# OCR-D/ocrd_keraslm

Hardware: AMD Instinct MI355X
Metric: chars/sec training (stacked-LSTM forward+backward+Adam) (higher is better)
Workload: dtype bf16; 1 GPU; cfg2: depth=2 width=512 length=256 V=256 1 context, stateful training, 3072 streams/GPU, synthetic 10M-char corpus (SURVEY.md 8d); streams_per_gpu=3072, global_batch=3072, seq_len=256, parallelism=dp1

## Files before the change

ocrd_keraslm_amd/csrc/api.hip:

```cpp
#include <hip/hip_runtime.h>
#include <stdio.h>
#include <stdlib.h>
#include <string.h>
#include <time.h>

#include <functional>
#include <utility>

#include <vector>

#include "kl_common.h"
#include "kl_kernels.h"

namespace {

inline size_t align_up(size_t x, size_t a) { return (x + a - 1) / a * a; }
inline int round_up_i(int x, int a) { return (x + a - 1) / a * a; }

struct Carver {
  unsigned char* base;
  size_t off = 0;
  explicit Carver(void* b) : base(reinterpret_cast<unsigned char*>(b)) {}
  template <typename T>
  T* take(size_t count) {
    off = align_up(off, 256);
    T* p = base ? reinterpret_cast<T*>(base + off) : nullptr;
    off += count * sizeof(T);
    return p;
  }
};

constexpr int KL_SCAN_FLAGS = 256 * 64;
struct Derived {
  std::vector<bf16_t*> UT_hi, UT_lo, KT_hi, KT_lo, Un, Kn;
  bf16_t *E_hi = nullptr, *E_lo = nullptr, *ET = nullptr;
  std::vector<bf16_t*> WTcat;
  std::vector<bf16_t*> UF, KF;
  bf16_t* EF = nullptr;
  std::vector<bf16_t*> WTperm;
  bf16_t* Ecat = nullptr;
  float* EK = nullptr;
  std::vector<float*> CtxK;
  std::vector<bf16_t*> KTp;
  std::vector<float*> bp;
  float* EKp = nullptr;
  bf16_t* comb = nullptr;
  std::vector<float*> CtxKp;
  unsigned* scan_flags = nullptr;
};

struct WindowWs {
  float* P1;
  std::vector<void*> H;
  std::vector<float*> C;
  float* logits;
  float* rowstat;
  int *s_idx, *s_ctx, *s_tgt;
  int* ids_tm = nullptr;
  int scan2_rows = 0;
  bool scan2_bwd = false;
  float *s_masks, *s_probs;
  unsigned *scan_cnt, *scan_status;
  float* reg_scratch;
  std::vector<bf16_t*> G, dZ, Hd;
  std::vector<bf16_t*> Cb;
  std::vector<bf16_t*> Xhi, Xlo;
  std::vector<bf16_t*> HTf, HdT;
  bool ht_ready = false;
  bool km_plan = false;
  unsigned p_bf16_mask = 0;
  bf16_t *dZT, *HT, *dlogits, *dlogitsT, *OHT, *dEKT_bf, *dEK_bf;
  std::vector<bf16_t*> OHC;
  bool segsum = false;
  void* seg_ws = nullptr;
  float *dH, *dEKT;
  std::vector<float*> dc0, dc1, dCtxKT;
};

}

struct kl_handle {
  kl_config cfg;
  int Vp;
  size_t n_params;
  std::vector<size_t> off_K, off_U, off_b, off_Ctx;
  size_t off_E;
  float* params = nullptr;
  void* derived_ws = nullptr;
  size_t derived_bytes = 0;
  Derived d;
  int precision = 0;
  struct GraphKey {
    int kind, B, T, flags, precision;
    const void *states, *loss_acc, *ws, *grads;
    int layout = 0;
    bool operator==(const GraphKey& o) const {
      return kind == o.kind && B == o.B && T == o.T && flags == o.flags && precision == o.precision &&
             states == o.states && loss_acc == o.loss_acc && ws == o.ws && grads == o.grads && layout == o.layout;
    }
  };
  std::vector<std::pair<GraphKey, hipGraphExec_t>> graphs;
  bool graphs_enabled = true;
  bool scan_enabled = true;
  bool seq_bwd = true;
  bool wide_bwd = true;
  void* host_step_ready = nullptr;
  std::vector<int32_t> host_pack;
  bool host_kernarg = true;
  void* walk_ready = nullptr;
  bool inc_ready = false;
  bool big_ready = false;
  bool il_ready = false;
  bool comb_ready = false;
  int last_only = 0;
  int loss_rows = 0;
  bool sentinel = true;
  bool gemm_an = true;
  bool xcd_local = false;
  bool sentinel_bwd = true;
  bool sentinel_roll = true;
  bool sentinel_bwd_all = false;
  bool xcd_local_bwd = false;
  bool w32 = true;
  bool w32_local = false;
  int w32_min_rb = 8;
  bool split8 = true;
  bool split_sentinel = true;
  bool inc_small = true;
  bool fused_step = true;
  bool inc_tile = true;
  int tile_var = 0;
  int tile_rows = -1;
  bool out_fused = true;
  int out_fused_min = 512;
  int inc_small_min = KL_SMALL_STEP_N;
  bool scan2 = true;
  int scan2_rows = 0;
  int scan2_pf = -1;
  bool scan2_bf16 = true;
  bool logits_ws = true;
  bool proj_ws = true;
  bool w128 = true;
  bool w128_tables = true;
  bool w128_multi = true;
  bool w128_fuse = true;
  int w128_min = 1;
  bool fwd8 = true;
  bool fwd8_all = false;
  bool fwd8_tab = true;
  bool fwd8_ls = true;
  bool fwd8_local = true;
  int fwd8_pf = -1;
  bool rt_local = true;
  bool regtile = true;
  bool scan2_flags = true;
  bool flags_zeroed = false;
  struct ViewNote {
    int B, T;
    const void* ws;
    int scan2_rows, g_interleaved, c_in_cb, dh_bf16;
    unsigned p_bf16_mask;
    unsigned wg_route = 0, wg_pair_mask = 0, wg_db_scan_mask = 0, hd_mask = 0;
    unsigned out_route = 0;
  };
  std::vector<ViewNote> view_notes;
  ViewNote* view_note(int B, int T, const void* ws, bool insert) {
    for (auto& n : view_notes)
      if (n.B == B && n.T == T && n.ws == ws) return &n;
    if (!insert) return nullptr;
    if (view_notes.size() >= 64) view_notes.erase(view_notes.begin());
    view_notes.push_back(ViewNote{B, T, ws, 0, 0, 0, 0, 0u});
    return &view_notes.back();
  }
  bool segsum = true;
  bool fuse_wg = true;
  int scan2_pfb = -1;
  int wide_fwd_min = 96;
  double trace_flops[2] = {0.0, 0.0};
  bool trace_on = false;
  std::vector<std::pair<hipEvent_t, hipEvent_t>> trace_ev[2];
  size_t trace_used[2] = {0, 0};
  bool trace_open[2] = {false, false};
  bool trace_persistent[2] = {false, false};
  const char* trace_name[2] = {"lstm_fwd_step_kernel", "lstm_bwd_step_kernel"};
  void trace_begin(int kind, hipStream_t s) {
    if (!trace_on) return;
    if (trace_used[kind] == trace_ev[kind].size()) {
      hipEvent_t a, b;
      if (hipEventCreate(&a) != hipSuccess || hipEventCreate(&b) != hipSuccess) { trace_on = false; return; }
      trace_ev[kind].emplace_back(a, b);
    }
    (void)hipEventRecord(trace_ev[kind][trace_used[kind]].first, s);
    trace_open[kind] = true;
  }
  void trace_end(int kind, hipStream_t s) {
    if (!trace_on || !trace_open[kind]) return;
    trace_open[kind] = false;
    (void)hipEventRecord(trace_ev[kind][trace_used[kind]].second, s);
    ++trace_used[kind];
  }
  void drop_graphs() {
    for (auto& g : graphs) (void)hipGraphExecDestroy(g.second);
    graphs.clear();
  }
};

namespace {

void layout(kl_handle* h) {
  const kl_config& c = h->cfg;
  const size_t W = c.width;
  size_t off = 0;
  h->off_E = off;
  off += (size_t)c.voc_size * W;
  h->off_Ctx.clear();
  for (int n = 0; n < c.n_ctx; ++n) {
    h->off_Ctx.push_back(off);
    off += (size_t)c.ctx_vocab * c.ctx_dim;
  }
  h->off_K.clear();
  h->off_U.clear();
  h->off_b.clear();
  for (int l = 0; l < c.depth; ++l) {
    const size_t D = l == 0 ? W + (size_t)c.ctx_dim * c.n_ctx : W;
    h->off_K.push_back(off);
    off += D * 4 * W;
    h->off_U.push_back(off);
    off += W * 4 * W;
    h->off_b.push_back(off);
    off += 4 * W;
  }
  h->n_params = off;
  h->Vp = round_up_i(c.voc_size, 32);
}

bool config_ok(const kl_config* c) {
  if (!c) return false;
  if (c->depth < 1 || c->depth > 16) return false;
  if (c->width < 32 || (c->width & 31)) return false;
// ... 12 lines not shown
  o.UT_hi.assign(c.depth, nullptr); o.UT_lo.assign(c.depth, nullptr);
  o.KT_hi.assign(c.depth, nullptr); o.KT_lo.assign(c.depth, nullptr);
  o.Un.assign(c.depth, nullptr); o.Kn.assign(c.depth, nullptr);
  for (int l = 0; l < c.depth; ++l) {
    o.UT_hi[l] = cv.take<bf16_t>(4 * W * W);
    o.UT_lo[l] = cv.take<bf16_t>(4 * W * W);
    o.KT_hi[l] = cv.take<bf16_t>(4 * W * W);
    o.KT_lo[l] = cv.take<bf16_t>(4 * W * W);
    o.Un[l] = cv.take<bf16_t>(4 * W * W);
    o.Kn[l] = cv.take<bf16_t>(4 * W * W);
  }
  o.E_hi = cv.take<bf16_t>(Vp * W);
  o.E_lo = cv.take<bf16_t>(Vp * W);
  o.ET = cv.take<bf16_t>(W * Vp);
  o.EK = cv.take<float>(V * 4 * W);
  o.WTcat.assign(c.depth, nullptr);
  for (int l = 0; l < c.depth; ++l) o.WTcat[l] = cv.take<bf16_t>(4 * W * 3 * (l == 0 ? W : 2 * W));
  o.WTperm.assign(c.depth, nullptr);
  if ((W & 31) == 0)
    for (int l = 0; l < c.depth; ++l) o.WTperm[l] = cv.take<bf16_t>(4 * W * 3 * (l == 0 ? W : 2 * W));
  o.Ecat = cv.take<bf16_t>(Vp * 3 * W);
  o.UF.assign(c.depth, nullptr);
  o.KF.assign(c.depth, nullptr);
  if ((W & 31) == 0) {
    for (int l = 0; l < c.depth; ++l) {
      o.UF[l] = cv.take<bf16_t>(4 * W * W * 2);
      if (l > 0) o.KF[l] = cv.take<bf16_t>(4 * W * W * 2);
    }
    o.EF = cv.take<bf16_t>(Vp * W * 2);
  }
  o.CtxK.assign(c.n_ctx, nullptr);
  for (int n = 0; n < c.n_ctx; ++n) o.CtxK[n] = cv.take<float>((size_t)c.ctx_vocab * 4 * W);
  o.KTp.assign(c.depth, nullptr);
  o.bp.assign(c.depth, nullptr);
  for (int l = 1; l < c.depth; ++l) {
    o.KTp[l] = cv.take<bf16_t>(4 * W * W);
    o.bp[l] = cv.take<float>(4 * W);
  }
  o.EKp = cv.take<float>(V * 4 * W);
  o.CtxKp.assign(c.n_ctx, nullptr);
  for (int n = 0; n < c.n_ctx; ++n) o.CtxKp[n] = cv.take<float>((size_t)c.ctx_vocab * 4 * W);
  o.scan_flags = cv.take<unsigned>(KL_SCAN_FLAGS + 64);
  o.comb = nullptr;
  if (h->fwd8_tab && W == 512 && c.n_ctx == 1 && V * (size_t)c.ctx_vocab * 4 * W * sizeof(bf16_t) <= ((size_t)512 << 20))
    o.comb = cv.take<bf16_t>(V * (size_t)c.ctx_vocab * 4 * W);
  return align_up(cv.off, 256);
}

bool kl_segsum_applicable(const kl_handle* h, int B, int T) {
  const kl_config& c = h->cfg;
  if (!h->segsum || B < 1 || T < 1 || (long)B * T > 0x7fffffffL) return false;
  return (long)kl_segment_sums_buckets(c.n_ctx, h->Vp, c.ctx_vocab) <= KL_SEGSUM_MAX_BUCKETS;
}

size_t carve_window(const kl_handle* h, void* base, int B, int T, int training, WindowWs* out) {
  const kl_config& c = h->cfg;
  const size_t W = c.width, V = c.voc_size, Vp = h->Vp, L = c.depth;
  const size_t BT = (size_t)B * T, BTp = round_up_i((int)BT, 8);
  Carver cv(base);
  WindowWs tmp;
  WindowWs& o = out ? *out : tmp;
  o.P1 = cv.take<float>(BT * 4 * W);
  o.H.assign(L, nullptr);
  o.C.assign(L, nullptr);
  for (size_t l = 0; l < L; ++l) {
    o.H[l] = training ? (void*)cv.take<bf16_t>((BT + B) * W) : (void*)cv.take<float>((BT + B) * W);
    o.C[l] = cv.take<float>((BT + B) * W);
  }
  o.Xhi.assign(L, nullptr); o.Xlo.assign(L, nullptr);
  if (!training) {
    for (size_t l = 0; l < L; ++l) {
      o.Xhi[l] = cv.take<bf16_t>((BT + B) * W);
      o.Xlo[l] = cv.take<bf16_t>((BT + B) * W);
    }
  }
  o.logits = cv.take<float>(BT * V);
  o.rowstat = cv.take<float>(BT * 2);
  o.s_idx = cv.take<int>(BT);
  o.s_ctx = cv.take<int>(BT * (size_t)(c.n_ctx > 0 ? c.n_ctx : 1));
  o.s_tgt = cv.take<int>(BT);
  o.s_masks = cv.take<float>(training ? L * (size_t)B * W : 1);
  o.s_probs = cv.take<float>(BT * V);
  o.scan_cnt = cv.take<unsigned>(L * ((size_t)(B + 15) / 16) * T);
  o.scan_status = cv.take<unsigned>(4 + 256);
  o.reg_scratch = cv.take<float>(3 * (W > (size_t)c.ctx_dim ? W : (size_t)c.ctx_dim) + (V > (size_t)c.ctx_vocab ? V : (size_t)c.ctx_vocab) + 8);
  if (training) {
    o.G.assign(L, nullptr); o.dZ.assign(L, nullptr); o.Hd.assign(L, nullptr); o.Cb.assign(L, nullptr);
    o.dc0.assign(L, nullptr); o.dc1.assign(L, nullptr);
    for (size_t l = 0; l < L; ++l) {
      o.G[l] = cv.take<bf16_t>(BT * 4 * W);
      o.dZ[l] = cv.take<bf16_t>(BT * 4 * W);
      o.Hd[l] = l > 0 ? cv.take<bf16_t>(BT * W) : nullptr;
      o.Cb[l] = cv.take<bf16_t>((BT + B) * W);
      o.dc0[l] = cv.take<float>((size_t)B * W);
      o.dc1[l] = cv.take<float>((size_t)B * W);
    }
    o.dZT = cv.take<bf16_t>(4 * W * BTp);
    o.HT = cv.take<bf16_t>(W * BTp);
    o.ids_tm = cv.take<int>((BT + B) * 2);
    o.HTf.assign(L, nullptr); o.HdT.assign(L, nullptr);
    if ((B & 7) == 0) {
      for (size_t l = 0; l < L; ++l) {
        o.HTf[l] = cv.take<bf16_t>(W * (BT + B));
        o.HdT[l] = l > 0 ? cv.take<bf16_t>(W * BT) : nullptr;
      }
    }
    o.dlogits = cv.take<bf16_t>(BT * Vp);
    o.dlogitsT = cv.take<bf16_t>(Vp * BTp);
    o.segsum = kl_segsum_applicable(h, B, T);
    o.OHT = o.segsum ? nullptr : cv.take<bf16_t>(Vp * BTp);
    o.seg_ws = o.segsum ? cv.take<char>(kl_segment_sums_ws_bytes(B, T, c.n_ctx, (int)Vp, c.ctx_vocab)) : nullptr;
    o.OHC.assign(c.n_ctx, nullptr);
    o.dCtxKT.assign(c.n_ctx, nullptr);
    for (int n = 0; n < c.n_ctx; ++n) {
      o.OHC[n] = (o.segsum && n == 0) ? nullptr : cv.take<bf16_t>((size_t)c.ctx_vocab * BTp);
      o.dCtxKT[n] = cv.take<float>(4 * W * (size_t)c.ctx_vocab);
    }
    o.dH = cv.take<float>(BT * W);
    o.dEKT = cv.take<float>(4 * W * Vp);
    o.dEKT_bf = cv.take<bf16_t>(4 * W * Vp);
    o.dEK_bf = cv.take<bf16_t>(Vp * 4 * W);
  }
  return align_up(cv.off, 256);
}

#define KL_TRY(expr)            \
  do {                          \
    int _e = (expr);            \
    if (_e != 0) return _e;     \
  } while (0)

int hip_ok(hipError_t e) { return e == hipSuccess ? 0 : KL_ERR_LAUNCH; }

int prepare_impl(kl_handle* h, int precision, hipStream_t s) {
  const kl_config& c = h->cfg;
  const int W = c.width, V = c.voc_size, Vp = h->Vp;
  const float* P = h->params;
  Derived& d = h->d;
  const bool split = precision == KL_PREC_SPLIT;
  if (!h->flags_zeroed) {
    hipStreamCaptureStatus cap = hipStreamCaptureStatusNone;
    if (hipStreamIsCapturing(s, &cap) == hipSuccess && cap == hipStreamCaptureStatusNone) {
      KL_TRY(kl_zero_async(d.scan_flags, (size_t)(KL_SCAN_FLAGS + 64) * sizeof(unsigned), s));
      h->flags_zeroed = true;
    }
  }
  const float* E = P + h->off_E;
  {
    KlConvJob jobs[KL_CONV_MAX_JOBS];
    int nj = 0;
    auto add = [&](const float* in, long ld_in, int rows, int cols, int rows_pad, bf16_t* hi, bf16_t* lo, long ld_out, int tr) -> int {
      jobs[nj++] = KlConvJob{in, ld_in, rows, cols, rows_pad, tr, hi, lo, ld_out};
      if (nj < KL_CONV_MAX_JOBS) return 0;
      nj = 0;
      return kl_launch_f32_to_bf16_jobs(jobs, KL_CONV_MAX_JOBS, s);
    };
    for (int l = 0; l < c.depth; ++l) {
      const float* K = P + h->off_K[l];
      const float* U = P + h->off_U[l];
      KL_TRY(add(U, 4 * W, W, 4 * W, W, d.UT_hi[l], split ? d.UT_lo[l] : nullptr, W, 1));
      KL_TRY(add(K, 4 * W, W, 4 * W, W, d.KT_hi[l], split ? d.KT_lo[l] : nullptr, W, 1));
      KL_TRY(add(U, 4 * W, W, 4 * W, W, d.Un[l], nullptr, 4 * W, 0));
      KL_TRY(add(K, 4 * W, W, 4 * W, W, d.Kn[l], nullptr, 4 * W, 0));
    }
    KL_TRY(add(E, W, V, W, Vp, d.E_hi, split ? d.E_lo : nullptr, W, 0));
    KL_TRY(add(E, W, V, W, Vp, d.ET, nullptr, Vp, 1));
    if (nj > 0) KL_TRY(kl_launch_f32_to_bf16_jobs(jobs, nj, s));
  }
  KlOperand op;
  memset(&op, 0, sizeof(op));
  op.A = E; op.lda = W; op.a_is_f32 = 1;
  op.WT_hi = d.KT_hi[0]; op.WT_lo = split ? d.KT_lo[0] : nullptr; op.ldw = W; op.K = W;
  KL_TRY(kl_launch_thin_gemm(&op, V, 4 * W, d.EK, 4 * W, nullptr, precision, s));
  for (int n = 0; n < c.n_ctx; ++n) {
    const float* Kc = P + h->off_K[0] + (size_t)(W + n * c.ctx_dim) * 4 * W;
    KL_TRY(kl_launch_small_table(P + h->off_Ctx[n], c.ctx_vocab, c.ctx_dim, Kc, 4 * W, 4 * W, d.CtxK[n], 4 * W, s));
  }
  h->il_ready = precision == KL_PREC_BF16 && h->scan2 && W == 512;
  h->comb_ready = false;
  if (h->il_ready) {
    for (int l = 1; l < c.depth; ++l) {
      KL_TRY(kl_launch_permute_gate_rows_bf16(d.KT_hi[l], d.KTp[l], W, W, s));
      KL_TRY(kl_launch_permute_gate_cols_f32(P + h->off_b[l], nullptr, d.bp[l], 1, W, s));
    }
    KL_TRY(kl_launch_permute_gate_cols_f32(d.EK, P + h->off_b[0], d.EKp, V, W, s));
    for (int n = 0; n < c.n_ctx; ++n) KL_TRY(kl_launch_permute_gate_cols_f32(d.CtxK[n], nullptr, d.CtxKp[n], c.ctx_vocab, W, s));
  }
  h->precision = precision;
  h->inc_ready = false;
  h->big_ready = false;
  return 0;
}

int prepare_incremental(kl_handle* h, hipStream_t s) {
  const kl_config& c = h->cfg;
  const int W = c.width, Vp = h->Vp;
  Derived& d = h->d;
  const bool split = h->precision == KL_PREC_SPLIT;
  if (d.EF) {
    for (int l = 0; l < c.depth; ++l) {
      KL_TRY(kl_launch_frag_major(d.UT_hi[l], split ? d.UT_lo[l] : nullptr, 4 * W, W, W, d.UF[l], s));
      if (l > 0) KL_TRY(kl_launch_frag_major(d.KT_hi[l], split ? d.KT_lo[l] : nullptr, 4 * W, W, W, d.KF[l], s));
    }
    KL_TRY(kl_launch_frag_major(d.E_hi, split ? d.E_lo : nullptr, Vp, W, W, d.EF, s));
  }
  h->inc_ready = true;
  return 0;
}

int prepare_big_step(kl_handle* h, hipStream_t s) {
  const kl_config& c = h->cfg;
  const int W = c.width, V = c.voc_size, Vp = h->Vp;
  const float* P = h->params;
  Derived& d = h->d;
  const bool split = h->precision == KL_PREC_SPLIT;
  const float* E = P + h->off_E;
  for (int l = 0; l < c.depth; ++l) {
    const int Kl = l == 0 ? W : 2 * W;
    const long ld = 3L * Kl;
    const float* K = P + h->off_K[l];
    const float* U = P + h->off_U[l];
    bf16_t* base = d.WTcat[l];
    const int uoff = l == 0 ? 0 : W;
    if (l > 0) {
      KL_TRY(kl_launch_f32_to_bf16_t(K, 4 * W, W, 4 * W, base, split ? base + 2 * Kl : nullptr, ld, 1, s));
      if (split) KL_TRY(kl_launch_f32_to_bf16_t(K, 4 * W, W, 4 * W, base + Kl, nullptr, ld, 1, s));
    }
    KL_TRY(kl_launch_f32_to_bf16_t(U, 4 * W, W, 4 * W, base + uoff, split ? base + 2 * Kl + uoff : nullptr, ld, 1, s));
    if (split) KL_TRY(kl_launch_f32_to_bf16_t(U, 4 * W, W, 4 * W, base + Kl + uoff, nullptr, ld, 1, s));
    if (d.WTperm[l]) KL_TRY(kl_launch_permute_gate_rows(base, d.WTperm[l], W, ld, s));
  }
  KL_TRY(kl_zero_async(d.Ecat, (size_t)Vp * 3 * W * sizeof(bf16_t), s));
  KL_TRY(kl_launch_f32_to_bf16_t(E, W, V, W, d.Ecat, split ? d.Ecat + 2 * W : nullptr, 3 * W, 0, s));
  if (split) KL_TRY(kl_launch_f32_to_bf16_t(E, W, V, W, d.Ecat + W, nullptr, 3 * W, 0, s));
  h->big_ready = true;
  return 0;
}

int build_comb(kl_handle* h, hipStream_t s) {
  const kl_config& c = h->cfg;
  KL_TRY(kl_launch_comb_table(h->d.EKp, h->d.CtxKp[0], c.voc_size, c.ctx_vocab, 4 * c.width, h->d.comb, s));
  h->comb_ready = true;
  return 0;
}

int plan_scan2(const kl_handle* h, int B, int T, bool km_plan, bool need_bwd) {
  const kl_config& c = h->cfg;
  const int W = c.width;
  if (!h->scan2 || !h->scan_enabled || !h->sentinel || !km_plan || T < 3) return 0;
  if (c.n_ctx > 1 && !h->scan2_bf16) return 0;
  if (W != 512) return 0;
  if (h->wide_fwd_min <= 0 || !kl_scan_fwd_wide_applicable(B, T, W) || ((B + 15) / 16) * (W / 64) < h->wide_fwd_min) return 0;
  if (need_bwd && (!h->wide_bwd || !h->seq_bwd || !h->sentinel_bwd || !h->sentinel_roll || !kl_scan_wide2_phases(B, T, W, 16, 6))) return 0;
  const int p16 = kl_scan_wide2_phases(B, T, W, 16, 5), p32 = kl_scan_wide2_phases(B, T, W, 32, 4);
  if (h->scan2_rows == 16) return p16 ? 16 : 0;
  if (h->scan2_rows == 32) return p32 ? 32 : 0;
  if (p32 >= 2) return 32;
  if (p16) return 16;
  return p32 ? 32 : 0;
}

struct FwdCall {
  kl_handle* h; int B, T; const int *idx, *ctx; float* states; const float* masks; int training, split; WindowWs& w; hipStream_t s;
  int W, L; size_t BW; int n_rb;
};
constexpr int FWD_PASS = -1;
static_assert(FWD_PASS < KL_OK, "FWD_PASS must not be a public return code");

static const void* h_rows(const FwdCall& c, int l, int block) {
// ... 283 lines not shown
  return 0;
}

static int fwd_split_fused(const FwdCall& c) {
  const kl_handle* h = c.h; const int L = c.L;
  if (!(!c.training && c.split == KL_PREC_SPLIT && h->scan_enabled && L <= KL_SCAN_MAXL)) return FWD_PASS;
  KlScanFwdSplit a = scan_args<KlScanFwdSplit>(c, L);
  for (int l = 0; l < L; ++l) split_layer_args(c, a, l, l, true);
  for (int l = 0; l < L; ++l) KL_TRY(split_planes(c, l));
  a.sentinel = h->split_sentinel ? 1 : 0;
  if (a.sentinel)
    for (int l = 0; l < L; ++l) KL_TRY(arm_split(c, l));
  else
    KL_TRY(kl_zero_coherent_async(c.w.scan_cnt, (size_t)L * c.n_rb * c.T, c.s));
  const int e = kl_launch_scan_fwd_split(a, c.s);
  return e == KL_ERR_SHAPE ? FWD_PASS : e;
}

static int fwd_fused_thin(const FwdCall& c) {
  kl_handle* h = c.h; const int L = c.L;
  if (!(c.training && h->scan_enabled && L <= KL_SCAN_MAXL)) return FWD_PASS;
  KlScanFwd a = scan_args<KlScanFwd>(c, L);
  for (int l = 0; l < L; ++l) thin_layer_args(c, a, l, l, true);
  KL_TRY(kl_zero_coherent_async(c.w.scan_cnt, (size_t)L * c.n_rb * c.T, c.s));
  h->trace_begin(0, c.s);
  const int e = kl_launch_scan_fwd(a, c.s);
  if (e != 0) return e == KL_ERR_SHAPE ? FWD_PASS : e;
  trace_fwd_scan(c, "lstm_scan_fwd_kernel", (2.0 * L - 1.0) * layer_flops(c));
  return 0;
}

static KlFwdStep wavefront_step(const FwdCall& c, int l, int t) {
  const kl_handle* h = c.h; const WindowWs& w = c.w; const Derived& d = h->d;
  const int B = c.B, W = c.W; const size_t BW = c.BW;
  const bool lo = c.split == KL_PREC_SPLIT;
  KlFwdStep S;
  memset(&S, 0, sizeof(S));
  S.n_rows = B; S.W = W; S.split = c.split; S.n_ops = l > 0 ? 2 : 1;
  KlOperand& u = S.op[S.n_ops - 1];
  u.A = h_rows(c, l, t); u.a_is_f32 = c.training ? 0 : 1; u.lda = W;
  u.WT_hi = d.UT_hi[l]; u.WT_lo = lo ? d.UT_lo[l] : nullptr; u.ldw = W; u.K = W;
  if (l > 0) {
    KlOperand& o = S.op[0];
    o.A = c.training ? (const void*)(layer_in(c, l) + (size_t)t * BW) : h_rows(c, l - 1, t + 1); o.a_is_f32 = c.training ? 0 : 1;
    o.lda = W; o.WT_hi = d.KT_hi[l]; o.WT_lo = lo ? d.KT_lo[l] : nullptr; o.ldw = W; o.K = W;
    S.bias = h->params + h->off_b[l];
  } else {
    S.T1 = w.P1 + (size_t)t * B * 4 * W; S.t1_ld = 4 * W;
  }
  S.c_prev = w.C[l] + (size_t)t * BW; S.c_prev_ld = W;
  S.c_out = w.C[l] + (size_t)(t + 1) * BW; S.c_out_ld = W;
  if (c.training) {
    const LayerMask m = layer_mask(c, l);
    S.h_out_bf16 = (bf16_t*)w.H[l] + (size_t)(t + 1) * BW; S.h_out_bf16_ld = W;
    S.gates_out = w.G[l] + (size_t)t * B * 4 * W; S.gates_ld = 4 * W;
    if (m.mask) {
      S.hmask = m.mask; S.hmask_ld = W;
      S.hd_out_bf16 = m.Hd + (size_t)t * BW; S.hd_out_ld = W;
    }
  } else {
    S.h_out_f32 = (float*)w.H[l] + (size_t)(t + 1) * BW; S.h_out_f32_ld = W;
  }
  return S;
}

static int fwd_wavefront(const FwdCall& c) {
  kl_handle* h = c.h; const int T = c.T, L = c.L;
  for (int dgl = 0; dgl < T + L - 1; ++dgl) {
    KlFwdStep steps[16];
    int ns = 0;
    for (int l = 0; l < L; ++l)
      if (dgl - l >= 0 && dgl - l < T) steps[ns++] = wavefront_step(c, l, dgl - l);
    for (int i = 0; i < ns; i += 4) {
      const bool steady = (ns == L) && dgl >= L && dgl + 8 < T;
      if (steady && dgl % 8 == 0) h->trace_begin(0, c.s);
      KL_TRY(kl_launch_fwd_steps(steps + i, ns - i < 4 ? ns - i : 4, c.s));
      if (steady && dgl % 8 == 7) h->trace_end(0, c.s);
    }
  }
  return 0;
}

int forward_impl(kl_handle* h, int B, int T, const int* idx, const int* ctx, float* states, const float* masks,
                 int training, WindowWs& w, hipStream_t s) {
  const int W = h->cfg.width, L = h->cfg.depth;
  const FwdCall c = {h, B, T, idx, ctx, states, masks, training, training ? 1 : h->precision, w, s, W, L, (size_t)B * W, (B + 15) / 16};
  for (int l = 0; l < L; ++l)
    KL_TRY(kl_launch_state_to_rows(states, B, W, L, l, training ? (bf16_t*)w.H[l] : nullptr, training ? nullptr : (float*)w.H[l], w.C[l], s));
  int e = fwd_wide(c);
  if (e == FWD_PASS && !fwd_w128_tables(c)) KL_TRY(gather_layer0(c));
  if (e == FWD_PASS) e = fwd_w128(c);
  if (e == FWD_PASS) e = fwd_layer_by_layer(c);
  if (e == FWD_PASS) e = fwd_split_pairs(c);
  if (e == FWD_PASS) e = fwd_split_layers(c);
  if (e == FWD_PASS) e = fwd_split_fused(c);
  if (e == FWD_PASS) e = fwd_fused_thin(c);
  if (e == FWD_PASS) e = fwd_wavefront(c);
  KL_TRY(e);
  for (int l = 0; l < L; ++l)
    KL_TRY(kl_launch_rows_to_state(h_rows(c, l, T), training ? 0 : 1, w.C[l] + (size_t)T * c.BW, B, W, L, l, states, s));
  return 0;
}

__global__ void scan_status_kernel(const unsigned* status, float* loss_acc) {
  if (threadIdx.x == 0 && (status[0] | status[1]) != 0) loss_acc[3] += 1.f;
}

__global__ void state_dist2_kernel(const float* __restrict__ pool, long slot_stride, int W, int k,
                                   const int* __restrict__ a, const int* __restrict__ b, int n,
                                   float* __restrict__ out) {
  const int lane = threadIdx.x & 63;
  const int i = blockIdx.x * (blockDim.x >> 6) + (threadIdx.x >> 6);
  if (i >= n) return;
  const float* pa = pool + (long)a[i] * slot_stride + (long)k * W;
  const float* pb = pool + (long)b[i] * slot_stride + (long)k * W;
  float acc = 0.f;
  for (int u = lane; u < W; u += 64) { const float q = pa[u] - pb[u]; acc += q * q; }
#pragma unroll
  for (int off = 32; off > 0; off >>= 1) acc += __shfl_xor(acc, off);
  if (lane == 0) out[i] = acc;
}

}

extern "C" {

int kl_abi_version(void) { return KL_ABI_VERSION; }

const char* kl_error_string(int code) {
  switch (code) {
    case KL_OK: return "ok";
    case KL_ERR_SHAPE: return "unsupported or inconsistent dimensions";
    case KL_ERR_LAUNCH: return "HIP launch/runtime error";
    case KL_ERR_STATE: return "call order violated (bind/prepare first)";
    case KL_ERR_WORKSPACE: return "workspace too small";
    case KL_ERR_ARG: return "null or invalid argument";
    default: return "unknown error";
  }
}

size_t kl_param_count(const kl_config* cfg) {
  if (!config_ok(cfg)) return 0;
  kl_handle tmp;
  tmp.cfg = *cfg;
  layout(&tmp);
  return tmp.n_params;
}

int kl_param_layout(const kl_config* cfg, int index, char* name, size_t name_cap, size_t* offset, size_t* rows,
                    size_t* cols) {
  if (!config_ok(cfg) || index < 0) return KL_ERR_ARG;
  kl_handle t;
  t.cfg = *cfg;
  layout(&t);
  const size_t W = cfg->width;
  char buf[32];
  size_t off, r, c;
  const int n_emb = 1 + cfg->n_ctx;
  if (index == 0) {
    snprintf(buf, sizeof buf, "E"); off = t.off_E; r = cfg->voc_size; c = W;
  } else if (index < n_emb) {
    snprintf(buf, sizeof buf, "Ctx%d", index - 1); off = t.off_Ctx[index - 1]; r = cfg->ctx_vocab; c = cfg->ctx_dim;
  } else {
    const int j = index - n_emb, l = j / 3, k = j % 3;
    if (l >= cfg->depth) return KL_ERR_ARG;
    const size_t D = l == 0 ? W + (size_t)cfg->ctx_dim * cfg->n_ctx : W;
    if (k == 0) { snprintf(buf, sizeof buf, "K%d", l); off = t.off_K[l]; r = D; c = 4 * W; }
    else if (k == 1) { snprintf(buf, sizeof buf, "U%d", l); off = t.off_U[l]; r = W; c = 4 * W; }
    else { snprintf(buf, sizeof buf, "b%d", l); off = t.off_b[l]; r = 1; c = 4 * W; }
  }
  if (name && name_cap) { strncpy(name, buf, name_cap - 1); name[name_cap - 1] = 0; }
  if (offset) *offset = off;
  if (rows) *rows = r;
  if (cols) *cols = c;
  return 0;
}

kl_handle* kl_create(const kl_config* cfg) {
  if (!config_ok(cfg)) return nullptr;
  kl_handle* h = new kl_handle();
  h->cfg = *cfg;
  layout(h);
  const char* env8tb = getenv("KL_FWD8_TAB");
  if (env8tb) h->fwd8_tab = atoi(env8tb) != 0;
  const char* env9 = getenv("KL_SEGSUM");
  if (env9) h->segsum = atoi(env9) != 0;
  return h;
}

void kl_destroy(kl_handle* h) {
  if (h) {
    h->drop_graphs();
    for (auto& list : h->trace_ev)
      for (auto& ev : list) {
        (void)hipEventDestroy(ev.first);
        (void)hipEventDestroy(ev.second);
      }
  }
  delete h;
}

size_t kl_derived_bytes(const kl_handle* h) { return h ? carve_derived(h, nullptr, nullptr) : 0; }

int kl_bind(kl_handle* h, float* params, void* derived, size_t derived_bytes) {
  if (!h || !params || !derived) return KL_ERR_ARG;
  if (derived_bytes < carve_derived(h, nullptr, nullptr)) return KL_ERR_WORKSPACE;
  h->params = params;
  h->derived_ws = derived;
  h->derived_bytes = derived_bytes;
  carve_derived(h, derived, &h->d);
  h->precision = 0;
  h->drop_graphs();
  const char* env = getenv("KL_GRAPH");
  h->graphs_enabled = !(env && env[0] == '0');
  const char* env2 = getenv("KL_SCAN");
  h->scan_enabled = !(env2 && env2[0] == '0');
  const char* env3 = getenv("KL_SEQ_BWD");
  h->seq_bwd = !(env3 && env3[0] == '0');
  const char* env4 = getenv("KL_WIDE_BWD");
  h->wide_bwd = !(env4 && env4[0] == '0');
  const char* env7 = getenv("KL_SENTINEL");
  h->sentinel = !(env7 && env7[0] == '0');
  const char* env7e = getenv("KL_GEMM_AN");
  h->gemm_an = !(env7e && env7e[0] == '0');
  const char* env7c = getenv("KL_XCD_LOCAL");
  h->xcd_local = env7c && env7c[0] == '1';
  const char* env7b = getenv("KL_SENTINEL_BWD");
  h->sentinel_bwd = h->sentinel && !(env7b && env7b[0] == '0');
  h->sentinel_bwd_all = env7b && env7b[0] == '2';
  const char* env7f = getenv("KL_SENTINEL_ROLL");
  h->sentinel_roll = !(env7f && env7f[0] == '0');
  const char* env7d = getenv("KL_XCD_LOCAL_BWD");
  h->xcd_local_bwd = h->xcd_local && env7d && env7d[0] == '1';
  const char* env6f = getenv("KL_W32");
  h->w32 = !(env6f && env6f[0] == '0');
  const char* env6g = getenv("KL_W32_LOCAL");
  h->w32_local = env6g && env6g[0] == '1';
  const char* env6h = getenv("KL_W32_MIN_RB");
  h->w32_min_rb = env6h ? atoi(env6h) : 8;
  const char* env6j = getenv("KL_SPLIT8");
  h->split8 = !(env6j && env6j[0] == '0');
  const char* env6c = getenv("KL_SPLIT_SENTINEL");
  h->split_sentinel = !(env6c && env6c[0] == '0');
  const char* env6b = getenv("KL_INC_SMALL");
  h->inc_small = !(env6b && env6b[0] == '0');
  const char* env6 = getenv("KL_FUSED_STEP");
  h->fused_step = !(env6 && env6[0] == '0');
  const char* env6k = getenv("KL_INC_TILE");
  h->inc_tile = !(env6k && env6k[0] == '0');
  const char* env6l = getenv("KL_TILE_VAR");
  h->tile_var = env6l ? atoi(env6l) : 0;
  const char* env6r = getenv("KL_TILE_ROWS");
  if (env6r) h->tile_rows = atoi(env6r);
  const char* env6m = getenv("KL_OUT_FUSED");
  h->out_fused = !(env6m && env6m[0] == '0');
  const char* env6n = getenv("KL_OUT_FUSED_MIN");
  if (env6n) h->out_fused_min = atoi(env6n);
  const char* env6o = getenv("KL_INC_SMALL_MIN");
  if (env6o) h->inc_small_min = atoi(env6o);
  const char* env6p = getenv("KL_HOST_KERNARG");
  h->host_kernarg = !(env6p && env6p[0] == '0');
  const char* env8 = getenv("KL_SCAN2");
  if (env8) h->scan2 = atoi(env8) != 0;
  const char* env8b = getenv("KL_SCAN2_ROWS");
  if (env8b) h->scan2_rows = atoi(env8b);
  const char* env8c = getenv("KL_SCAN2_PF");
  if (env8c) h->scan2_pf = atoi(env8c);
  const char* env8e = getenv("KL_SCAN2_BF16");
  if (env8e) h->scan2_bf16 = atoi(env8e) != 0;
  const char* env8i = getenv("KL_LOGITS_WS");
  if (env8i) h->logits_ws = atoi(env8i) != 0;
  const char* env8h = getenv("KL_PROJ_WS");
  if (env8h) h->proj_ws = atoi(env8h) != 0;
  const char* env8p = getenv("KL_W128");
  if (env8p) h->w128 = atoi(env8p) != 0;
  const char* env8s = getenv("KL_W128_FUSE");
  if (env8s) h->w128_fuse = atoi(env8s) != 0;
  const char* env8t = getenv("KL_W128_TABLES");
  if (env8t) h->w128_tables = atoi(env8t) != 0;
  const char* env8mm = getenv("KL_W128_MULTI");
  if (env8mm) h->w128_multi = atoi(env8mm) != 0;
  const char* env8q = getenv("KL_W128_MIN");
  if (env8q) h->w128_min = atoi(env8q);
  const char* env8m = getenv("KL_FWD8");
  if (env8m) { h->fwd8 = atoi(env8m) != 0; h->fwd8_all = atoi(env8m) == 2; }
  const char* env8r = getenv("KL_FWD8_LS");
  if (env8r) h->fwd8_ls = atoi(env8r) != 0;
  const char* env8n = getenv("KL_FWD8_LOCAL");
  if (env8n) h->fwd8_local = atoi(env8n) != 0;
  const char* env8o = getenv("KL_FWD8_PF");
  if (env8o) h->fwd8_pf = atoi(env8o);
  const char* env8l = getenv("KL_RT_LOCAL");
  if (env8l) h->rt_local = atoi(env8l) != 0;
  const char* env8k = getenv("KL_REGTILE");
  if (env8k) h->regtile = atoi(env8k) != 0;
  const char* env8g = getenv("KL_SCAN2_FLAGS");
  if (env8g) h->scan2_flags = atoi(env8g) != 0;
  h->flags_zeroed = false;
  const char* env8f = getenv("KL_FUSE_WG");
  if (env8f) h->fuse_wg = atoi(env8f) != 0;
  const char* env8d = getenv("KL_SCAN2_PFB");
  if (env8d) h->scan2_pfb = atoi(env8d);
  const char* env5 = getenv("KL_WIDE_FWD_MIN");
  if (env5) h->wide_fwd_min = atoi(env5);
  return kl_zero_page_ready();
}

int kl_prepare(kl_handle* h, int precision, void* stream) {
  if (!h) return KL_ERR_ARG;
  if (!h->params) return KL_ERR_STATE;
  if (precision != KL_PREC_BF16 && precision != KL_PREC_SPLIT) return KL_ERR_ARG;
  return prepare_impl(h, precision, (hipStream_t)stream);
}

size_t kl_window_workspace_bytes(const kl_handle* h, int B, int T, int training) {
  if (!h || B < 1 || T < 1) return 0;
  return carve_window(h, nullptr, B, T, training, nullptr);
}

static int window_logits(kl_handle* h, int B, int T, const int32_t* idx, const int32_t* ctx, float* states, WindowWs& w,
                         hipStream_t s) {
  const int W = h->cfg.width, V = h->cfg.voc_size, L = h->cfg.depth;
  KL_TRY(kl_zero_async(w.scan_status, (4 + 256) * sizeof(unsigned), s));
  KL_TRY(forward_impl(h, B, T, idx, ctx, states, nullptr, 0, w, s));
  KlOperand op;
  memset(&op, 0, sizeof(op));
  op.A = (float*)w.H[L - 1] + (size_t)B * W; op.lda = W; op.a_is_f32 = 1;
  op.WT_hi = h->d.E_hi; op.WT_lo = h->precision == 3 ? h->d.E_lo : nullptr; op.ldw = W; op.K = W;
  return kl_launch_thin_gemm(&op, B * T, V, w.logits, V, nullptr, h->precision, s);
}

static int forward_window_tail(kl_handle* h, WindowWs& w, int B, int T, const int32_t* tgt, int mean_rows, float* probs, float* loss_acc, hipStream_t s) {
  const int V = h->cfg.voc_size;
  KL_TRY(kl_launch_softmax_ce(w.logits, V, B * T, V, tgt, B, T, 1.0f / (h->last_only ? (float)mean_rows : (float)mean_rows * (float)T),
                              nullptr, 0, tgt ? loss_acc : nullptr, w.rowstat, 1, s, h->last_only));
  if (probs) {
    if (B == 1) KL_TRY(hip_ok(hipMemcpyAsync(probs, w.logits, (size_t)T * V * sizeof(float), hipMemcpyDeviceToDevice, s)));
    else KL_TRY(kl_launch_rows_tm_to_bm(w.logits, V, probs, B, T, V, s));
  }
  if (loss_acc) hipLaunchKernelGGL(scan_status_kernel, dim3(1), dim3(64), 0, s, w.scan_status, loss_acc);
  return hip_ok(hipGetLastError());
}

static int window_logits_training(kl_handle* h, int B, int T, const int32_t* idx, const int32_t* ctx, float* states, WindowWs& w,
                                  hipStream_t s) {
  const int W = h->cfg.width, V = h->cfg.voc_size, L = h->cfg.depth;
  KL_TRY(kl_zero_async(w.scan_status, (4 + 256) * sizeof(unsigned), s));
  w.km_plan = true;
  w.scan2_rows = plan_scan2(h, B, T, true, false);
  KL_TRY(forward_impl(h, B, T, idx, ctx, states, nullptr, 1, w, s));
  const bf16_t* Htop = (const bf16_t*)w.H[L - 1] + (size_t)B * W;
  return kl_launch_gemm_tn(Htop, h->d.E_hi, w.logits, nullptr, B * T, V, W, W, W, V, 0, 1, 1.f, s);
}

static int forward_window_body(kl_handle* h, int B, int T, const int32_t* idx, const int32_t* ctx, const int32_t* tgt,
                      float* states, float* probs, float* loss_acc, void* ws, size_t ws_bytes, void* stream) {
  if (!h || !idx || !states || !ws || B < 1 || T < 1) return KL_ERR_ARG;
  if (h->cfg.n_ctx > 0 && !ctx) return KL_ERR_ARG;
  if (!h->precision) return KL_ERR_STATE;
  hipStream_t s = (hipStream_t)stream;
  WindowWs w;
  if (h->precision == KL_PREC_BF16 && ws_bytes >= carve_window(h, nullptr, B, T, 1, nullptr)) {
    carve_window(h, ws, B, T, 1, &w);
    KL_TRY(window_logits_training(h, B, T, idx, ctx, states, w, s));
    const int mean_rows = (h->loss_rows > 0 && h->loss_rows <= B) ? h->loss_rows : B;
    return forward_window_tail(h, w, B, T, tgt, mean_rows, probs, loss_acc, s);
  }
  if (ws_bytes < carve_window(h, ws, B, T, 0, &w)) return KL_ERR_WORKSPACE;
  KL_TRY(window_logits(h, B, T, idx, ctx, states, w, s));
  return forward_window_tail(h, w, B, T, tgt, B, probs, loss_acc, s);
}

struct TrainCall {
  kl_handle* h; int B, T; const int32_t *idx, *ctx, *tgt; const float* masks; float *grads, *loss_acc; hipStream_t s;
  WindowWs& w; kl_handle::ViewNote& note;
  int W, V, Vp, L, BT, BTp; size_t BW;
  int ksplit;
  long ldtf;
  int dh_mode;
  bool top_masked; float inv_count;
  bool wide_fits, seq128, sequential;
};
constexpr int TRAIN_PASS = -1;
static_assert(TRAIN_PASS < KL_OK, "TRAIN_PASS must not be a public return code");

struct RowsOperand {
  const bf16_t* km; long ld;
  const bf16_t* t; long ldt;
};
static RowsOperand layer_out(const TrainCall& c, int l) {
  const WindowWs& w = c.w;
  if (c.masks != nullptr && l > 0) return {w.Hd[l], c.W, w.ht_ready ? w.HdT[l] : nullptr, c.BT};
  return {(const bf16_t*)w.H[l] + c.BW, c.W, w.ht_ready ? w.HTf[l] + c.B : nullptr, c.ldtf};
}

static int rows_product(const TrainCall& c, bool km, const RowsOperand& a, int M, const RowsOperand& x, int N, float* out, long ldc, bool out_t) {
  const bool onehot = x.km == nullptr;
  if (km) return kl_launch_gemm_an(a.km, onehot ? x.t : x.km, out, M, N, c.BT, a.ld, onehot ? x.ldt : x.ld, ldc, out_t ? 1 : 0, c.s, onehot ? 0 : 1);
  const bf16_t* xT = x.t;
  long ldx = x.ldt; int K = onehot ? c.BTp : c.BT;
  if (!xT) {
    KL_TRY(kl_launch_transpose_bf16(x.km, x.ld, c.w.HT, c.BTp, c.BT, N, c.s));
    xT = c.w.HT; ldx = c.BTp; K = c.BTp;
  }
  return out_t ? kl_launch_gemm_tn(xT, a.t, out, nullptr, N, M, K, ldx, a.ldt, ldc, 2, c.ksplit, 1.f, c.s)
               : kl_launch_gemm_tn(a.t, xT, out, nullptr, M, N, K, a.ldt, ldx, ldc, 2, c.ksplit, 1.f, c.s);
}

static int onehot(const TrainCall& c, const int32_t* src, int classes, int rows, int var, int n_vars, bf16_t* out, float* sums) {
  if (kl_launch_onehot_dense(src, c.B, c.T, rows, var, n_vars, out, c.BTp, c.s) == KL_ERR_SHAPE) {
    KL_TRY(kl_zero_async(out, (size_t)rows * c.BTp * sizeof(bf16_t), c.s));
    KL_TRY(kl_launch_onehot_t(src, c.B, c.T, classes, var, n_vars, out, c.BTp, c.s));
  }
  return kl_zero_async(sums, (size_t)4 * c.W * rows * sizeof(float), c.s);
}

static int train_output_layer(const TrainCall& c) {
  kl_handle* h = c.h; WindowWs& w = c.w; const Derived& d = h->d; hipStream_t s = c.s;
  const int B = c.B, T = c.T, W = c.W, V = c.V, Vp = c.Vp, BT = c.BT, BTp = c.BTp;
  const RowsOperand top = layer_out(c, c.L - 1);
  int fe = KL_ERR_SHAPE;
  if (h->logits_ws && c.loss_acc != nullptr && w.rowstat != nullptr && V == Vp)
    fe = kl_launch_logits_ce_ws(top.km, d.E_hi, c.tgt, w.dlogits, w.rowstat, B, T, W, V, Vp, c.inv_count, h->last_only, s);
  bool dh_done = false;
  if (fe == KL_ERR_SHAPE && h->logits_ws && W == 128 && c.loss_acc != nullptr && w.rowstat != nullptr && !w.scan2_bwd) {
    fe = kl_launch_logits_ce_w128(top.km, d.E_hi, d.ET, c.tgt, w.dlogits, w.dH, w.rowstat, B, T, W, V, Vp, c.inv_count, h->last_only, s);
    dh_done = fe == 0;
  }
  if (fe != 0 && fe != KL_ERR_SHAPE) return fe;
  if (fe == 0) c.note.out_route |= dh_done ? KL_OUT_LOGITS_W128 : KL_OUT_LOGITS_WS;
  if (fe == 0) KL_TRY(kl_launch_rowstat_reduce(w.rowstat, BT, c.loss_acc, s));
  else {
    KL_TRY(kl_launch_gemm_tn(top.km, d.E_hi, w.logits, nullptr, BT, V, W, W, W, V, 0, 1, 1.f, s));
    KL_TRY(kl_launch_softmax_ce(w.logits, V, BT, V, c.tgt, B, T, c.inv_count, w.dlogits, Vp, c.loss_acc, w.rowstat, 1, s, h->last_only));
  }
  int de = KL_ERR_SHAPE;
  if (c.dh_mode == 1 && h->logits_ws) de = kl_launch_dh_ws(w.dlogits, d.ET, reinterpret_cast<bf16_t*>(w.dH), BT, W, Vp, s);
  if (de == 0) c.note.out_route |= KL_OUT_DH_WS;
  if (dh_done) de = 0;
  if (de == KL_ERR_SHAPE) de = kl_launch_gemm_tn(w.dlogits, d.ET, w.dH, nullptr, BT, W, Vp, Vp, Vp, W, c.dh_mode, 1, 1.f, s);
  KL_TRY(de);
  if (BTp != BT) {
    KL_TRY(kl_zero_async(w.dlogitsT, (size_t)Vp * BTp * sizeof(bf16_t), s));
    KL_TRY(kl_zero_async(w.HT, (size_t)W * BTp * sizeof(bf16_t), s));
    KL_TRY(kl_zero_async(w.dZT, (size_t)4 * W * BTp * sizeof(bf16_t), s));
  }
  const bool km_e = w.km_plan && Vp == V && kl_gemm_an_applicable(V, W, BT, Vp);
  if (km_e) c.note.out_route |= KL_OUT_DE_KMAJOR;
  if (!km_e) KL_TRY(kl_launch_transpose_bf16(w.dlogits, Vp, w.dlogitsT, BTp, BT, Vp, s));
  return rows_product(c, km_e, {w.dlogits, Vp, w.dlogitsT, BTp}, V, top, W, c.grads + h->off_E, W, false);
}

static int table_grads(const TrainCall& c) {
  kl_handle* h = c.h; WindowWs& w = c.w; const kl_config& cf = h->cfg; const Derived& d = h->d; hipStream_t s = c.s;
  const int B = c.B, T = c.T, W = c.W, V = c.V, Vp = c.Vp, BT = c.BT, BTp = c.BTp;
  const bool km = w.km_plan, seg = w.segsum;
  const RowsOperand dz = {w.dZ[0], 4 * W, w.dZT, BTp};
  bool pair_ctx = false;
  if (seg) {
    KL_TRY(kl_launch_segment_sums(w.dZ[0], 4 * W, B, T, 4 * W, c.idx, c.ctx, cf.n_ctx, Vp, cf.ctx_vocab, w.dEKT,
                                  cf.n_ctx > 0 ? w.dCtxKT[0] : nullptr, w.seg_ws, s));
    KL_TRY(kl_launch_f32_to_bf16_t(w.dEKT, 4 * W, Vp, 4 * W, w.dEKT_bf, nullptr, Vp, 1, s));
    KL_TRY(kl_launch_f32_to_bf16_t(w.dEKT, 4 * W, Vp, 4 * W, w.dEK_bf, nullptr, 4 * W, 0, s));
  } else {
    KL_TRY(onehot(c, c.idx, V, Vp, 0, 1, w.OHT, w.dEKT));
    pair_ctx = km && h->fuse_wg && cf.n_ctx >= 1 && (Vp % 128) == 0 && kl_gemm_an_applicable(4 * W, Vp + cf.ctx_vocab, BT, 4 * W);
    if (pair_ctx) {
      KL_TRY(onehot(c, c.ctx, cf.ctx_vocab, cf.ctx_vocab, 0, cf.n_ctx, w.OHC[0], w.dCtxKT[0]));
      const int pe = kl_launch_gemm_an2(w.dZ[0], w.OHT, w.dEKT, 4 * W, Vp, BT, 4 * W, BTp, Vp, 0,
                                        w.OHC[0], w.dCtxKT[0], cf.ctx_vocab, BTp, cf.ctx_vocab, 0, s, 0);
      if (pe == KL_ERR_SHAPE) pair_ctx = false;
      else KL_TRY(pe);
    }
    if (!pair_ctx) KL_TRY(rows_product(c, km, dz, 4 * W, {nullptr, 0, w.OHT, BTp}, Vp, w.dEKT, Vp, false));
    KL_TRY(kl_launch_f32_to_bf16_t(w.dEKT, Vp, 4 * W, Vp, w.dEKT_bf, nullptr, Vp, 0, s));
    KL_TRY(kl_launch_f32_to_bf16_t(w.dEKT, Vp, 4 * W, Vp, w.dEK_bf, nullptr, 4 * W, 1, s));
  }
  c.note.wg_route |= (seg ? KL_WG_SEGSUM : 0) | (pair_ctx ? KL_WG_PAIR_CTX : 0);
  KL_TRY(kl_launch_gemm_tn(d.ET, w.dEKT_bf, c.grads + h->off_K[0], nullptr, W, 4 * W, Vp, Vp, Vp, 4 * W, 0, 1, 1.f, s));
  KL_TRY(kl_launch_gemm_tn(w.dEK_bf, d.Kn[0], c.grads + h->off_E, nullptr, V, W, 4 * W, 4 * W, 4 * W, W, 2, 1, 1.f, s));
  for (int n = 0; n < cf.n_ctx; ++n) {
    const bool seg_n = seg && n == 0;
    if (!(pair_ctx && n == 0) && !seg_n) {
      KL_TRY(onehot(c, c.ctx, cf.ctx_vocab, cf.ctx_vocab, n, cf.n_ctx, w.OHC[n], w.dCtxKT[n]));
      KL_TRY(rows_product(c, km, dz, 4 * W, {nullptr, 0, w.OHC[n], BTp}, cf.ctx_vocab, w.dCtxKT[n], cf.ctx_vocab, false));
    }
    const size_t krow = (size_t)(W + n * cf.ctx_dim) * 4 * W;
    KL_TRY(kl_launch_ctx_grads(h->params + h->off_Ctx[n], h->params + h->off_K[0] + krow, 4 * W, cf.ctx_vocab, cf.ctx_dim,
                               w.dCtxKT[n], seg_n ? 1 : cf.ctx_vocab, 4 * W, c.grads + h->off_K[0] + krow, 4 * W,
                               c.grads + h->off_Ctx[n], s, seg_n ? 4 * W : 1));
  }
  return 0;
}

static int weight_grads(const TrainCall& c, int l, bool dzt_ready, bool db_done) {
  kl_handle* h = c.h; WindowWs& w = c.w; hipStream_t s = c.s;
  const int W = c.W, BT = c.BT; const bool km = w.km_plan;
  if (!dzt_ready && !km) KL_TRY(kl_launch_transpose_bf16(w.dZ[l], 4 * W, w.dZT, c.BTp, BT, 4 * W, s));
  const RowsOperand dz = {w.dZ[l], 4 * W, w.dZT, c.BTp}, Hprev = {(const bf16_t*)w.H[l], W, w.ht_ready ? w.HTf[l] : nullptr, c.ldtf};
  bool pair_uk = km && l > 0 && h->fuse_wg && (W % 128) == 0 && kl_gemm_an_applicable(4 * W, 2 * W, BT, 4 * W);
  if (pair_uk) {
    const int pe = kl_launch_gemm_an2(w.dZ[l], Hprev.km, c.grads + h->off_U[l], 4 * W, W, BT, 4 * W, W, 4 * W, 1,
                                      layer_out(c, l - 1).km, c.grads + h->off_K[l], W, W, 4 * W, 1, s, 1);
    if (pe == KL_ERR_SHAPE) pair_uk = false;
    else KL_TRY(pe);
  }
  c.note.wg_route |= km ? KL_WG_KMAJOR : (w.ht_ready ? KL_WG_SCAN_T : KL_WG_TRANSPOSE);
  if (pair_uk) c.note.wg_pair_mask |= 1u << l;
  if (db_done) c.note.wg_db_scan_mask |= 1u << l;
  if (!pair_uk) KL_TRY(rows_product(c, km, dz, 4 * W, Hprev, W, c.grads + h->off_U[l], 4 * W, true));
  if (!db_done) KL_TRY(kl_launch_colsum_bf16(w.dZ[l], 4 * W, BT, 4 * W, c.grads + h->off_b[l], s));
  if (l == 0) return table_grads(c);
  if (!pair_uk) KL_TRY(rows_product(c, km, dz, 4 * W, layer_out(c, l - 1), W, c.grads + h->off_K[l], 4 * W, true));
  return 0;
}

static KlScanBwd bwd_scan_args(const TrainCall& c, int first, int n) {
  const Derived& d = c.h->d;
  KlScanBwd a;
  memset(&a, 0, sizeof(a));
  a.B = c.B; a.T = c.T; a.W = c.W; a.L = n;
  for (int j = 0; j < n; ++j) {
    const int l = first + j;
    a.Un[j] = d.Un[l]; a.G[j] = c.w.G[l]; a.C[j] = c.w.C[l]; a.dZ[j] = c.w.dZ[l];
    a.mask[j] = (c.masks != nullptr && l > 0) ? c.masks + (size_t)l * c.BW : nullptr;
  }
  a.dH = c.w.dH; a.status = c.w.scan_status + 1;
  return a;
}

static int arm_dz(const TrainCall& c, int l, ArmMode mode) {
  const size_t T = c.T, BW = c.BW;
  if (mode == ARM_COUNTERS) return kl_zero_coherent_async(c.w.scan_cnt, (size_t)((c.B + 15) / 16) * T, c.s);
  const size_t first = mode == ARM_ROLLING ? (T - 2) * BW * 4 : 0, steps = mode == ARM_ROLLING ? 2 : T;
  return kl_fill_u32_async(c.w.dZ[l] + first, steps * BW * 4 * sizeof(bf16_t), 0xFFFFFFFFu, c.s);
}

static void trace_bwd_scan(const TrainCall& c, const char* kernel, double flops) {
  c.h->trace_persistent[1] = true; c.h->trace_name[1] = kernel; c.h->trace_flops[1] = flops;
  c.h->trace_end(1, c.s);
}

static int bwd_w128_multi(const TrainCall& c) {
  kl_handle* h = c.h;
  const int B = c.B, T = c.T, W = c.W, L = c.L;
  if (!(c.seq128 && h->w128_fuse && h->w128_multi && kl_scan_w128_multi_fits(B, L))) return TRAIN_PASS;
  KlScanBwd a = bwd_scan_args(c, 0, L);
  for (int l = 0; l < L; ++l) { a.Kn[l] = h->d.Kn[l]; a.db_l[l] = c.grads + h->off_b[l]; }
  const bool roll = h->sentinel_roll && T >= 3;
  a.sentinel = roll ? 2 : 1;
  for (int l = 1; l < L; ++l) KL_TRY(arm_dz(c, l, roll ? ARM_ROLLING : ARM_ALL_STEPS));
  h->trace_begin(1, c.s);
  const int e = kl_launch_scan_bwd_w128_multi(a, c.s);
  if (e != 0) return e == KL_ERR_SHAPE ? TRAIN_PASS : e;
  trace_bwd_scan(c, "lstm_scan_bwd_w128_multi_kernel", (double)(2 * L - 1) * B * T * (2.0 * W * 4.0 * W));
  for (int l = L - 1; l >= 0; --l) KL_TRY(weight_grads(c, l, false, true));
  return 0;
}

enum BwdKernel { BWD_REGTILE, BWD_WIDE2, BWD_WIDE, BWD_W128, BWD_W32, BWD_THIN };
static const char* const BWD_KERNEL_NAME[] = {"lstm_scan_bwd_regtile_kernel", "lstm_scan_bwd_wide2_kernel", "lstm_scan_bwd_wide_kernel",
                                              "lstm_scan_bwd_w128_kernel",    "lstm_scan_bwd_w32_kernel",   "lstm_scan_bwd_kernel"};

static int launch_layer_scan(const TrainCall& c, int l, KlScanBwd& a, bool rt, bool fuse_dx, BwdKernel* ran) {
  kl_handle* h = c.h; WindowWs& w = c.w; hipStream_t s = c.s;
  if (w.scan2_bwd) {
    *ran = rt ? BWD_REGTILE : BWD_WIDE2;
    return rt ? kl_launch_scan_bwd_regtile(a, s) : kl_launch_scan_bwd_wide2(a, s);
  }
  *ran = BWD_WIDE;
  int e = h->wide_bwd ? kl_launch_scan_bwd_wide(a, s) : KL_ERR_SHAPE;
  if (e == KL_ERR_SHAPE && c.seq128) {
    KlScanBwd a1 = a;
// ... 53 lines not shown
    BwdKernel ran;
    KL_TRY(launch_layer_scan(c, l, a, rt, fuse_dx, &ran));
    trace_bwd_scan(c, BWD_KERNEL_NAME[ran], (double)B * T * (2.0 * W * 4.0 * W));
    KL_TRY(weight_grads(c, l, a.dZT != nullptr, ran != BWD_THIN));
  }
  return 0;
}

static int bwd_fused_thin(const TrainCall& c) {
  kl_handle* h = c.h;
  const int B = c.B, T = c.T, W = c.W, L = c.L;
  if (!(h->scan_enabled && L <= KL_SCAN_MAXL)) return TRAIN_PASS;
  KlScanBwd a = bwd_scan_args(c, 0, L);
  a.counters = c.w.scan_cnt;
  for (int l = 0; l < L; ++l) a.Kn[l] = h->d.Kn[l];
  KL_TRY(kl_zero_coherent_async(c.w.scan_cnt, (size_t)L * ((B + 15) / 16) * T, c.s));
  h->trace_begin(1, c.s);
  const int e = kl_launch_scan_bwd(a, c.s);
  if (e != 0) return e == KL_ERR_SHAPE ? TRAIN_PASS : e;
  trace_bwd_scan(c, "lstm_scan_bwd_kernel", (double)B * T * (2.0 * (2.0 * L - 1.0) * W * 4.0 * W));
  return 0;
}

static int bwd_wavefront(const TrainCall& c) {
  kl_handle* h = c.h; WindowWs& w = c.w; const Derived& d = h->d; hipStream_t s = c.s;
  const int B = c.B, T = c.T, W = c.W, L = c.L;
  const size_t BW = c.BW; const float* masks = c.masks;
  for (int dgl = 0; dgl < T + L - 1; ++dgl) {
    KlBwdStep steps[16];
    int ns = 0;
    for (int j = 0; j < L; ++j) {
      const int l = L - 1 - j;
      const int t = T - 1 - (dgl - j);
      if (t < 0 || t >= T) continue;
      KlBwdStep& S = steps[ns++];
      memset(&S, 0, sizeof(S));
      S.n_rows = B; S.W = W;
      int p = 0;
      if (l < L - 1) {
        KlOperand& o = S.op[p++];
        o.A = w.dZ[l + 1] + (size_t)t * B * 4 * W; o.lda = 4 * W; o.a_is_f32 = 0;
        o.WT_hi = d.Kn[l + 1]; o.ldw = 4 * W; o.K = 4 * W;
        if (masks != nullptr && l > 0) { S.op0_mask = masks + (size_t)l * BW; S.op0_mask_ld = W; }
      } else {
        S.dh_in = w.dH + (size_t)t * BW; S.dh_in_ld = W;
        if (c.top_masked) { S.dh_mask = masks + (size_t)l * BW; S.dh_mask_ld = W; }
      }
      if (t < T - 1) {
        KlOperand& o = S.op[p++];
        o.A = w.dZ[l] + (size_t)(t + 1) * B * 4 * W; o.lda = 4 * W; o.a_is_f32 = 0;
        o.WT_hi = d.Un[l]; o.ldw = 4 * W; o.K = 4 * W;
      }
      S.n_ops = p;
      if (S.op0_mask && !(l < L - 1)) S.op0_mask = nullptr;
      S.gates = w.G[l] + (size_t)t * B * 4 * W; S.gates_ld = 4 * W;
      S.c = w.C[l] + (size_t)(t + 1) * BW; S.c_ld = W;
      S.c_prev = w.C[l] + (size_t)t * BW; S.c_prev_ld = W;
      float* dc_rd = (t & 1) ? w.dc1[l] : w.dc0[l];
      float* dc_wr = (t & 1) ? w.dc0[l] : w.dc1[l];
      if (t < T - 1) { S.dc_in = dc_rd; S.dc_in_ld = W; }
      S.dc_out = dc_wr; S.dc_out_ld = W;
      S.dz_out = w.dZ[l] + (size_t)t * B * 4 * W; S.dz_ld = 4 * W;
    }
    for (int i = 0; i < ns; i += 4) {
      const bool steady = (ns == L) && dgl >= L && dgl + 8 < T;
      if (steady && dgl % 8 == 0) h->trace_begin(1, s);
      KL_TRY(kl_launch_bwd_steps(steps + i, ns - i < 4 ? ns - i : 4, s));
      if (steady && dgl % 8 == 7) h->trace_end(1, s);
    }
  }
  return 0;
}

static int train_window_body(kl_handle* h, int B, int T, const int32_t* idx, const int32_t* ctx, const int32_t* tgt,
                    float* states, const float* masks, float* grads, float* loss_acc, void* ws, size_t ws_bytes,
                    void* stream) {
  hipStream_t s = (hipStream_t)stream;
  WindowWs w;
  if (ws_bytes < carve_window(h, ws, B, T, 1, &w)) return KL_ERR_WORKSPACE;
  const kl_config& cf = h->cfg;
  const int W = cf.width, V = cf.voc_size, Vp = h->Vp, L = cf.depth;
  const int BT = B * T, BTp = round_up_i(BT, 8);
  const float* P = h->params;
  KL_TRY(kl_zero_async(grads, h->n_params * sizeof(float), s));
  KL_TRY(kl_zero_async(w.scan_status, (4 + 256) * sizeof(unsigned), s));
  w.km_plan = h->gemm_an && BTp == BT && kl_gemm_an_applicable(4 * W, W, BT, 4 * W);
  w.scan2_rows = plan_scan2(h, B, T, w.km_plan, true);
  w.scan2_bwd = w.scan2_rows != 0;
  KL_TRY(forward_impl(h, B, T, idx, ctx, states, masks, 1, w, s));
  const int n_rb_all = (B + 15) / 16, nug = W / 16;
  const bool thin_fits = (n_rb_all + 512 / nug - 1) / (512 / nug) <= (W == 1024 ? 8 : 4) &&
                         (long)T * B * 4 * W * 2 <= 0xfffffff0L;
  const bool wide_fits = h->wide_bwd && kl_scan_bwd_wide_applicable(B, T, W) && BTp == BT && (B & 7) == 0;
  const bool seq128 = h->scan_enabled && h->seq_bwd && h->w128 && B >= h->w128_min && kl_scan_w128_applicable(B, T, W) && !w.scan2_bwd;
  const bool sequential = seq128 || (h->scan_enabled && h->seq_bwd &&
                          ((L > 1 && L <= KL_SCAN_MAXL && (W == 512 || W == 256 || W == 128) && n_rb_all > 512 / (L * nug)) ||
                           W == 1024 || (L > KL_SCAN_MAXL && (W == 512 || W == 256 || W == 128 || W == 64))) &&
                          (thin_fits || wide_fits));
  const int mean_rows = (h->loss_rows > 0 && h->loss_rows <= B) ? h->loss_rows : B;
  const TrainCall c = {h, B, T, idx, ctx, tgt, masks, grads, loss_acc, s, w, *h->view_note(B, T, ws, true), W, V, Vp, L, BT, BTp, (size_t)B * W,
                        BT >= 4096 ? 8 : (BT >= 1024 ? 4 : 1),  (long)(T + 1) * B,
                        w.scan2_bwd ? 1 : 0,
                        masks != nullptr && L > 1,
                        1.0f / (h->last_only ? (float)mean_rows : (float)mean_rows * (float)T), wide_fits, seq128, sequential};
  c.note = kl_handle::ViewNote{B, T, ws, w.scan2_rows, w.scan2_bwd ? 1 : 0, (w.scan2_bwd && h->scan2_bf16) ? 1 : 0, w.scan2_bwd ? 1 : 0,
                               w.p_bf16_mask};
  c.note.hd_mask = masks != nullptr ? ((1u << L) - 1u) & ~1u : 0u;
  KL_TRY(train_output_layer(c));
  int e = bwd_w128_multi(c);
  if (e == TRAIN_PASS) e = bwd_layer_by_layer(c);
  if (e == TRAIN_PASS) {
    e = bwd_fused_thin(c);
    if (e == TRAIN_PASS) e = bwd_wavefront(c);
    for (int l = L - 1; l >= 0 && e == 0; --l) e = weight_grads(c, l, false, false);
  }
  KL_TRY(e);
  std::vector<const float*> ctabs(cf.n_ctx);
  std::vector<float*> gctabs(cf.n_ctx);
  for (int n = 0; n < cf.n_ctx; ++n) { ctabs[n] = P + h->off_Ctx[n]; gctabs[n] = grads + h->off_Ctx[n]; }
  KL_TRY(kl_launch_regulariser_grads(P + h->off_E, V, W, ctabs.data(), cf.n_ctx, cf.ctx_vocab, cf.ctx_dim,
                                     grads + h->off_E, gctabs.data(), loss_acc, w.reg_scratch, s));
  hipLaunchKernelGGL(scan_status_kernel, dim3(1), dim3(64), 0, s, w.scan_status, loss_acc);
  return hip_ok(hipGetLastError());
}

int kl_adam_step_scaled(kl_handle* h, const float* grads, float grad_scale, float* m, float* v, int t, float lr, float b1,
                        float b2, float eps, float clip, void* stream) {
  if (!h || !grads || !m || !v || t < 1) return KL_ERR_ARG;
  if (!h->params) return KL_ERR_STATE;
  hipStream_t s = (hipStream_t)stream;
  const double lr_t = (double)lr * sqrt(1.0 - pow((double)b2, (double)t)) / (1.0 - pow((double)b1, (double)t));
  KL_TRY(kl_launch_adam(h->params, grads, m, v, h->n_params, (float)lr_t, b1, b2, eps, clip, grad_scale, s));
  return prepare_impl(h, h->precision ? h->precision : KL_PREC_BF16, s);
}

int kl_adam_step(kl_handle* h, const float* grads, float* m, float* v, int t, float lr, float b1, float b2,
                 float eps, float clip, void* stream) {
  return kl_adam_step_scaled(h, grads, 1.0f, m, v, t, lr, b1, b2, eps, clip, stream);
}

namespace {
struct StepWs {
  float* prow;
  float* z;
  bf16_t* A3;
  bf16_t* rows[16];
  size_t bytes;
};
static StepWs step_carve(const kl_handle* h, int n, void* ws) {
  const size_t W = h->cfg.width;
  Carver cv(ws);
  StepWs w;
  w.prow = cv.take<float>((size_t)n * 4 * W);
  w.z = cv.take<float>((size_t)n * 4 * W);
  w.A3 = cv.take<bf16_t>((size_t)n * 3 * 2 * W);
  for (int l = 0; l < h->cfg.depth; ++l) w.rows[l] = cv.take<bf16_t>((size_t)n * 3 * (l == 0 ? 1 : 2) * W);
  w.bytes = align_up(cv.off, 256);
  return w;
}

struct GateSrc { const float* T1; const int32_t* i1; const float* T2; const int32_t* i2; const float* bias; };
static GateSrc gate_src(const kl_handle* h, int l, const float* prow, const int32_t* idx, const int32_t* ctx) {
  if (l > 0) return {nullptr, nullptr, nullptr, nullptr, h->params + h->off_b[l]};
  if (prow) return {prow, nullptr, nullptr, nullptr, nullptr};
  return {h->d.EK, idx, h->d.CtxK[0], ctx, h->params + h->off_b[0]};
}

static KlIncCellArgs inc_cell_args(const kl_handle* h, int l, int n, float* pool, const int32_t* slot_in, const int32_t* slot_out,
                                   const float* prow, const int32_t* idx, const int32_t* ctx) {
  const int W = h->cfg.width;
  const GateSrc g = gate_src(h, l, prow, idx, ctx);
  KlIncCellArgs a;
  memset(&a, 0, sizeof(a));
  a.n = n; a.W = W; a.split = h->precision;
  a.pool = pool; a.slot_ld = (long)2 * h->cfg.depth * W; a.slot_in = slot_in; a.slot_out = slot_out;
  a.h_off = 2 * l * W; a.c_off = (2 * l + 1) * W; a.x_off = l > 0 ? 2 * (l - 1) * W : -1;
  a.UF = h->d.UF[l]; a.KF = h->d.KF[l];
  a.T1 = g.T1; a.i1 = g.i1; a.T2 = g.T2; a.i2 = g.i2; a.bias = g.bias;
  return a;
}

static int output_thin(const kl_handle* h, int n, const float* pool, const int32_t* slots, float* out, bool softmax, hipStream_t s) {
  const Derived& d = h->d;
  const int W = h->cfg.width, L = h->cfg.depth, V = h->cfg.voc_size, split = h->precision;
  KlOperand op;
  memset(&op, 0, sizeof(op));
  op.A = pool + (size_t)2 * (L - 1) * W; op.lda = (long)2 * L * W; op.row_index = slots; op.a_is_f32 = 1;
  op.WT_hi = d.E_hi; op.WT_lo = split == 3 ? d.E_lo : nullptr; op.ldw = W; op.K = W;
  KL_TRY(kl_launch_thin_gemm(&op, n, V, out, V, nullptr, split, s));
  return softmax ? kl_launch_softmax_ce(out, V, n, V, nullptr, n, 1, 1.f, nullptr, 0, nullptr, nullptr, 0, s) : 0;
}

struct StepCall {
  kl_handle* h; int n; const int32_t *idx, *ctx; float* pool; const int32_t *slot_in, *slot_out; float* probs;
  const float* prow;
  hipStream_t s;
};

struct StepPlan {
  int layers, out;
  KlIncTilePlan tile;
  KlIncCellPlan cell[16];
// ... 556 lines not shown
                      float* tprob, int32_t* alt_id, float* alt_p, int32_t* rank, void* stream) {
  return kl_launch_rate_topk(logits, ld, rows, V, tgt, B, T, K, tprob, alt_id, alt_p, rank, (hipStream_t)stream);
}

}

extern "C" int kl_test_fwd_step(const uint16_t* A, long lda, const uint16_t* WT, long ldw, int K, int n_ops,
                                int n_rows, int W, int fused, int iters, float* c_out, uint16_t* h_out,
                                void* stream) {
  KlFwdStep st[4];
  if (fused < 1 || fused > 4 || n_ops < 1 || n_ops > 2) return KL_ERR_ARG;
  for (int f = 0; f < fused; ++f) {
    KlFwdStep& S = st[f];
    memset(&S, 0, sizeof(S));
    S.n_rows = n_rows; S.W = W; S.split = 1; S.n_ops = n_ops;
    for (int p = 0; p < n_ops; ++p) {
      KlOperand& o = S.op[p];
      o.A = A; o.lda = lda; o.WT_hi = WT + (size_t)(f * 2 + p) * (size_t)4 * W * ldw; o.ldw = ldw;
      o.K = K; o.a_is_f32 = 0;
    }
    S.c_out = c_out + (size_t)f * n_rows * W; S.c_out_ld = W;
    S.h_out_bf16 = h_out + (size_t)f * n_rows * W; S.h_out_bf16_ld = W;
  }
  for (int i = 0; i < iters; ++i) {
    int e = kl_launch_fwd_steps(st, fused, (hipStream_t)stream);
    if (e) return e;
  }
  return 0;
}


namespace {

int run_graphed(kl_handle* h, const kl_handle::GraphKey& key, hipStream_t s, const std::function<int()>& body) {
  if (!h->graphs_enabled || h->trace_on || s == nullptr) return body();
  for (auto& g : h->graphs)
    if (g.first == key) return hip_ok(hipGraphLaunch(g.second, s));
  if (hipStreamBeginCapture(s, hipStreamCaptureModeThreadLocal) != hipSuccess) {
    (void)hipGetLastError();
    h->graphs_enabled = false;
    return body();
  }
  const int e = body();
  hipGraph_t graph = nullptr;
  const hipError_t ce = hipStreamEndCapture(s, &graph);
  if (e != 0 || ce != hipSuccess || graph == nullptr) {
    if (graph) (void)hipGraphDestroy(graph);
    (void)hipGetLastError();
    h->graphs_enabled = false;
    return e != 0 ? e : body();
  }
  hipGraphExec_t exec = nullptr;
  const hipError_t ie = hipGraphInstantiate(&exec, graph, nullptr, nullptr, 0);
  (void)hipGraphDestroy(graph);
  if (ie != hipSuccess || exec == nullptr) {
    (void)hipGetLastError();
    h->graphs_enabled = false;
    return body();
  }
  if (h->graphs.size() >= 16) h->drop_graphs();
  h->graphs.emplace_back(key, exec);
  return hip_ok(hipGraphLaunch(exec, s));
}

}

extern "C" int kl_set_loss_rows(kl_handle* h, int rows) {
  if (!h || rows < 0) return KL_ERR_ARG;
  h->loss_rows = rows;
  return 0;
}

extern "C" int kl_set_window_mode(kl_handle* h, int last_only) {
  if (!h) return KL_ERR_ARG;
  h->last_only = last_only ? 1 : 0;
  return 0;
}

namespace {

int stage_window(const kl_handle* h, const WindowWs& w, int B, int T, const int32_t* idx, const int32_t* ctx,
                 const int32_t* tgt, const float* masks, hipStream_t s) {
  const size_t BT = (size_t)B * T;
  KL_TRY(hip_ok(hipMemcpyAsync(w.s_idx, idx, BT * sizeof(int), hipMemcpyDeviceToDevice, s)));
  if (h->cfg.n_ctx > 0)
    KL_TRY(hip_ok(hipMemcpyAsync(w.s_ctx, ctx, BT * h->cfg.n_ctx * sizeof(int), hipMemcpyDeviceToDevice, s)));
  if (tgt) KL_TRY(hip_ok(hipMemcpyAsync(w.s_tgt, tgt, BT * sizeof(int), hipMemcpyDeviceToDevice, s)));
  if (masks)
    KL_TRY(hip_ok(hipMemcpyAsync(w.s_masks, masks, (size_t)h->cfg.depth * B * h->cfg.width * sizeof(float),
                                 hipMemcpyDeviceToDevice, s)));
  return 0;
}

}

extern "C" int kl_forward_window(kl_handle* h, int B, int T, const int32_t* idx, const int32_t* ctx, const int32_t* tgt,
                                 float* states, float* probs, float* loss_acc, void* ws, size_t ws_bytes,
                                 void* stream) {
  if (!h || !idx || !states || !ws || B < 1 || T < 1) return KL_ERR_ARG;
  if (h->cfg.n_ctx > 0 && !ctx) return KL_ERR_ARG;
  if (!h->precision) return KL_ERR_STATE;
  hipStream_t s = (hipStream_t)stream;
  WindowWs w;
  const int layout = (h->precision == KL_PREC_BF16 && ws_bytes >= carve_window(h, nullptr, B, T, 1, nullptr)) ? 1 : 0;
  if (ws_bytes < carve_window(h, ws, B, T, layout, &w)) return KL_ERR_WORKSPACE;
  const size_t BT = (size_t)B * T;
  KL_TRY(stage_window(h, w, B, T, idx, ctx, tgt, nullptr, s));
  kl_handle::GraphKey key{0, B, T, (tgt ? 1 : 0) | (probs ? 2 : 0) | (h->last_only ? 4 : 0) | (h->loss_rows << 3), h->precision, states, loss_acc, ws, nullptr, layout};
  KL_TRY(run_graphed(h, key, s, [&]() {
    return forward_window_body(h, B, T, w.s_idx, w.s_ctx, tgt ? w.s_tgt : nullptr, states, probs ? w.s_probs : nullptr,
                               loss_acc, ws, ws_bytes, stream);
  }));
  if (probs)
    KL_TRY(hip_ok(hipMemcpyAsync(probs, w.s_probs, BT * h->cfg.voc_size * sizeof(float), hipMemcpyDeviceToDevice, s)));
  return 0;
}

namespace {

struct AltsWs {
  float* tprob;
  int* alt_id;
  float* alt_p;
  int* rank;
};

size_t carve_alts(void* base, size_t BT, int K, AltsWs* out) {
  Carver cv(base);
  AltsWs tmp;
  AltsWs& o = out ? *out : tmp;
  o.tprob = cv.take<float>(BT);
  o.alt_id = cv.take<int>(BT * K);
  o.alt_p = cv.take<float>(BT * K);
  o.rank = cv.take<int>(BT);
  return align_up(cv.off, 256);
}

int rate_window_impl(kl_handle* h, int layout, int K, int B, int T, const int32_t* idx, const int32_t* ctx,
                     const int32_t* tgt, float* states, float* tprob, int32_t* alt_id, float* alt_p, int32_t* rank,
                     double* bits, float* status, void* ws, size_t ws_bytes, void* stream) {
  const bool alts = K != 0;
  if (!h || !idx || !states || !ws || B < 1 || T < 1) return KL_ERR_ARG;
  if (h->cfg.n_ctx > 0 && !ctx) return KL_ERR_ARG;
  if (alts ? !tgt || !alt_id || !alt_p || K < 1 || K > KL_RATE_ALTS_MAX : (tprob || bits) && !tgt) return KL_ERR_ARG;
  if ((layout ? h->precision != KL_PREC_BF16 : !h->precision) || h->last_only) return KL_ERR_STATE;
  hipStream_t s = (hipStream_t)stream;
  WindowWs w;
  AltsWs a{};
  const size_t BT = (size_t)B * T;
  const size_t n_window = carve_window(h, nullptr, B, T, layout, nullptr);
  if (ws_bytes < n_window + (alts ? carve_alts(nullptr, BT, K, nullptr) : 0)) return KL_ERR_WORKSPACE;
  carve_window(h, ws, B, T, layout, &w);
  if (alts) carve_alts(reinterpret_cast<unsigned char*>(ws) + n_window, BT, K, &a);
  else a.tprob = w.s_probs;
  const bool pick = alts || tprob || bits;
  KL_TRY(stage_window(h, w, B, T, idx, ctx, pick ? tgt : nullptr, nullptr, s));
  const int flags = (tprob ? 1 : 0) | (bits ? 2 : 0) | (alts ? (rank ? 4 : 0) | (K << 3) : 0);
  kl_handle::GraphKey key{(alts ? 3 : 2) + 2 * layout, B, T, flags, h->precision, states, status, ws, bits, layout};
  KL_TRY(run_graphed(h, key, s, [&]() {
    const int V = h->cfg.voc_size;
    KL_TRY(layout ? window_logits_training(h, B, T, w.s_idx, w.s_ctx, states, w, s)
                  : window_logits(h, B, T, w.s_idx, w.s_ctx, states, w, s));
    if (alts) KL_TRY(kl_launch_rate_topk(w.logits, V, B * T, V, w.s_tgt, B, T, K, a.tprob, a.alt_id, a.alt_p, a.rank, s));
    else if (pick) KL_TRY(kl_launch_rate_pick(w.logits, V, B * T, V, w.s_tgt, B, T, a.tprob, s));
    if (bits) KL_TRY(kl_launch_rate_bits(a.tprob, w.s_tgt, B, T, bits, s));
    if (status) hipLaunchKernelGGL(scan_status_kernel, dim3(1), dim3(64), 0, s, w.scan_status, status);
// ... 202 lines not shown
```

ocrd_keraslm_amd/csrc/elementwise.hip:

```cpp
#include <string.h>

#include "kl_common.h"
#include "kl_kernels.h"

namespace {

struct CtxTabs { const float* t[8]; };

__global__ void embed_gather_kernel(const float* __restrict__ E, CtxTabs tabs, int n_ctx, int ctx_dim, int W,
                                    const int* __restrict__ idx, const int* __restrict__ ctx, int B, int T,
                                    bf16_t* __restrict__ X, long ldx, int Dp) {
  const int chunks = Dp >> 3;
  const long total = (long)B * T * chunks;
  for (long e = blockIdx.x * (long)blockDim.x + threadIdx.x; e < total; e += (long)gridDim.x * blockDim.x) {
    const int c = (int)(e % chunks);
    const long row = e / chunks;
    const int b = (int)(row % B), t = (int)(row / B);
    const int id = idx[(long)b * T + t];
    frag16 o;
#pragma unroll
    for (int j = 0; j < 8; ++j) {
      const int d = c * 8 + j;
      float v = 0.f;
      if (d < W) {
        v = E[(long)id * W + d];
      } else if (d < W + n_ctx * ctx_dim) {
        const int n = (d - W) / ctx_dim, dd = (d - W) % ctx_dim;
        const int cid = ctx[((long)b * T + t) * n_ctx + n];
        v = tabs.t[n][(long)cid * ctx_dim + dd];
      }
      o.s[j] = f2bf(v);
    }
    *reinterpret_cast<uint4*>(X + row * ldx + c * 8) = o.u;
  }
}

__global__ void transpose_bf16_kernel(const bf16_t* __restrict__ in, long ld_in, bf16_t* __restrict__ out,
                                      long ld_out, int rows, int cols) {
  __shared__ bf16_t tile[64][66];
  const int r0 = blockIdx.y * 64, c0 = blockIdx.x * 64;
  const int tx = threadIdx.x & 63, ty = threadIdx.x >> 6;
  for (int i = ty; i < 64; i += 4) {
    const int r = r0 + i, c = c0 + tx;
    tile[i][tx] = (r < rows && c < cols) ? in[(long)r * ld_in + c] : (bf16_t)0;
  }
  __syncthreads();
  for (int i = ty; i < 64; i += 4) {
    const int c = c0 + i, r = r0 + tx;
    if (c < cols && r < rows) out[(long)c * ld_out + r] = tile[tx][i];
  }
}

__global__ void f32_to_bf16_kernel(const float* __restrict__ in, long ld_in, int rows, int cols,
                                   bf16_t* __restrict__ out_hi, bf16_t* __restrict__ out_lo, long ld_out,
                                   int transpose) {
  __shared__ float tile[64][65];
  const int r0 = blockIdx.y * 64, c0 = blockIdx.x * 64;
  const int tx = threadIdx.x & 63, ty = threadIdx.x >> 6;
  for (int i = ty; i < 64; i += 4) {
    const int r = r0 + i, c = c0 + tx;
    tile[i][tx] = (r < rows && c < cols) ? in[(long)r * ld_in + c] : 0.f;
  }
  __syncthreads();
  for (int i = ty; i < 64; i += 4) {
    int orow, ocol;
    float v;
    if (transpose) {
      orow = c0 + i; ocol = r0 + tx; v = tile[tx][i];
      if (orow >= cols || ocol >= rows) continue;
    } else {
      orow = r0 + i; ocol = c0 + tx; v = tile[i][tx];
      if (orow >= rows || ocol >= cols) continue;
    }
    bf16_t hi, lo;
    split_bf16(v, hi, lo);
    out_hi[(long)orow * ld_out + ocol] = hi;
    if (out_lo) out_lo[(long)orow * ld_out + ocol] = lo;
  }
}

__global__ void f32_to_bf16_jobs_kernel(const KlConvJobs jobs) {
  __shared__ float tile[64][65];
  const KlConvJob __attribute__((address_space(4)))* jp =
      (const KlConvJob __attribute__((address_space(4)))*)__builtin_amdgcn_kernarg_segment_ptr() + blockIdx.z;
  const float* in = jp->in;
  const long ld_in = jp->ld_in, ld_out = jp->ld_out;
  const int rows = jp->rows, cols = jp->cols, rows_pad = jp->rows_pad, transpose = jp->transpose;
  bf16_t* out_hi = jp->out_hi;
  bf16_t* out_lo = jp->out_lo;
  const int r0 = blockIdx.y * 64, c0 = blockIdx.x * 64;
  if (r0 >= rows_pad || c0 >= cols) return;
  const int tx = threadIdx.x & 63, ty = threadIdx.x >> 6;
  for (int i = ty; i < 64; i += 4) {
    const int r = r0 + i, c = c0 + tx;
    tile[i][tx] = (r < rows && c < cols) ? in[(long)r * ld_in + c] : 0.f;
  }
  __syncthreads();
  for (int i = ty; i < 64; i += 4) {
    int orow, ocol;
    float v;
    if (transpose) {
      orow = c0 + i; ocol = r0 + tx; v = tile[tx][i];
      if (orow >= cols || ocol >= rows_pad) continue;
    } else {
      orow = r0 + i; ocol = c0 + tx; v = tile[i][tx];
      if (orow >= rows_pad || ocol >= cols) continue;
    }
    bf16_t hi, lo;
    split_bf16(v, hi, lo);
    out_hi[(long)orow * ld_out + ocol] = hi;
    if (out_lo) out_lo[(long)orow * ld_out + ocol] = lo;
  }
}

__global__ void softmax_ce_kernel(float* __restrict__ logits, long ld, int rows, int V, const int* __restrict__ tgt,
                                  int B, int T, float inv_count, bf16_t* __restrict__ dlogits, long ld_dl,
                                  float* __restrict__ rowstat, int time_major, int last_only) {
  const int lane = threadIdx.x & 63;
  const int row = blockIdx.x * (blockDim.x >> 6) + (threadIdx.x >> 6);
  if (row >= rows) return;
  float* x = logits + (long)row * ld;
  float mx = -INFINITY;
  int amax = 0;
  for (int v = lane; v < V; v += 64) {
    const float a = x[v];
    if (a > mx) { mx = a; amax = v; }
  }
#pragma unroll
  for (int off = 32; off > 0; off >>= 1) {
    const float o = __shfl_xor(mx, off);
    const int oi = __shfl_xor(amax, off);
    if (o > mx || (o == mx && oi < amax)) { mx = o; amax = oi; }
  }
  float sum = 0.f;
  for (int v = lane; v < V; v += 64) sum += expf(x[v] - mx);
#pragma unroll
  for (int off = 32; off > 0; off >>= 1) sum += __shfl_xor(sum, off);
  const float inv = 1.f / sum;
  int t = -2;
  bool counts = true;
  if (tgt) {
    const int b = time_major ? row % B : row / T;
    const int tt = time_major ? row / B : row % T;
    t = tgt[(long)b * T + tt];
    if (last_only && tt != T - 1) { t = -1; counts = false; }
    if (t < -1) { t = -1; counts = false; }
  }
  const bool keep_probs = dlogits == nullptr;
  float pt = 0.f;
  for (int v = lane; v < V; v += 64) {
    const float p = expf(x[v] - mx) * inv;
    if (keep_probs) x[v] = p;
    if (v == t) pt = p;
  }
  if (!tgt) return;
#pragma unroll
  for (int off = 32; off > 0; off >>= 1) pt += __shfl_xor(pt, off);
  const bool valid = t >= 0;
  const bool active = valid && pt >= 1e-7f && pt <= 1.f - 1e-7f;
  if (dlogits) {
    bf16_t* d = dlogits + (long)row * ld_dl;
    for (int v = lane; v < ld_dl; v += 64) {
      float g = (active && v < V) ? expf(x[v] - mx) * inv : 0.f;
      if (active && v == t) g -= 1.f;
      d[v] = f2bf(g * inv_count);
    }
  }
  if (lane == 0 && rowstat) {
    float l = 0.f;
    if (valid) {
      const float pc = fminf(fmaxf(pt, 1e-7f), 1.f - 1e-7f);
      l = -logf(pc) * inv_count;
    }
    const int tsafe = valid ? t : 0;
    rowstat[2 * (long)row] = l;
    rowstat[2 * (long)row + 1] = (counts && amax == tsafe) ? inv_count : 0.f;
  }
}

__global__ void softmax_ce_v256_kernel(float* __restrict__ logits, long ld, int rows, int V, const int* __restrict__ tgt,
                                       int B, int T, float inv_count, bf16_t* __restrict__ dlogits, long ld_dl,
                                       float* __restrict__ rowstat, int time_major, int last_only) {
  const int lane = threadIdx.x & 63;
  const int row = blockIdx.x * (blockDim.x >> 6) + (threadIdx.x >> 6);
  if (row >= rows) return;
  float* x = logits + (long)row * ld;
// ... 107 lines not shown
}

__global__ void onehot_dense_kernel(const int* __restrict__ ids, int B, int T, int n_rows, int col, int n_cols,
                                    bf16_t* __restrict__ out, long ld) {
  const long r0 = ((long)blockIdx.x * blockDim.x + threadIdx.x) * 8;
  if (r0 >= ld) return;
  const long total = (long)B * T;
  int id[8];
#pragma unroll
  for (int j = 0; j < 8; ++j) {
    const long r = r0 + j;
    id[j] = -1;
    if (r < total) {
      const int b = (int)(r % B), t = (int)(r / B);
      id[j] = ids[((long)b * T + t) * n_cols + col];
    }
  }
  const int v0 = blockIdx.y * 32;
  for (int v = v0; v < v0 + 32 && v < n_rows; ++v) {
    uint4 w;
    w.x = (id[0] == v ? 0x3F80u : 0u) | (id[1] == v ? 0x3F800000u : 0u);
    w.y = (id[2] == v ? 0x3F80u : 0u) | (id[3] == v ? 0x3F800000u : 0u);
    w.z = (id[4] == v ? 0x3F80u : 0u) | (id[5] == v ? 0x3F800000u : 0u);
    w.w = (id[6] == v ? 0x3F80u : 0u) | (id[7] == v ? 0x3F800000u : 0u);
    *reinterpret_cast<uint4*>(out + (long)v * ld + r0) = w;
  }
}

__global__ void reg_stats_kernel(const float* __restrict__ X, int R, int D, float* __restrict__ scratch) {
  extern __shared__ float sm[];
  float* col = sm;
  float* red = sm + D;
  const int tid = threadIdx.x, nt = blockDim.x;
  float* mean = scratch;
  float* s1 = scratch + D;
  float* s2 = scratch + 2 * D;
  float* nr = scratch + 3 * D;
  for (int d = tid; d < D; d += nt) col[d] = 0.f;
  __syncthreads();
  if (D <= nt) {
    const int ng = nt / D, g = tid / D, d = tid % D;
    if (g < ng) {
      float a = 0.f;
#pragma unroll 8
      for (int r = 1 + g; r < R; r += ng) a += X[(long)r * D + d];
      atomicAdd(&col[d], a);
    }
  } else {
    for (int d = tid; d < D; d += nt) {
      float a = 0.f;
#pragma unroll 8
      for (int r = 1; r < R; ++r) a += X[(long)r * D + d];
      col[d] = a;
    }
  }
  float n1 = 0.f, n2 = 0.f;
  for (int r = tid >> 6; r < R; r += nt >> 6) {
    float a = 0.f;
    for (int d = tid & 63; d < D; d += 64) { const float x = X[(long)r * D + d]; a += x * x; }
#pragma unroll
    for (int off = 32; off > 0; off >>= 1) a += __shfl_xor(a, off);
    if ((tid & 63) == 0) {
      nr[r] = a;
      if (r >= 1) { n1 += a; n2 += a * a; }
    }
  }
  __syncthreads();
  for (int d = tid; d < D; d += nt) {
    const float a = col[d];
    mean[d] = a / (float)(R - 1);
    s1[d] = a - X[(long)(R - 1) * D + d];
    s2[d] = a - X[(long)1 * D + d];
  }
  red[tid] = n1;
  red[nt + tid] = n2;
  __syncthreads();
  for (int s = nt >> 1; s > 0; s >>= 1) {
    if (tid < s) { red[tid] += red[tid + s]; red[nt + tid] += red[nt + tid + s]; }
    __syncthreads();
  }
  if (tid == 0) { scratch[3 * D + R] = red[0]; scratch[3 * D + R + 1] = red[nt]; }
}

__global__ void reg_apply_kernel(const float* __restrict__ X, int R, int D, float* __restrict__ gX, int mode,
                                 const float* __restrict__ scratch, float* __restrict__ loss_acc) {
  __shared__ float red[256];
  const float* mean = scratch;
  const float* s1 = scratch + D;
  const float* s2 = scratch + 2 * D;
  const float* nr = scratch + 3 * D;
  const float N1 = scratch[3 * D + R], N2 = scratch[3 * D + R + 1];
  const float c_low = mode == 0 ? 0.01f : 0.02f;
  const float Rp = (float)(R - 1);
  float loss = 0.f;
  const long total = (long)R * D;
  for (long e = blockIdx.x * (long)blockDim.x + threadIdx.x; e < total; e += (long)gridDim.x * blockDim.x) {
    const int r = (int)(e / D), d = (int)(e % D);
    const float x = X[e];
    const float q = 1.f - nr[r];
    float g = -4.f * c_low * q * x;
    if (d == 0) loss += c_low * q * q;
    if (mode == 0) {
      if (r == 0) { const float u = x - mean[d]; g += 2.f * u; loss += u * u; }
    } else {
      if (r >= 2) g += 0.2f * s1[d];
      if (r == 0) {
        const float md = mean[d];
        g += 4.f * (Rp * x - N1 * md);
        loss += 0.2f * s1[d] * s2[d] + 2.f * (Rp * x * x - 2.f * x * md * N1 + md * md * N2);
      }
    }
    gX[e] += g;
  }
  red[threadIdx.x] = loss;
  __syncthreads();
  for (int s = blockDim.x >> 1; s > 0; s >>= 1) {
    if (threadIdx.x < s) red[threadIdx.x] += red[threadIdx.x + s];
    __syncthreads();
  }
  if (threadIdx.x == 0 && loss_acc) atomicAdd(loss_acc + 2, red[0]);
}

__global__ void state_to_rows_kernel(const float* __restrict__ states, int B, int W, int L, int layer,
                                     bf16_t* __restrict__ h_bf16, float* __restrict__ h_f32,
                                     float* __restrict__ c_f32) {
  const long total = (long)B * W;
  for (long e = blockIdx.x * (long)blockDim.x + threadIdx.x; e < total; e += (long)gridDim.x * blockDim.x) {
    const int b = (int)(e / W), u = (int)(e % W);
    const float* s = states + ((long)b * 2 * L + 2 * layer) * W;
    if (h_bf16) h_bf16[e] = f2bf(s[u]);
    if (h_f32) h_f32[e] = s[u];
    if (c_f32) c_f32[e] = s[W + u];
  }
}

__global__ void fill_f32_kernel(float* p, size_t n, float v) {
  for (size_t i = blockIdx.x * (size_t)blockDim.x + threadIdx.x; i < n; i += (size_t)gridDim.x * blockDim.x) p[i] = v;
}

inline int grid_for(long total, int block) {
  long g = (total + block - 1) / block;
  if (g > 2048) g = 2048;
  if (g < 1) g = 1;
  return (int)g;
}
inline int ok() { return hipGetLastError() == hipSuccess ? 0 : KL_ERR_LAUNCH; }

}

int kl_launch_embed_gather(const float* E, const float* const* ctx_tabs, int n_ctx, int ctx_dim, int W,
                           const int* idx, const int* ctx, int B, int T, bf16_t* X, long ldx, int Dp,
                           hipStream_t stream) {
  if (n_ctx > 8 || (Dp & 7) || (ldx & 7)) return KL_ERR_SHAPE;
  CtxTabs tabs;
  for (int i = 0; i < 8; ++i) tabs.t[i] = i < n_ctx ? ctx_tabs[i] : nullptr;
  const long total = (long)B * T * (Dp >> 3);
  hipLaunchKernelGGL(embed_gather_kernel, dim3(grid_for(total, 256)), dim3(256), 0, stream, E, tabs, n_ctx, ctx_dim,
                     W, idx, ctx, B, T, X, ldx, Dp);
  return ok();
}

int kl_launch_transpose_bf16(const bf16_t* in, long ld_in, bf16_t* out, long ld_out, int rows, int cols,
                             hipStream_t stream) {
  dim3 grid((cols + 63) / 64, (rows + 63) / 64);
  hipLaunchKernelGGL(transpose_bf16_kernel, grid, dim3(256), 0, stream, in, ld_in, out, ld_out, rows, cols);
  return ok();
}

int kl_launch_f32_to_bf16_t(const float* in, long ld_in, int rows, int cols, bf16_t* out_hi, bf16_t* out_lo,
                            long ld_out, int transpose, hipStream_t stream) {
  dim3 grid((cols + 63) / 64, (rows + 63) / 64);
  hipLaunchKernelGGL(f32_to_bf16_kernel, grid, dim3(256), 0, stream, in, ld_in, rows, cols, out_hi, out_lo, ld_out,
                     transpose);
  return ok();
}

int kl_launch_f32_to_bf16_jobs(const KlConvJob* jobs, int n, hipStream_t stream) {
  if (n < 1 || n > KL_CONV_MAX_JOBS) return KL_ERR_SHAPE;
  KlConvJobs all;
  memset(&all, 0, sizeof(all));
  int gx = 1, gy = 1;
  for (int j = 0; j < n; ++j) {
    all.job[j] = jobs[j];
    if (all.job[j].rows_pad < all.job[j].rows) all.job[j].rows_pad = all.job[j].rows;
    gx = max(gx, (jobs[j].cols + 63) / 64);
    gy = max(gy, (all.job[j].rows_pad + 63) / 64);
  }
  hipLaunchKernelGGL(f32_to_bf16_jobs_kernel, dim3(gx, gy, n), dim3(256), 0, stream, all);
  return ok();
}

__global__ void comb_table_kernel(const float* __restrict__ A, const float* __restrict__ B, int R2, int N8, bf16_t* __restrict__ out, long total) {
  for (long e = blockIdx.x * (long)blockDim.x + threadIdx.x; e < total; e += (long)gridDim.x * blockDim.x) {
    const int j = (int)(e % N8);
    const long row = e / N8;
    const int c = (int)(row % R2), v = (int)(row / R2);
    const float4* pa = reinterpret_cast<const float4*>(A + ((long)v * N8 + j) * 8);
    const float4* pb = reinterpret_cast<const float4*>(B + ((long)c * N8 + j) * 8);
    const float4 a0 = pa[0], a1 = pa[1], b0 = pb[0], b1 = pb[1];
    uint4 o;
    o.x = (unsigned)f2bf(a0.x + b0.x) | ((unsigned)f2bf(a0.y + b0.y) << 16);
    o.y = (unsigned)f2bf(a0.z + b0.z) | ((unsigned)f2bf(a0.w + b0.w) << 16);
    o.z = (unsigned)f2bf(a1.x + b1.x) | ((unsigned)f2bf(a1.y + b1.y) << 16);
// ... 97 lines not shown

int kl_launch_state_to_rows(const float* states, int B, int W, int L, int layer, bf16_t* h_bf16, float* h_f32,
                            float* c_f32, hipStream_t stream) {
  hipLaunchKernelGGL(state_to_rows_kernel, dim3(grid_for((long)B * W, 256)), dim3(256), 0, stream, states, B, W, L,
                     layer, h_bf16, h_f32, c_f32);
  return ok();
}

int kl_launch_fill_f32(float* p, size_t n, float v, hipStream_t stream) {
  hipLaunchKernelGGL(fill_f32_kernel, dim3(grid_for((long)n, 256)), dim3(256), 0, stream, p, n, v);
  return ok();
}

namespace {
__global__ void zero_kernel(uint4* p16, size_t n16, unsigned* tail, size_t ntail) {
  for (size_t i = blockIdx.x * (size_t)blockDim.x + threadIdx.x; i < n16; i += (size_t)gridDim.x * blockDim.x)
    p16[i] = uint4{0, 0, 0, 0};
  if (blockIdx.x == 0 && threadIdx.x < ntail) tail[threadIdx.x] = 0;
}
__global__ void zero_coherent_kernel(unsigned* p, size_t n) {
  for (size_t i = blockIdx.x * (size_t)blockDim.x + threadIdx.x; i < n; i += (size_t)gridDim.x * blockDim.x)
    __hip_atomic_store(p + i, 0u, __ATOMIC_RELAXED, __HIP_MEMORY_SCOPE_AGENT);
}
}

int kl_zero_async(void* p, size_t bytes, hipStream_t stream) {
  if (bytes == 0) return 0;
  if ((reinterpret_cast<uintptr_t>(p) & 3) || (bytes & 3)) return KL_ERR_ARG;
  uintptr_t a = reinterpret_cast<uintptr_t>(p);
  size_t head = ((16 - (a & 15)) & 15);
  if (head > bytes) head = bytes;
  unsigned* hp = reinterpret_cast<unsigned*>(p);
  size_t nhead = head / 4;
  uint4* body = reinterpret_cast<uint4*>(a + head);
  size_t n16 = (bytes - head) / 16;
  unsigned* tp = reinterpret_cast<unsigned*>(a + head + n16 * 16);
  size_t ntail = (bytes - head - n16 * 16) / 4;
  if (nhead) hipLaunchKernelGGL(zero_kernel, dim3(1), dim3(64), 0, stream, (uint4*)nullptr, (size_t)0, hp, nhead);
  long g = (long)((n16 + 255) / 256);
  if (g > 2048) g = 2048;
  if (g < 1) g = 1;
  hipLaunchKernelGGL(zero_kernel, dim3((unsigned)g), dim3(256), 0, stream, body, n16, tp, ntail);
  return ok();
}

namespace {
__global__ void fill16_kernel(uint4* p, size_t n16, unsigned v) {
  for (size_t i = blockIdx.x * (size_t)blockDim.x + threadIdx.x; i < n16; i += (size_t)gridDim.x * blockDim.x)
    p[i] = uint4{v, v, v, v};
}
}

int kl_fill_u32_async(void* p, size_t bytes, unsigned value, hipStream_t stream) {
  if (bytes == 0) return 0;
  if ((reinterpret_cast<uintptr_t>(p) & 15) || (bytes & 15)) return KL_ERR_ARG;
  const size_t n16 = bytes / 16;
  long g = (long)((n16 + 255) / 256);
  if (g > 4096) g = 4096;
  hipLaunchKernelGGL(fill16_kernel, dim3((unsigned)g), dim3(256), 0, stream, reinterpret_cast<uint4*>(p), n16, value);
  return ok();
}

int kl_zero_coherent_async(unsigned* p, size_t n_words, hipStream_t stream) {
  if (n_words == 0) return 0;
  long g = (long)((n_words + 255) / 256);
  if (g > 1024) g = 1024;
  hipLaunchKernelGGL(zero_coherent_kernel, dim3((unsigned)g), dim3(256), 0, stream, p, n_words);
  return ok();
}

namespace {
__global__ void fill_bf16_kernel(bf16_t* p, size_t n, bf16_t v) {
  for (size_t i = blockIdx.x * (size_t)blockDim.x + threadIdx.x; i < n; i += (size_t)gridDim.x * blockDim.x) p[i] = v;
}
}

int kl_launch_fill_bf16(bf16_t* p, size_t n, unsigned short bits, hipStream_t stream) {
  long g = (long)((n + 255) / 256);
  if (g > 1024) g = 1024;
  if (g < 1) g = 1;
  hipLaunchKernelGGL(fill_bf16_kernel, dim3((unsigned)g), dim3(256), 0, stream, p, n, (bf16_t)bits);
  return ok();
}
```

ocrd_keraslm_amd/csrc/kl_kernels.h:

```cpp
#pragma once
#include <hip/hip_runtime.h>
#include <stdint.h>

#include "keraslm_hip.h"

typedef unsigned short bf16_t;

#include <atomic>
#include <mutex>
#define KL_MAX_DEVICES 64
struct KlLdsGrant {
  std::atomic<size_t> granted[KL_MAX_DEVICES];
  std::mutex slow;
};
static inline int kl_grant_lds(KlLdsGrant& g, const void* fn, size_t lds) {
  int dev = 0;
  if (hipGetDevice(&dev) != hipSuccess) return KL_ERR_LAUNCH;
  if (dev < 0 || dev >= KL_MAX_DEVICES)
    return hipFuncSetAttribute(fn, hipFuncAttributeMaxDynamicSharedMemorySize, (int)lds) == hipSuccess ? 0 : KL_ERR_LAUNCH;
  if (lds <= g.granted[dev].load(std::memory_order_acquire)) return 0;
  std::lock_guard<std::mutex> lock(g.slow);
  if (lds <= g.granted[dev].load(std::memory_order_relaxed)) return 0;
  if (hipFuncSetAttribute(fn, hipFuncAttributeMaxDynamicSharedMemorySize, (int)lds) != hipSuccess) return KL_ERR_LAUNCH;
  g.granted[dev].store(lds, std::memory_order_release);
// ... 138 lines not shown
  bf16_t* HdT; long ldt_d;
  unsigned* counters;
  unsigned* status;
  int sentinel;
  unsigned* xcc_slots; unsigned gen;
  const int* ids_tm;
  int V, ctx_vocab;
  int pf_mode;
  bf16_t* Cb;
  int p_bf16;
  const bf16_t* KT; const bf16_t* X;
};
bool kl_scan_w128_applicable(int B, int T, int W);
int kl_launch_scan_fwd_w128(KlScanFwdWide args, hipStream_t stream);
int kl_scan_w128_tables_max_ctx();
bool kl_scan_w128_multi_fits(int B, int L);
int kl_launch_scan_fwd_w128_multi(const KlScanFwdWide* layers, int L, hipStream_t stream);
bool kl_scan_fwd_wide_applicable(int B, int T, int W);
int kl_launch_scan_fwd_wide(KlScanFwdWide args, hipStream_t stream);
int kl_scan_wide2_phases(int B, int T, int W, int rows, int max_np);
int kl_launch_scan_fwd_wide2(KlScanFwdWide args, int rows, hipStream_t stream);
int kl_launch_scan_fwd8(KlScanFwdWide args, hipStream_t stream, bool lockstep = false);
int kl_launch_permute_gate_cols_f32(const float* in, const float* bias, float* out, long rows, int W, hipStream_t stream);
int kl_launch_permute_gate_rows_bf16(const bf16_t* in, bf16_t* out, int W, int K, hipStream_t stream);
int kl_launch_p_gather_il(const float* EKp, const float* const* CtxKp, int n_ctx, const int* idx, const int* ctx, int B, int T, int W,
                          int V, int ctx_vocab, bf16_t* out, hipStream_t stream);
int kl_launch_ids_tm(const int* idx, const int* ctx, int n_ctx, int B, int T, int W, int V, int ctx_vocab, int* out,
                     hipStream_t stream);

struct KlScanBwd {
  int B, T, W, L;
  int n_rb, n_rg;
  const bf16_t* Un[KL_SCAN_MAXL];
  const bf16_t* Kn[KL_SCAN_MAXL];
  const bf16_t* G[KL_SCAN_MAXL];
  const float* C[KL_SCAN_MAXL];
  bf16_t* dZ[KL_SCAN_MAXL];
  const float* dH;
  const float* mask[KL_SCAN_MAXL];
  unsigned* counters;
  unsigned* status;
  bf16_t* dZT; long ldt;
  float* db;
  float* db_l[KL_SCAN_MAXL];
  int sentinel;
  unsigned* xcc_slots; unsigned gen;
  int pf_mode;
  const bf16_t* dHb;
  const bf16_t* Cb;
  unsigned* flags; const unsigned* epoch;
};
int kl_launch_scan_epoch(unsigned* flags, int n_flags, unsigned* epoch, unsigned step, hipStream_t stream);
int kl_launch_scan_bwd(KlScanBwd args, hipStream_t stream);
bool kl_scan_bwd_wide_applicable(int B, int T, int W);
int kl_scan_wide_blocks_per_wg(int B, int W);
int kl_launch_scan_bwd_wide(KlScanBwd args, hipStream_t stream);
int kl_launch_scan_bwd_wide2(KlScanBwd args, hipStream_t stream);
int kl_launch_scan_bwd_regtile(KlScanBwd args, hipStream_t stream);
int kl_launch_scan_bwd_w32(KlScanBwd args, hipStream_t stream);
int kl_launch_scan_bwd_w128(KlScanBwd args, hipStream_t stream);
int kl_launch_scan_bwd_w128_multi(KlScanBwd args, hipStream_t stream);
int kl_scan_bwd_regtile_min_np();
int kl_launch_logits_ce_ws(const bf16_t* X, const bf16_t* E, const int* tgt, bf16_t* dlogits, float* rowstat, int B, int T, int W,
                           int V, long ld_dl, float inv_count, int last_only, hipStream_t stream);
int kl_launch_dh_ws(const bf16_t* dlogits, const bf16_t* ET, bf16_t* dH, long M, int W, int Vp, hipStream_t stream);
int kl_launch_logits_ce_w128(const bf16_t* X, const bf16_t* E, const bf16_t* ET, const int* tgt, bf16_t* dlogits, float* dH, float* rowstat, int B,
                             int T, int W, int V, int Vp, float inv_count, int last_only, hipStream_t stream);
int kl_launch_rowstat_reduce(const float* rowstat, int rows, float* loss_acc, hipStream_t stream);
int kl_launch_proj_ws(const bf16_t* X, const bf16_t* KTp, const float* bp, bf16_t* P, long M, int W, unsigned* status,
                      hipStream_t stream);

int kl_launch_thin_gemm(const KlOperand* op, int M, int N, float* C, long ldc, const float* bias, int split,
                        hipStream_t stream);

int kl_launch_embed_gather(const float* E, const float* const* ctx_tabs, int n_ctx, int ctx_dim, int W,
                           const int* idx, const int* ctx, int B, int T, bf16_t* X, long ldx, int Dp,
                           hipStream_t stream);
int kl_launch_transpose_bf16(const bf16_t* in, long ld_in, bf16_t* out, long ld_out, int rows, int cols,
                             hipStream_t stream);
#define KL_CONV_MAX_JOBS 24
struct KlConvJob {
  const float* in; long ld_in; int rows, cols, rows_pad, transpose;
  bf16_t* out_hi; bf16_t* out_lo; long ld_out;
};
struct KlConvJobs { KlConvJob job[KL_CONV_MAX_JOBS]; };
int kl_launch_f32_to_bf16_jobs(const KlConvJob* jobs, int n, hipStream_t stream);
int kl_launch_comb_table(const float* A, const float* B, int R1, int R2, int N, bf16_t* out, hipStream_t stream);
int kl_launch_rows_tm(const int* idx, const int* ctx, int n_ctx, int Bn, int T, int V, int R2, int* out, hipStream_t stream);
int kl_launch_f32_to_bf16_t(const float* in, long ld_in, int rows, int cols, bf16_t* out_hi, bf16_t* out_lo,
                            long ld_out, int transpose, hipStream_t stream);
int kl_launch_softmax_ce(float* logits, long ld, int rows, int V, const int* tgt, int B, int T, float inv_count,
                         bf16_t* dlogits, long ld_dl, float* loss_acc, float* rowstat, int time_major,
                         hipStream_t stream, int last_only = 0);
int kl_launch_adam(float* p, const float* g, float* m, float* v, size_t n, float lr_t, float b1, float b2,
                   float eps, float clip, float grad_scale, hipStream_t stream);
int kl_launch_onehot_t(const int* ids, int B, int T, int n_classes, int col, int n_cols, bf16_t* out, long ld,
                       hipStream_t stream);
int kl_launch_onehot_dense(const int* ids, int B, int T, int n_rows, int col, int n_cols, bf16_t* out, long ld,
                           hipStream_t stream);
int kl_launch_regulariser_grads(const float* E, int V, int W, const float* const* ctx_tabs, int n_ctx, int ctx_vocab,
                                int ctx_dim, float* gE, float* const* gCtx, float* loss_acc, float* scratch,
                                hipStream_t stream);
int kl_launch_state_to_rows(const float* states, int B, int W, int L, int layer, bf16_t* h_bf16, float* h_f32,
                            float* c_f32, hipStream_t stream);
int kl_launch_fill_f32(float* p, size_t n, float v, hipStream_t stream);
int kl_launch_fill_bf16(bf16_t* p, size_t n, unsigned short bits, hipStream_t stream);
int kl_zero_async(void* p, size_t bytes, hipStream_t stream);
int kl_fill_u32_async(void* p, size_t bytes, unsigned value, hipStream_t stream);
int kl_zero_coherent_async(unsigned* p, size_t n_words, hipStream_t stream);

int kl_launch_small_table(const float* A, int R, int D, const float* Kmat, long ldk, int N, float* C, long ldc,
                          hipStream_t stream);
int kl_launch_p1_gather(const float* EK, const float* const* ctxk, int n_ctx, const float* bias, const int* idx,
                        const int* ctx, int B, int T, int N, float* P, hipStream_t stream);
int kl_launch_colsum_bf16(const bf16_t* in, long ld, int rows, int cols, float* out, hipStream_t stream);
int kl_launch_rows_to_state(const void* h_rows, int h_is_f32, const float* c_rows, int B, int W, int L, int layer,
                            float* states, hipStream_t stream);
int kl_launch_ctx_grads(const float* Ctx, const float* K0rows, long ldk, int R, int D, const float* dT, long ldt, int N,
                        float* gK, long ldg, float* gCtx, hipStream_t stream, long ldr = 1);
int kl_launch_rows_tm_to_bm(const float* in, long ld_in, float* out, int B, int T, int V, hipStream_t stream);

#define KL_SEGSUM_MAX_BUCKETS 65535
int kl_segment_sums_buckets(int n_ctx, int V, int R);
int kl_segment_sums_share(long BT);
size_t kl_segment_sums_ws_bytes(int B, int T, int n_ctx, int V, int R);
int kl_launch_segment_sums(const bf16_t* dZ, long ld, int B, int T, int cols, const int* idx, const int* ctx, int n_ctx, int V, int R,
                           float* dEK, float* dCtxK, void* ws, hipStream_t stream);

int kl_launch_rate_pick(const float* logits, long ld, int rows, int V, const int* tgt, int B, int T, float* tprob,
                        hipStream_t stream);
int kl_launch_rate_bits(const float* tprob, const int* tgt, int B, int T, double* bits, hipStream_t stream);

int kl_launch_rate_topk(const float* logits, long ld, int rows, int V, const int* tgt, int B, int T, int K, float* tprob,
                        int* alt_id, float* alt_p, int* rank, hipStream_t stream);

#define KL_SMALL_STEP_N 16
struct KlIncCellArgs {
  int n, W, split;
  float* pool; long slot_ld;
  const int* slot_in; const int* slot_out;
  int h_off, c_off, x_off;
  const bf16_t* UF; const bf16_t* KF;
  const float* T1; const int* i1; const float* T2; const int* i2; const float* bias;
};
#define KL_HOST_STEP_MAX 256
struct KlHostIdx {
  int slot_in[KL_HOST_STEP_MAX];
  int slot_out[KL_HOST_STEP_MAX];
  unsigned short idx[KL_HOST_STEP_MAX];
  unsigned short ctx[KL_HOST_STEP_MAX];
};
struct KlHostTargets { unsigned short t[KL_HOST_STEP_MAX]; };
struct KlStepFinish {
  int n, V, W;
  const float* logits; long ld;
  int softmax, by_target, head_k;
  const int* target;
  const float* pool; long slot_ld; const int* slot_out;
  float* probs_host; float* heads_host; unsigned* done_host; unsigned ticket;
  unsigned* counter;
};
int kl_launch_step_finish(const KlStepFinish& a, const KlHostTargets* tx, hipStream_t stream);
int kl_launch_inc_cell(const KlIncCellArgs& a, hipStream_t stream, const KlHostIdx* hx = nullptr, int* slots_copy = nullptr);
struct KlIncCellPlan { int nmt, gen; size_t lds; };
int kl_plan_inc_cell(int n, int W, bool has_x, bool host_idx, KlIncCellPlan* out);

struct KlWalkOut {
  int total, n, V, W, lo, head_k;
  const float* pool; long slot_ld; int h_off;
  const bf16_t* EF;
  const int* slots; const int* targets; const int* last;
  float* tprob_host; float* heads_host; unsigned* done_host; unsigned ticket;
  unsigned* counter;
};
int kl_launch_walk_out(const KlWalkOut& a, hipStream_t stream);

#define KL_BEAM_MAX_ROWS 256
#define KL_BEAM_MAX_FAN 16
struct KlBeamExpand {
  int rows, fan, V; float floor;
  const float* probs;
  const unsigned char* valid;
  const float* cum_in;
  const int* slot_new; int zero_slot;
  int* idx_next; int* slot_in_next; float* cum_next;
  int* parent_log; int* idx_log; float* cum_log; int* n_live;
  unsigned long long* keys; int* cand;
};
size_t kl_beam_ws_bytes(int rows, int fan);
int kl_launch_beam_expand(KlBeamExpand a, void* ws, hipStream_t stream);

#define KL_SAMPLE_MAX_ROWS 1024
#define KL_SAMPLE_MAX_TOPK 64
struct KlSamplePick {
  int rows, V, top_k; float temperature, floor;
  unsigned key0, key1, step, row0;
  const float* probs;
  const unsigned char* valid;
  const float* cum_in;
  int* idx_next; float* cum_next; float* u_log;
  float* w;
};
size_t kl_sample_ws_bytes(int rows, int V);
int kl_launch_sample_pick(KlSamplePick a, void* ws, hipStream_t stream);

int kl_launch_inc_tile(const KlIncCellArgs& a, int variant, hipStream_t stream, int rows = -1);
struct KlIncTilePlan { int rows, nx, ny, px, py; };
int kl_plan_inc_tile(int n, int W, int rows, KlIncTilePlan* out);
int kl_launch_out_softmax(const float* pool, long slot_ld, const int* slot_out, int h_off, const bf16_t* EF, int split,
                          int n, int W, int V, float* probs, long ldp, hipStream_t stream);
// ... 10 lines not shown
```

ocrd_keraslm_amd/csrc/segsum.hip:

```cpp
#include "kl_common.h"
#include "kl_kernels.h"
#include "keraslm_hip.h"

namespace {

constexpr int SEG_SLAB = 512;
constexpr int SEG_UNROLL = 8;
constexpr int SEG_SCAN_THREADS = 1024;
constexpr int SEG_SCAN_Q = 16;

typedef __attribute__((ext_vector_type(4))) unsigned u32x4;

__host__ __device__ inline long seg_pad(long n) { return (n + 63) & ~63L; }

__device__ __forceinline__ void seg_key(const int* __restrict__ idx, const int* __restrict__ ctx, int n_ctx, long src, int V, int R,
                                        int& bucket, unsigned& packed) {
  const int v = idx[src];
  const int vv = (v >= 0 && v < V) ? v : V;
  int cc = R;
  if (n_ctx > 0) {
    const int c = ctx[src * n_ctx];
    if (c >= 0 && c < R) cc = c;
  }
  bucket = vv * (R + 1) + cc;
// ... 115 lines not shown
  __builtin_amdgcn_wave_barrier();
#pragma unroll
  for (int i = 0; i < 8; ++i) {
    const int col = col_base + i * 64 + lane;
    if (col < cols) unsafeAtomicAdd(row + col, v[i]);
  }
}

__global__ __launch_bounds__(256) void segsum_gather_kernel(const bf16_t* __restrict__ dZ, long ld, int BT, int cols, int n_slabs, int share,
                                                            const int* __restrict__ order, const unsigned* __restrict__ skey, int V,
                                                            int R, float* __restrict__ dEK, float* __restrict__ dCtxK) {
  __shared__ __attribute__((aligned(16))) float strips[4][SEG_SLAB];
  const int wave = __builtin_amdgcn_readfirstlane(threadIdx.x >> 6), lane = threadIdx.x & 63;
  const unsigned unit = blockIdx.x * 4u + (unsigned)wave;
  const int slab = (int)(unit % (unsigned)n_slabs);
  const long p0 = (long)(unit / (unsigned)n_slabs) * share;
  if (p0 >= BT) return;
  const long p1 = p0 + share < BT ? p0 + share : BT;
  float* strip = strips[wave];
  const int col_base = slab * SEG_SLAB, col0 = col_base + lane * 8;
  const bool act = col0 < cols;
  const bf16_t* src = dZ + (act ? col0 : col_base);

  uint4 a[SEG_UNROLL];
  unsigned ka[SEG_UNROLL];
  auto fetch = [&](long p) {
#pragma unroll
    for (int j = 0; j < SEG_UNROLL; ++j) {
      const long q = p + j < p1 ? p + j : p1 - 1;
      const unsigned r = (unsigned)order[q];
      ka[j] = skey[q];
      const u32x4 t = __builtin_nontemporal_load(reinterpret_cast<const u32x4*>(src + (size_t)r * (size_t)ld));
      a[j] = uint4{t.x, t.y, t.z, t.w};
    }
  };

  float run[8], chr[8];
#pragma unroll
  for (int i = 0; i < 8; ++i) run[i] = chr[i] = 0.f;
  unsigned cur = skey[p0];
  auto close_run = [&](unsigned next, bool last) {
    const unsigned c = cur & 0xffffu, v = cur >> 16;
    if (c < (unsigned)R) seg_flush(strip, run, dCtxK + (size_t)c * cols, col_base, cols);
#pragma unroll
    for (int i = 0; i < 8; ++i) { chr[i] += run[i]; run[i] = 0.f; }
    if (last || (next >> 16) != v) {
      if (v < (unsigned)V) seg_flush(strip, chr, dEK + (size_t)v * cols, col_base, cols);
#pragma unroll
      for (int i = 0; i < 8; ++i) chr[i] = 0.f;
    }
    cur = next;
  };

  for (long p = p0; p < p1; p += SEG_UNROLL) {
    fetch(p);
#pragma unroll
    for (int j = 0; j < SEG_UNROLL; ++j) {
      if (p + j < p1) {
        if (ka[j] != cur) close_run(ka[j], false);
        seg_add_row(run, a[j]);
      }
    }
  }
  close_run(cur, true);
}

inline int ok() { return hipGetLastError() == hipSuccess ? 0 : KL_ERR_LAUNCH; }

}

int kl_segment_sums_buckets(int n_ctx, int V, int R) { return (V + 1) * ((n_ctx > 0 ? R : 0) + 1); }

int kl_segment_sums_share(long BT) {
  long s = (BT + 2047) / 2048;
  s = (s + SEG_UNROLL - 1) / SEG_UNROLL * SEG_UNROLL;
  return (int)(s > 256 ? 256 : s);
}

size_t kl_segment_sums_ws_bytes(int B, int T, int n_ctx, int V, int R) {
  const long BT = (long)B * T;
  return (size_t)(seg_pad(kl_segment_sums_buckets(n_ctx, V, R) + 1) + 2 * seg_pad(BT)) * sizeof(int);
}

int kl_launch_segment_sums(const bf16_t* dZ, long ld, int B, int T, int cols, const int* idx, const int* ctx, int n_ctx, int V, int R,
                           float* dEK, float* dCtxK, void* ws, hipStream_t stream) {
  const long BT = (long)B * T;
  if (B < 1 || T < 1 || BT > 0x7fffffffL || V < 1 || n_ctx < 0 || (n_ctx > 0 && R < 1)) return KL_ERR_SHAPE;
  if (n_ctx == 0) R = 0;
  if ((cols & 7) || cols < 8 || (ld & 7) || ld < cols) return KL_ERR_SHAPE;
  if ((long)(V + 1) * (R + 1) > KL_SEGSUM_MAX_BUCKETS) return KL_ERR_SHAPE;
  if (!dZ || !idx || !dEK || !ws || (n_ctx > 0 && (!ctx || !dCtxK))) return KL_ERR_ARG;
  if (((size_t)dZ & 15) || ((size_t)dEK & 15) || ((size_t)dCtxK & 15) || ((size_t)ws & 15)) return KL_ERR_ARG;
  const long nbp = seg_pad((long)(V + 1) * (R + 1) + 1);
  int* offs = reinterpret_cast<int*>(ws);
  int* order = offs + nbp;
  unsigned* skey = reinterpret_cast<unsigned*>(order + seg_pad(BT));

  const size_t n_a = (size_t)nbp / 4, n_b = (size_t)V * cols / 4, n_c = (size_t)R * cols / 4;
  size_t g = (n_a + n_b + n_c + 255) / 256;
  if (g > 1024) g = 1024;
  hipLaunchKernelGGL(segsum_init_kernel, dim3((unsigned)g), dim3(256), 0, stream, reinterpret_cast<uint4*>(offs), n_a,
                     reinterpret_cast<uint4*>(dEK), n_b, reinterpret_cast<uint4*>(dCtxK), n_c);
  const unsigned gr = (unsigned)((BT + 255) / 256);
  hipLaunchKernelGGL(segsum_hist_kernel, dim3(gr), dim3(256), 0, stream, idx, ctx, n_ctx, B, T, V, R, offs);
  const int n4 = (int)(nbp / 4), per4 = (n4 + SEG_SCAN_THREADS - 1) / SEG_SCAN_THREADS;
  hipLaunchKernelGGL(segsum_scan_kernel, dim3(1), dim3(SEG_SCAN_THREADS), 0, stream, reinterpret_cast<int4*>(offs), n4, per4);
  hipLaunchKernelGGL(segsum_scatter_kernel, dim3(gr), dim3(256), 0, stream, idx, ctx, n_ctx, B, T, V, R, offs, order, skey);
  const int n_slabs = (cols + SEG_SLAB - 1) / SEG_SLAB, share = kl_segment_sums_share(BT);
  const long units = (BT + share - 1) / share * n_slabs;
  hipLaunchKernelGGL(segsum_gather_kernel, dim3((unsigned)((units + 3) / 4)), dim3(256), 0, stream, dZ, ld, (int)BT, cols, n_slabs, share,
                     order, skey, V, R, dEK, dCtxK);
  return ok();
}
```

ocrd_keraslm_amd/csrc/tables.hip:

```cpp
#include "kl_common.h"
#include "kl_kernels.h"

namespace {

__global__ void small_table_kernel(const float* __restrict__ A, int R, int D, const float* __restrict__ Kmat,
                                   long ldk, int N, float* __restrict__ C, long ldc) {
  const long total = (long)R * N;
  for (long e = blockIdx.x * (long)blockDim.x + threadIdx.x; e < total; e += (long)gridDim.x * blockDim.x) {
    const int r = (int)(e / N), n = (int)(e % N);
    float a = 0.f;
    for (int k = 0; k < D; ++k) a = fmaf(A[(long)r * D + k], Kmat[(long)k * ldk + n], a);
    C[(long)r * ldc + n] = a;
  }
}

struct Tabs { const float* t[8]; };

__global__ void p1_gather_kernel(const float* __restrict__ EK, Tabs ctxk, int n_ctx, const float* __restrict__ bias,
                                 const int* __restrict__ idx, const int* __restrict__ ctx, int B, int T, int N4,
                                 float* __restrict__ P) {
  const long total = (long)B * T * N4;
  for (long e = blockIdx.x * (long)blockDim.x + threadIdx.x; e < total; e += (long)gridDim.x * blockDim.x) {
    const int c = (int)(e % N4);
    const long row = e / N4;
    const int b = (int)(row % B), t = (int)(row / B);
    const long src = (long)b * T + t;
    float4 v = reinterpret_cast<const float4*>(EK)[(long)idx[src] * N4 + c];
    const float4 bb = reinterpret_cast<const float4*>(bias)[c];
    v.x += bb.x; v.y += bb.y; v.z += bb.z; v.w += bb.w;
    for (int n = 0; n < n_ctx; ++n) {
      const float4 q = reinterpret_cast<const float4*>(ctxk.t[n])[(long)ctx[src * n_ctx + n] * N4 + c];
      v.x += q.x; v.y += q.y; v.z += q.z; v.w += q.w;
    }
    reinterpret_cast<float4*>(P)[row * N4 + c] = v;
  }
}

__global__ void colsum_bf16_kernel(const bf16_t* __restrict__ in, long ld, int rows, int cols, float* __restrict__ out) {
  __shared__ float red[4][64];
  const int tx = threadIdx.x & 63, ty = threadIdx.x >> 6;
  const int col = blockIdx.x * 64 + tx;
  const int rchunk = (rows + gridDim.y - 1) / gridDim.y;
  const int rb = blockIdx.y * rchunk, re = min(rows, rb + rchunk);
  float a = 0.f;
  if (col < cols)
    for (int r = rb + ty; r < re; r += 4) a += bf2f(in[(long)r * ld + col]);
  red[ty][tx] = a;
  __syncthreads();
  if (ty == 0 && col < cols) atomicAdd(out + col, red[0][tx] + red[1][tx] + red[2][tx] + red[3][tx]);
}

__global__ void rows_to_state_kernel(const void* __restrict__ h_rows, int h_is_f32, const float* __restrict__ c_rows,
                                     int B, int W, int L, int layer, float* __restrict__ states) {
  const long total = (long)B * W;
  for (long e = blockIdx.x * (long)blockDim.x + threadIdx.x; e < total; e += (long)gridDim.x * blockDim.x) {
    const int b = (int)(e / W), u = (int)(e % W);
    float* s = states + ((long)b * 2 * L + 2 * layer) * W;
    s[u] = h_is_f32 ? reinterpret_cast<const float*>(h_rows)[e] : bf2f(reinterpret_cast<const bf16_t*>(h_rows)[e]);
    s[W + u] = c_rows[e];
  }
}

__global__ void ctx_grad_k_kernel(const float* __restrict__ Ctx, int R, int D, const float* __restrict__ dT, long ldt, long ldr,
                                  int N, float* __restrict__ gK, long ldg) {
  const long total = (long)D * N;
  for (long e = blockIdx.x * (long)blockDim.x + threadIdx.x; e < total; e += (long)gridDim.x * blockDim.x) {
    const int d = (int)(e / N), col = (int)(e % N);
    float a = 0.f;
    for (int r = 0; r < R; ++r) a = fmaf(Ctx[(long)r * D + d], dT[(long)col * ldt + r * ldr], a);
    gK[(long)d * ldg + col] += a;
  }
}
__global__ void ctx_grad_c_kernel(const float* __restrict__ Krows, long ldk, int R, int D, const float* __restrict__ dT,
                                  long ldt, long ldr, int N, float* __restrict__ gCtx) {
  const int lane = threadIdx.x & 63;
  const long item = blockIdx.x * (long)(blockDim.x >> 6) + (threadIdx.x >> 6);
  if (item >= (long)R * D) return;
  const int r = (int)(item / D), d = (int)(item % D);
  float a = 0.f;
  for (int col = lane; col < N; col += 64) a = fmaf(dT[(long)col * ldt + r * ldr], Krows[(long)d * ldk + col], a);
#pragma unroll
  for (int off = 32; off > 0; off >>= 1) a += __shfl_xor(a, off);
  if (lane == 0) gCtx[(long)r * D + d] += a;
}

__global__ void rows_tm_to_bm_kernel(const float* __restrict__ in, long ld_in, float* __restrict__ out, int B, int T,
                                     int V) {
  const long total = (long)B * T * V;
  for (long e = blockIdx.x * (long)blockDim.x + threadIdx.x; e < total; e += (long)gridDim.x * blockDim.x) {
    const int v = (int)(e % V);
    const long row = e / V;
    const int b = (int)(row / T), t = (int)(row % T);
    out[e] = in[((long)t * B + b) * ld_in + v];
  }
}

inline int grid_for(long total, int block) {
  long g = (total + block - 1) / block;
  if (g > 4096) g = 4096;
  if (g < 1) g = 1;
  return (int)g;
}
inline int ok() { return hipGetLastError() == hipSuccess ? 0 : KL_ERR_LAUNCH; }

}

int kl_launch_small_table(const float* A, int R, int D, const float* Kmat, long ldk, int N, float* C, long ldc,
                          hipStream_t stream) {
  hipLaunchKernelGGL(small_table_kernel, dim3(grid_for((long)R * N, 256)), dim3(256), 0, stream, A, R, D, Kmat, ldk, N,
                     C, ldc);
  return ok();
}

int kl_launch_p1_gather(const float* EK, const float* const* ctxk, int n_ctx, const float* bias, const int* idx,
                        const int* ctx, int B, int T, int N, float* P, hipStream_t stream) {
  if (n_ctx > 8 || (N & 3)) return KL_ERR_SHAPE;
  Tabs tabs;
  for (int i = 0; i < 8; ++i) tabs.t[i] = i < n_ctx ? ctxk[i] : nullptr;
  hipLaunchKernelGGL(p1_gather_kernel, dim3(grid_for((long)B * T * (N / 4), 256)), dim3(256), 0, stream, EK, tabs,
                     n_ctx, bias, idx, ctx, B, T, N / 4, P);
  return ok();
}

int kl_launch_colsum_bf16(const bf16_t* in, long ld, int rows, int cols, float* out, hipStream_t stream) {
  int ry = (rows + 255) / 256;
  if (ry > 64) ry = 64;
  if (ry < 1) ry = 1;
  hipLaunchKernelGGL(colsum_bf16_kernel, dim3((cols + 63) / 64, ry), dim3(256), 0, stream, in, ld, rows, cols, out);
  return ok();
}

int kl_launch_rows_to_state(const void* h_rows, int h_is_f32, const float* c_rows, int B, int W, int L, int layer,
                            float* states, hipStream_t stream) {
  hipLaunchKernelGGL(rows_to_state_kernel, dim3(grid_for((long)B * W, 256)), dim3(256), 0, stream, h_rows, h_is_f32,
                     c_rows, B, W, L, layer, states);
  return ok();
}

int kl_launch_ctx_grads(const float* Ctx, const float* K0rows, long ldk, int R, int D, const float* dT, long ldt, int N,
                        float* gK, long ldg, float* gCtx, hipStream_t stream, long ldr) {
  hipLaunchKernelGGL(ctx_grad_k_kernel, dim3(grid_for((long)D * N, 256)), dim3(256), 0, stream, Ctx, R, D, dT, ldt, ldr, N,
                     gK, ldg);
  const long items = (long)R * D;
  hipLaunchKernelGGL(ctx_grad_c_kernel, dim3((unsigned)((items + 3) / 4)), dim3(256), 0, stream, K0rows, ldk, R, D, dT,
                     ldt, ldr, N, gCtx);
  return ok();
}

int kl_launch_rows_tm_to_bm(const float* in, long ld_in, float* out, int B, int T, int V, hipStream_t stream) {
  hipLaunchKernelGGL(rows_tm_to_bm_kernel, dim3(grid_for((long)B * T * V, 256)), dim3(256), 0, stream, in, ld_in, out,
                     B, T, V);
  return ok();
}
```

Baseline: 36.19 million chars/s.

## Fold small per-step launches into batched multi-job kernels behind KL_FOLD

Adds a default-on fold mode that merges many small kernel launches into fewer batched ones. It covers window-entry zeroing plus state-to-rows, rows-to-state for all layers, table and permute jobs in prepare, the paired bf16 conversions, and a combined ctx-grad kernel. It also folds the rowstat and regulariser reductions using counters and pre-zeroes the segsum buffers so their init kernel can be skipped. A split-K count is added for the dE gemm. The aim is to cut launch and graph-node overhead in a run of many small operations, at the cost of more complex code and new counter and workspace state.

```diff
diff --git a/ocrd_keraslm_amd/csrc/api.hip b/ocrd_keraslm_amd/csrc/api.hip
--- a/ocrd_keraslm_amd/csrc/api.hip
+++ b/ocrd_keraslm_amd/csrc/api.hip
@@ -31,6 +31,7 @@
 };
 
 constexpr int KL_SCAN_FLAGS = 256 * 64;
+constexpr int KL_STATUS_WORDS = 4 + 256, KL_FOLD_COUNTERS = 16, KL_FOLD_CNT_ROWSTAT = 12;
 struct Derived {
   std::vector<bf16_t*> UT_hi, UT_lo, KT_hi, KT_lo, Un, Kn;
   bf16_t *E_hi = nullptr, *E_lo = nullptr, *ET = nullptr;
@@ -62,6 +63,7 @@
   float *s_masks, *s_probs;
   unsigned *scan_cnt, *scan_status;
   float* reg_scratch;
+  float* fold_ws = nullptr;
   std::vector<bf16_t*> G, dZ, Hd;
   std::vector<bf16_t*> Cb;
   std::vector<bf16_t*> Xhi, Xlo;
@@ -155,6 +157,7 @@
   bool regtile = true;
   bool scan2_flags = true;
   bool flags_zeroed = false;
+  bool fold = true;
   struct ViewNote {
     int B, T;
     const void* ws;
@@ -333,7 +336,7 @@
   o.s_masks = cv.take<float>(training ? L * (size_t)B * W : 1);
   o.s_probs = cv.take<float>(BT * V);
   o.scan_cnt = cv.take<unsigned>(L * ((size_t)(B + 15) / 16) * T);
-  o.scan_status = cv.take<unsigned>(4 + 256);
+  o.scan_status = cv.take<unsigned>(KL_STATUS_WORDS + KL_FOLD_COUNTERS);
   o.reg_scratch = cv.take<float>(3 * (W > (size_t)c.ctx_dim ? W : (size_t)c.ctx_dim) + (V > (size_t)c.ctx_vocab ? V : (size_t)c.ctx_vocab) + 8);
   if (training) {
     o.G.assign(L, nullptr); o.dZ.assign(L, nullptr); o.Hd.assign(L, nullptr); o.Cb.assign(L, nullptr);
@@ -371,6 +374,7 @@
     o.dEKT = cv.take<float>(4 * W * Vp);
     o.dEKT_bf = cv.take<bf16_t>(4 * W * Vp);
     o.dEK_bf = cv.take<bf16_t>(Vp * 4 * W);
+    o.fold_ws = cv.take<float>(2 * KL_ROWSTAT_FOLD_MAX_BLOCKS + kl_regulariser_fold_floats((int)V, (int)W, c.n_ctx, c.ctx_vocab, c.ctx_dim));
   }
   return align_up(cv.off, 256);
 }
@@ -397,11 +401,12 @@
     }
   }
   const float* E = P + h->off_E;
+  const bool il = precision == KL_PREC_BF16 && h->scan2 && W == 512;
   {
     KlConvJob jobs[KL_CONV_MAX_JOBS];
     int nj = 0;
-    auto add = [&](const float* in, long ld_in, int rows, int cols, int rows_pad, bf16_t* hi, bf16_t* lo, long ld_out, int tr) -> int {
-      jobs[nj++] = KlConvJob{in, ld_in, rows, cols, rows_pad, tr, hi, lo, ld_out};
+    auto add = [&](const float* in, long ld_in, int rows, int cols, int rows_pad, bf16_t* hi, bf16_t* lo, long ld_out, int tr, int gate_w = 0) -> int {
+      jobs[nj++] = KlConvJob{in, ld_in, rows, cols, rows_pad, tr, hi, lo, ld_out, gate_w};
       if (nj < KL_CONV_MAX_JOBS) return 0;
       nj = 0;
       return kl_launch_f32_to_bf16_jobs(jobs, KL_CONV_MAX_JOBS, s);
@@ -413,6 +418,7 @@
       KL_TRY(add(K, 4 * W, W, 4 * W, W, d.KT_hi[l], split ? d.KT_lo[l] : nullptr, W, 1));
       KL_TRY(add(U, 4 * W, W, 4 * W, W, d.Un[l], nullptr, 4 * W, 0));
       KL_TRY(add(K, 4 * W, W, 4 * W, W, d.Kn[l], nullptr, 4 * W, 0));
+      if (h->fold && il && l > 0) KL_TRY(add(K, 4 * W, W, 4 * W, W, d.KTp[l], nullptr, W, 1, W));
     }
     KL_TRY(add(E, W, V, W, Vp, d.E_hi, split ? d.E_lo : nullptr, W, 0));
     KL_TRY(add(E, W, V, W, Vp, d.ET, nullptr, Vp, 1));
@@ -423,19 +429,32 @@
   op.A = E; op.lda = W; op.a_is_f32 = 1;
   op.WT_hi = d.KT_hi[0]; op.WT_lo = split ? d.KT_lo[0] : nullptr; op.ldw = W; op.K = W;
   KL_TRY(kl_launch_thin_gemm(&op, V, 4 * W, d.EK, 4 * W, nullptr, precision, s));
-  for (int n = 0; n < c.n_ctx; ++n) {
-    const float* Kc = P + h->off_K[0] + (size_t)(W + n * c.ctx_dim) * 4 * W;
-    KL_TRY(kl_launch_small_table(P + h->off_Ctx[n], c.ctx_vocab, c.ctx_dim, Kc, 4 * W, 4 * W, d.CtxK[n], 4 * W, s));
-  }
-  h->il_ready = precision == KL_PREC_BF16 && h->scan2 && W == 512;
+  h->il_ready = il;
   h->comb_ready = false;
-  if (h->il_ready) {
-    for (int l = 1; l < c.depth; ++l) {
-      KL_TRY(kl_launch_permute_gate_rows_bf16(d.KT_hi[l], d.KTp[l], W, W, s));
-      KL_TRY(kl_launch_permute_gate_cols_f32(P + h->off_b[l], nullptr, d.bp[l], 1, W, s));
-    }
-    KL_TRY(kl_launch_permute_gate_cols_f32(d.EK, P + h->off_b[0], d.EKp, V, W, s));
-    for (int n = 0; n < c.n_ctx; ++n) KL_TRY(kl_launch_permute_gate_cols_f32(d.CtxK[n], nullptr, d.CtxKp[n], c.ctx_vocab, W, s));
+  if (h->fold && 1 + c.depth + c.n_ctx <= KL_TABLE_MAX_JOBS) {
+    KlTableJob tj[KL_TABLE_MAX_JOBS];
+    int nt = 0;
+    for (int n = 0; n < c.n_ctx; ++n)
+      tj[nt++] = KlTableJob{1, c.ctx_vocab, c.ctx_dim, W, P + h->off_Ctx[n], P + h->off_K[0] + (size_t)(W + n * c.ctx_dim) * 4 * W, 4 * W, d.CtxK[n],
+                            il ? d.CtxKp[n] : nullptr};
+    if (il) {
+      for (int l = 1; l < c.depth; ++l) tj[nt++] = KlTableJob{0, 1, 0, W, P + h->off_b[l], nullptr, 0, nullptr, d.bp[l]};
+      tj[nt++] = KlTableJob{0, V, 0, W, d.EK, P + h->off_b[0], 0, nullptr, d.EKp};
+    }
+    if (nt > 0) KL_TRY(kl_launch_table_jobs(tj, nt, s));
+  } else {
+    for (int n = 0; n < c.n_ctx; ++n) {
+      const float* Kc = P + h->off_K[0] + (size_t)(W + n * c.ctx_dim) * 4 * W;
+      KL_TRY(kl_launch_small_table(P + h->off_Ctx[n], c.ctx_vocab, c.ctx_dim, Kc, 4 * W, 4 * W, d.CtxK[n], 4 * W, s));
+    }
+    if (il) {
+      for (int l = 1; l < c.depth; ++l) {
+        KL_TRY(kl_launch_permute_gate_rows_bf16(d.KT_hi[l], d.KTp[l], W, W, s));
+        KL_TRY(kl_launch_permute_gate_cols_f32(P + h->off_b[l], nullptr, d.bp[l], 1, W, s));
+      }
+      KL_TRY(kl_launch_permute_gate_cols_f32(d.EK, P + h->off_b[0], d.EKp, V, W, s));
+      for (int n = 0; n < c.n_ctx; ++n) KL_TRY(kl_launch_permute_gate_cols_f32(d.CtxK[n], nullptr, d.CtxKp[n], c.ctx_vocab, W, s));
+    }
   }
   h->precision = precision;
   h->inc_ready = false;
@@ -885,11 +904,22 @@
 }
 
 int forward_impl(kl_handle* h, int B, int T, const int* idx, const int* ctx, float* states, const float* masks,
-                 int training, WindowWs& w, hipStream_t s) {
+                 int training, WindowWs& w, hipStream_t s, const KlWindowEntry& zeros) {
   const int W = h->cfg.width, L = h->cfg.depth;
   const FwdCall c = {h, B, T, idx, ctx, states, masks, training, training ? 1 : h->precision, w, s, W, L, (size_t)B * W, (B + 15) / 16};
-  for (int l = 0; l < L; ++l)
-    KL_TRY(kl_launch_state_to_rows(states, B, W, L, l, training ? (bf16_t*)w.H[l] : nullptr, training ? nullptr : (float*)w.H[l], w.C[l], s));
+  if (h->fold) {
+    KlWindowEntry e = zeros;
+    e.states = states; e.B = B; e.W = W; e.L = L;
+    for (int l = 0; l < L; ++l) {
+      e.h_bf16[l] = training ? (bf16_t*)w.H[l] : nullptr; e.h_f32[l] = training ? nullptr : (float*)w.H[l]; e.c_f32[l] = w.C[l];
+    }
+    KL_TRY(kl_launch_window_entry(e, s));
+  } else {
+    for (int j = 0; j < KL_ENTRY_MAX_ZERO; ++j)
+      if (zeros.zero[j]) KL_TRY(kl_zero_async(zeros.zero[j], zeros.zero_bytes[j], s));
+    for (int l = 0; l < L; ++l)
+      KL_TRY(kl_launch_state_to_rows(states, B, W, L, l, training ? (bf16_t*)w.H[l] : nullptr, training ? nullptr : (float*)w.H[l], w.C[l], s));
+  }
   int e = fwd_wide(c);
   if (e == FWD_PASS && !fwd_w128_tables(c)) KL_TRY(gather_layer0(c));
   if (e == FWD_PASS) e = fwd_w128(c);
@@ -900,6 +930,11 @@
   if (e == FWD_PASS) e = fwd_fused_thin(c);
   if (e == FWD_PASS) e = fwd_wavefront(c);
   KL_TRY(e);
+  if (h->fold) {
+    const void* hr[KL_ENTRY_MAX_LAYERS]; const float* cr[KL_ENTRY_MAX_LAYERS];
+    for (int l = 0; l < L; ++l) { hr[l] = h_rows(c, l, T); cr[l] = w.C[l] + (size_t)T * c.BW; }
+    return kl_launch_rows_to_state_all(hr, training ? 0 : 1, cr, B, W, L, states, s);
+  }
   for (int l = 0; l < L; ++l)
     KL_TRY(kl_launch_rows_to_state(h_rows(c, l, T), training ? 0 : 1, w.C[l] + (size_t)T * c.BW, B, W, L, l, states, s));
   return 0;
@@ -1016,6 +1051,8 @@
   h->drop_graphs();
   const char* env = getenv("KL_GRAPH");
   h->graphs_enabled = !(env && env[0] == '0');
+  const char* envf = getenv("KL_FOLD");
+  h->fold = !(envf && envf[0] == '0');
   const char* env2 = getenv("KL_SCAN");
   h->scan_enabled = !(env2 && env2[0] == '0');
   const char* env3 = getenv("KL_SEQ_BWD");
@@ -1124,8 +1161,10 @@
 static int window_logits(kl_handle* h, int B, int T, const int32_t* idx, const int32_t* ctx, float* states, WindowWs& w,
                          hipStream_t s) {
   const int W = h->cfg.width, V = h->cfg.voc_size, L = h->cfg.depth;
-  KL_TRY(kl_zero_async(w.scan_status, (4 + 256) * sizeof(unsigned), s));
-  KL_TRY(forward_impl(h, B, T, idx, ctx, states, nullptr, 0, w, s));
+  KlWindowEntry zeros;
+  memset(&zeros, 0, sizeof(zeros));
+  zeros.zero[0] = w.scan_status; zeros.zero_bytes[0] = KL_STATUS_WORDS * sizeof(unsigned);
+  KL_TRY(forward_impl(h, B, T, idx, ctx, states, nullptr, 0, w, s, zeros));
   KlOperand op;
   memset(&op, 0, sizeof(op));
   op.A = (float*)w.H[L - 1] + (size_t)B * W; op.lda = W; op.a_is_f32 = 1;
@@ -1148,10 +1187,12 @@
 static int window_logits_training(kl_handle* h, int B, int T, const int32_t* idx, const int32_t* ctx, float* states, WindowWs& w,
                                   hipStream_t s) {
   const int W = h->cfg.width, V = h->cfg.voc_size, L = h->cfg.depth;
-  KL_TRY(kl_zero_async(w.scan_status, (4 + 256) * sizeof(unsigned), s));
+  KlWindowEntry zeros;
+  memset(&zeros, 0, sizeof(zeros));
+  zeros.zero[0] = w.scan_status; zeros.zero_bytes[0] = KL_STATUS_WORDS * sizeof(unsigned);
   w.km_plan = true;
   w.scan2_rows = plan_scan2(h, B, T, true, false);
-  KL_TRY(forward_impl(h, B, T, idx, ctx, states, nullptr, 1, w, s));
+  KL_TRY(forward_impl(h, B, T, idx, ctx, states, nullptr, 1, w, s, zeros));
   const bf16_t* Htop = (const bf16_t*)w.H[L - 1] + (size_t)B * W;
   return kl_launch_gemm_tn(Htop, h->d.E_hi, w.logits, nullptr, B * T, V, W, W, W, V, 0, 1, 1.f, s);
 }
@@ -1232,7 +1273,8 @@
   }
   if (fe != 0 && fe != KL_ERR_SHAPE) return fe;
   if (fe == 0) c.note.out_route |= dh_done ? KL_OUT_LOGITS_W128 : KL_OUT_LOGITS_WS;
-  if (fe == 0) KL_TRY(kl_launch_rowstat_reduce(w.rowstat, BT, c.loss_acc, s));
+  if (fe == 0) KL_TRY(h->fold ? kl_launch_rowstat_reduce_fold(w.rowstat, BT, c.loss_acc, w.fold_ws, w.scan_status + KL_STATUS_WORDS + KL_FOLD_CNT_ROWSTAT, s)
+                              : kl_launch_rowstat_reduce(w.rowstat, BT, c.loss_acc, s));
   else {
     KL_TRY(kl_launch_gemm_tn(top.km, d.E_hi, w.logits, nullptr, BT, V, W, W, W, V, 0, 1, 1.f, s));
     KL_TRY(kl_launch_softmax_ce(w.logits, V, BT, V, c.tgt, B, T, c.inv_count, w.dlogits, Vp, c.loss_acc, w.rowstat, 1, s, h->last_only));
@@ -1254,6 +1296,13 @@
   return rows_product(c, km_e, {w.dlogits, Vp, w.dlogitsT, BTp}, V, top, W, c.grads + h->off_E, W, false);
 }
 
+static int kl_table_de_splits(int V, int W) {
+  const int tiles = ((V + 63) / 64) * ((W + 127) / 128), most = 4 * W / 128;
+  int sp = (256 + tiles - 1) / tiles;
+  if (sp > most) sp = most;
+  return sp < 1 ? 1 : sp;
+}
+
 static int table_grads(const TrainCall& c) {
   kl_handle* h = c.h; WindowWs& w = c.w; const kl_config& cf = h->cfg; const Derived& d = h->d; hipStream_t s = c.s;
   const int B = c.B, T = c.T, W = c.W, V = c.V, Vp = c.Vp, BT = c.BT, BTp = c.BTp;
@@ -1262,9 +1311,14 @@
   bool pair_ctx = false;
   if (seg) {
     KL_TRY(kl_launch_segment_sums(w.dZ[0], 4 * W, B, T, 4 * W, c.idx, c.ctx, cf.n_ctx, Vp, cf.ctx_vocab, w.dEKT,
-                                  cf.n_ctx > 0 ? w.dCtxKT[0] : nullptr, w.seg_ws, s));
-    KL_TRY(kl_launch_f32_to_bf16_t(w.dEKT, 4 * W, Vp, 4 * W, w.dEKT_bf, nullptr, Vp, 1, s));
-    KL_TRY(kl_launch_f32_to_bf16_t(w.dEKT, 4 * W, Vp, 4 * W, w.dEK_bf, nullptr, 4 * W, 0, s));
+                                  cf.n_ctx > 0 ? w.dCtxKT[0] : nullptr, w.seg_ws, s,  h->fold));
+    if (h->fold) {
+      const KlConvJob two[2] = {{w.dEKT, 4 * W, Vp, 4 * W, Vp, 1, w.dEKT_bf, nullptr, Vp, 0}, {w.dEKT, 4 * W, Vp, 4 * W, Vp, 0, w.dEK_bf, nullptr, 4 * W, 0}};
+      KL_TRY(kl_launch_f32_to_bf16_jobs(two, 2, s));
+    } else {
+      KL_TRY(kl_launch_f32_to_bf16_t(w.dEKT, 4 * W, Vp, 4 * W, w.dEKT_bf, nullptr, Vp, 1, s));
+      KL_TRY(kl_launch_f32_to_bf16_t(w.dEKT, 4 * W, Vp, 4 * W, w.dEK_bf, nullptr, 4 * W, 0, s));
+    }
   } else {
     KL_TRY(onehot(c, c.idx, V, Vp, 0, 1, w.OHT, w.dEKT));
     pair_ctx = km && h->fuse_wg && cf.n_ctx >= 1 && (Vp % 128) == 0 && kl_gemm_an_applicable(4 * W, Vp + cf.ctx_vocab, BT, 4 * W);
@@ -1276,12 +1330,17 @@
       else KL_TRY(pe);
     }
     if (!pair_ctx) KL_TRY(rows_product(c, km, dz, 4 * W, {nullptr, 0, w.OHT, BTp}, Vp, w.dEKT, Vp, false));
-    KL_TRY(kl_launch_f32_to_bf16_t(w.dEKT, Vp, 4 * W, Vp, w.dEKT_bf, nullptr, Vp, 0, s));
-    KL_TRY(kl_launch_f32_to_bf16_t(w.dEKT, Vp, 4 * W, Vp, w.dEK_bf, nullptr, 4 * W, 1, s));
+    if (h->fold) {
+      const KlConvJob two[2] = {{w.dEKT, Vp, 4 * W, Vp, 4 * W, 0, w.dEKT_bf, nullptr, Vp, 0}, {w.dEKT, Vp, 4 * W, Vp, 4 * W, 1, w.dEK_bf, nullptr, 4 * W, 0}};
+      KL_TRY(kl_launch_f32_to_bf16_jobs(two, 2, s));
+    } else {
+      KL_TRY(kl_launch_f32_to_bf16_t(w.dEKT, Vp, 4 * W, Vp, w.dEKT_bf, nullptr, Vp, 0, s));
+      KL_TRY(kl_launch_f32_to_bf16_t(w.dEKT, Vp, 4 * W, Vp, w.dEK_bf, nullptr, 4 * W, 1, s));
+    }
   }
   c.note.wg_route |= (seg ? KL_WG_SEGSUM : 0) | (pair_ctx ? KL_WG_PAIR_CTX : 0);
   KL_TRY(kl_launch_gemm_tn(d.ET, w.dEKT_bf, c.grads + h->off_K[0], nullptr, W, 4 * W, Vp, Vp, Vp, 4 * W, 0, 1, 1.f, s));
-  KL_TRY(kl_launch_gemm_tn(w.dEK_bf, d.Kn[0], c.grads + h->off_E, nullptr, V, W, 4 * W, 4 * W, 4 * W, W, 2, 1, 1.f, s));
+  KL_TRY(kl_launch_gemm_tn(w.dEK_bf, d.Kn[0], c.grads + h->off_E, nullptr, V, W, 4 * W, 4 * W, 4 * W, W, 2, h->fold ? kl_table_de_splits(V, W) : 1, 1.f, s));
   for (int n = 0; n < cf.n_ctx; ++n) {
     const bool seg_n = seg && n == 0;
     if (!(pair_ctx && n == 0) && !seg_n) {
@@ -1289,9 +1348,16 @@
       KL_TRY(rows_product(c, km, dz, 4 * W, {nullptr, 0, w.OHC[n], BTp}, cf.ctx_vocab, w.dCtxKT[n], cf.ctx_vocab, false));
     }
     const size_t krow = (size_t)(W + n * cf.ctx_dim) * 4 * W;
-    KL_TRY(kl_launch_ctx_grads(h->params + h->off_Ctx[n], h->params + h->off_K[0] + krow, 4 * W, cf.ctx_vocab, cf.ctx_dim,
+    int ce = KL_ERR_SHAPE;
+    if (h->fold)
+      ce = kl_launch_ctx_grads_fold(h->params + h->off_Ctx[n], h->params + h->off_K[0] + krow, 4 * W, cf.ctx_vocab, cf.ctx_dim,
+                                    w.dCtxKT[n], seg_n ? 1 : cf.ctx_vocab, 4 * W, c.grads + h->off_K[0] + krow, 4 * W,
+                                    c.grads + h->off_Ctx[n], s, seg_n ? 4 * W : 1);
+    if (ce == KL_ERR_SHAPE)
+      ce = kl_launch_ctx_grads(h->params + h->off_Ctx[n], h->params + h->off_K[0] + krow, 4 * W, cf.ctx_vocab, cf.ctx_dim,
                                w.dCtxKT[n], seg_n ? 1 : cf.ctx_vocab, 4 * W, c.grads + h->off_K[0] + krow, 4 * W,
-                               c.grads + h->off_Ctx[n], s, seg_n ? 4 * W : 1));
+                               c.grads + h->off_Ctx[n], s, seg_n ? 4 * W : 1);
+    KL_TRY(ce);
   }
   return 0;
 }
@@ -1511,12 +1577,19 @@
   const int W = cf.width, V = cf.voc_size, Vp = h->Vp, L = cf.depth;
   const int BT = B * T, BTp = round_up_i(BT, 8);
   const float* P = h->params;
-  KL_TRY(kl_zero_async(grads, h->n_params * sizeof(float), s));
-  KL_TRY(kl_zero_async(w.scan_status, (4 + 256) * sizeof(unsigned), s));
+  KlWindowEntry zeros;
+  memset(&zeros, 0, sizeof(zeros));
+  zeros.zero[0] = grads; zeros.zero_bytes[0] = h->n_params * sizeof(float);
+  zeros.zero[1] = w.scan_status; zeros.zero_bytes[1] = (KL_STATUS_WORDS + KL_FOLD_COUNTERS) * sizeof(unsigned);
+  if (h->fold && w.segsum) {
+    zeros.zero[2] = w.seg_ws; zeros.zero_bytes[2] = kl_segment_sums_counter_bytes(cf.n_ctx, Vp, cf.ctx_vocab);
+    zeros.zero[3] = w.dEKT; zeros.zero_bytes[3] = (size_t)Vp * 4 * W * sizeof(float);
+    if (cf.n_ctx > 0) { zeros.zero[4] = w.dCtxKT[0]; zeros.zero_bytes[4] = (size_t)cf.ctx_vocab * 4 * W * sizeof(float); }
+  }
   w.km_plan = h->gemm_an && BTp == BT && kl_gemm_an_applicable(4 * W, W, BT, 4 * W);
   w.scan2_rows = plan_scan2(h, B, T, w.km_plan, true);
   w.scan2_bwd = w.scan2_rows != 0;
-  KL_TRY(forward_impl(h, B, T, idx, ctx, states, masks, 1, w, s));
+  KL_TRY(forward_impl(h, B, T, idx, ctx, states, masks, 1, w, s, zeros));
   const int n_rb_all = (B + 15) / 16, nug = W / 16;
   const bool thin_fits = (n_rb_all + 512 / nug - 1) / (512 / nug) <= (W == 1024 ? 8 : 4) &&
                          (long)T * B * 4 * W * 2 <= 0xfffffff0L;
@@ -1547,6 +1620,9 @@
   std::vector<const float*> ctabs(cf.n_ctx);
   std::vector<float*> gctabs(cf.n_ctx);
   for (int n = 0; n < cf.n_ctx; ++n) { ctabs[n] = P + h->off_Ctx[n]; gctabs[n] = grads + h->off_Ctx[n]; }
+  if (h->fold && loss_acc != nullptr)
+    return kl_launch_regulariser_grads_fold(P + h->off_E, V, W, ctabs.data(), cf.n_ctx, cf.ctx_vocab, cf.ctx_dim, grads + h->off_E, gctabs.data(),
+                                            loss_acc, w.fold_ws + 2 * KL_ROWSTAT_FOLD_MAX_BLOCKS, w.scan_status + KL_STATUS_WORDS, w.scan_status, s);
   KL_TRY(kl_launch_regulariser_grads(P + h->off_E, V, W, ctabs.data(), cf.n_ctx, cf.ctx_vocab, cf.ctx_dim,
                                      grads + h->off_E, gctabs.data(), loss_acc, w.reg_scratch, s));
   hipLaunchKernelGGL(scan_status_kernel, dim3(1), dim3(64), 0, s, w.scan_status, loss_acc);
@@ -2269,6 +2345,15 @@
 int stage_window(const kl_handle* h, const WindowWs& w, int B, int T, const int32_t* idx, const int32_t* ctx,
                  const int32_t* tgt, const float* masks, hipStream_t s) {
   const size_t BT = (size_t)B * T;
+  if (h->fold) {
+    KlCopyJob jobs[KL_COPY_MAX_JOBS];
+    int nj = 0;
+    jobs[nj++] = KlCopyJob{idx, w.s_idx, BT};
+    if (h->cfg.n_ctx > 0) jobs[nj++] = KlCopyJob{ctx, w.s_ctx, BT * h->cfg.n_ctx};
+    if (tgt) jobs[nj++] = KlCopyJob{tgt, w.s_tgt, BT};
+    if (masks) jobs[nj++] = KlCopyJob{masks, w.s_masks, (size_t)h->cfg.depth * B * h->cfg.width};
+    return kl_launch_copy_jobs(jobs, nj, s);
+  }
   KL_TRY(hip_ok(hipMemcpyAsync(w.s_idx, idx, BT * sizeof(int), hipMemcpyDeviceToDevice, s)));
   if (h->cfg.n_ctx > 0)
     KL_TRY(hip_ok(hipMemcpyAsync(w.s_ctx, ctx, BT * h->cfg.n_ctx * sizeof(int), hipMemcpyDeviceToDevice, s)));
diff --git a/ocrd_keraslm_amd/csrc/elementwise.hip b/ocrd_keraslm_amd/csrc/elementwise.hip
--- a/ocrd_keraslm_amd/csrc/elementwise.hip
+++ b/ocrd_keraslm_amd/csrc/elementwise.hip
@@ -88,6 +88,7 @@
   const int rows = jp->rows, cols = jp->cols, rows_pad = jp->rows_pad, transpose = jp->transpose;
   bf16_t* out_hi = jp->out_hi;
   bf16_t* out_lo = jp->out_lo;
+  const int gate_w = jp->gate_w;
   const int r0 = blockIdx.y * 64, c0 = blockIdx.x * 64;
   if (r0 >= rows_pad || c0 >= cols) return;
   const int tx = threadIdx.x & 63, ty = threadIdx.x >> 6;
@@ -102,6 +103,7 @@
     if (transpose) {
       orow = c0 + i; ocol = r0 + tx; v = tile[tx][i];
       if (orow >= cols || ocol >= rows_pad) continue;
+      if (gate_w) orow = (orow % gate_w) * 4 + orow / gate_w;
     } else {
       orow = r0 + i; ocol = c0 + tx; v = tile[i][tx];
       if (orow >= rows_pad || ocol >= cols) continue;
@@ -375,9 +377,9 @@
   if (tid == 0) { scratch[3 * D + R] = red[0]; scratch[3 * D + R + 1] = red[nt]; }
 }
 
-__global__ void reg_apply_kernel(const float* __restrict__ X, int R, int D, float* __restrict__ gX, int mode,
-                                 const float* __restrict__ scratch, float* __restrict__ loss_acc) {
-  __shared__ float red[256];
+__device__ __forceinline__ void reg_apply_body(const float* __restrict__ X, int R, int D, float* __restrict__ gX, int mode,
+                                               const float* __restrict__ scratch, float* __restrict__ loss_acc, unsigned bid, unsigned nb,
+                                               float* red) {
   const float* mean = scratch;
   const float* s1 = scratch + D;
   const float* s2 = scratch + 2 * D;
@@ -387,7 +389,7 @@
   const float Rp = (float)(R - 1);
   float loss = 0.f;
   const long total = (long)R * D;
-  for (long e = blockIdx.x * (long)blockDim.x + threadIdx.x; e < total; e += (long)gridDim.x * blockDim.x) {
+  for (long e = bid * (long)blockDim.x + threadIdx.x; e < total; e += (long)nb * blockDim.x) {
     const int r = (int)(e / D), d = (int)(e % D);
     const float x = X[e];
     const float q = 1.f - nr[r];
@@ -412,6 +414,12 @@
     __syncthreads();
   }
   if (threadIdx.x == 0 && loss_acc) atomicAdd(loss_acc + 2, red[0]);
+}
+
+__global__ void reg_apply_kernel(const float* __restrict__ X, int R, int D, float* __restrict__ gX, int mode,
+                                 const float* __restrict__ scratch, float* __restrict__ loss_acc) {
+  __shared__ float red[256];
+  reg_apply_body(X, R, D, gX, mode, scratch, loss_acc, blockIdx.x, gridDim.x, red);
 }
 
 __global__ void state_to_rows_kernel(const float* __restrict__ states, int B, int W, int L, int layer,
@@ -675,3 +683,253 @@
   hipLaunchKernelGGL(fill_bf16_kernel, dim3((unsigned)g), dim3(256), 0, stream, p, n, (bf16_t)bits);
   return ok();
 }
+
+namespace {
+
+#define KL_KERNARG(T) ((const T __attribute__((address_space(4)))*)__builtin_amdgcn_kernarg_segment_ptr())
+
+__device__ __forceinline__ bool fold_last_block(unsigned* counter, unsigned n, int* flag) {
+  asm volatile("s_waitcnt vmcnt(0)" ::: "memory");
+  __syncthreads();
+  if (threadIdx.x == 0) {
+    const unsigned got = __hip_atomic_fetch_add(counter, 1u, __ATOMIC_RELAXED, __HIP_MEMORY_SCOPE_AGENT);
+    *flag = got == n - 1u ? 1 : 0;
+    if (got == n - 1u) __hip_atomic_store(counter, 0u, __ATOMIC_RELAXED, __HIP_MEMORY_SCOPE_AGENT);
+  }
+  __syncthreads();
+  return *flag != 0;
+}
+__device__ __forceinline__ void fold_post(float* p, float v) { __hip_atomic_store(p, v, __ATOMIC_RELAXED, __HIP_MEMORY_SCOPE_AGENT); }
+__device__ __forceinline__ float fold_peek(const float* p) { return __hip_atomic_load(p, __ATOMIC_RELAXED, __HIP_MEMORY_SCOPE_AGENT); }
+
+__device__ __forceinline__ void fold_zero(void* p, size_t bytes, unsigned bid, unsigned nb) {
+  typedef __attribute__((ext_vector_type(4))) unsigned u32x4;
+  typedef __attribute__((address_space(1))) u32x4 g_uint4;
+  typedef __attribute__((address_space(1))) unsigned g_u32;
+  const uintptr_t a = reinterpret_cast<uintptr_t>(p);
+  size_t head = (16 - (a & 15)) & 15;
+  if (head > bytes) head = bytes;
+  const size_t n16 = (bytes - head) / 16, ntail = (bytes - head - n16 * 16) / 4;
+  g_uint4* body = (g_uint4*)(a + head);
+  const size_t i0 = bid * (size_t)blockDim.x + threadIdx.x, stride = (size_t)nb * blockDim.x;
+  for (size_t i = i0; i < n16; i += stride) body[i] = u32x4{0u, 0u, 0u, 0u};
+  if (bid == 0) {
+    if (threadIdx.x < head / 4) ((g_u32*)a)[threadIdx.x] = 0u;
+    if (threadIdx.x < ntail) ((g_u32*)(a + head + n16 * 16))[threadIdx.x] = 0u;
+  }
+}
+
+__global__ __launch_bounds__(256) void window_entry_kernel(const KlWindowEntry e) {
+  const int job = blockIdx.y;
+  if (job < KL_ENTRY_MAX_ZERO) {
+    void* p = KL_KERNARG(KlWindowEntry)->zero[job];
+    const size_t bytes = KL_KERNARG(KlWindowEntry)->zero_bytes[job];
+    if (p != nullptr && bytes != 0) fold_zero(p, bytes, blockIdx.x, gridDim.x);
+    return;
+  }
+  const int layer = job - KL_ENTRY_MAX_ZERO;
+  bf16_t* h_bf16 = KL_KERNARG(KlWindowEntry)->h_bf16[layer];
+  float* h_f32 = KL_KERNARG(KlWindowEntry)->h_f32[layer];
+  float* c_f32 = KL_KERNARG(KlWindowEntry)->c_f32[layer];
+  const int W = e.W, L = e.L;
+  const long total = (long)e.B * W;
+  for (long i = blockIdx.x * (long)blockDim.x + threadIdx.x; i < total; i += (long)gridDim.x * blockDim.x) {
+    const int b = (int)(i / W), u = (int)(i % W);
+    const float* s = e.states + ((long)b * 2 * L + 2 * layer) * W;
+    if (h_bf16) h_bf16[i] = f2bf(s[u]);
+    if (h_f32) h_f32[i] = s[u];
+    if (c_f32) c_f32[i] = s[W + u];
+  }
+}
+
+__global__ __launch_bounds__(256) void copy_jobs_kernel(const KlCopyJobs jobs) {
+  const KlCopyJob __attribute__((address_space(4)))* jp = &KL_KERNARG(KlCopyJobs)->job[blockIdx.y];
+  const unsigned* src = reinterpret_cast<const unsigned*>(jp->src);
+  unsigned* dst = reinterpret_cast<unsigned*>(jp->dst);
+  const size_t words = jp->words;
+  const size_t i0 = blockIdx.x * (size_t)blockDim.x + threadIdx.x, stride = (size_t)gridDim.x * blockDim.x;
+  if (((reinterpret_cast<uintptr_t>(src) | reinterpret_cast<uintptr_t>(dst)) & 15) == 0) {
+    const size_t n16 = words / 4;
+    for (size_t i = i0; i < n16; i += stride) reinterpret_cast<uint4*>(dst)[i] = reinterpret_cast<const uint4*>(src)[i];
+    for (size_t i = n16 * 4 + i0; i < words; i += stride) dst[i] = src[i];
+  } else {
+    for (size_t i = i0; i < words; i += stride) dst[i] = src[i];
+  }
+}
+
+__global__ __launch_bounds__(256) void rowstat_reduce_fold_kernel(const float* __restrict__ rowstat, int rows, float* part,
+                                                                  unsigned* counter, float* __restrict__ loss_acc) {
+  __shared__ float red[2][256];
+  __shared__ int flag;
+  const int tid = threadIdx.x;
+  float a = 0.f, b = 0.f;
+  for (int r = blockIdx.x * 256 + tid; r < rows; r += gridDim.x * 256) {
+    const float2 v = reinterpret_cast<const float2*>(rowstat)[r];
+    a += v.x;
+    b += v.y;
+  }
+  red[0][tid] = a;
+  red[1][tid] = b;
+  __syncthreads();
+  for (int s = 128; s > 0; s >>= 1) {
+    if (tid < s) { red[0][tid] += red[0][tid + s]; red[1][tid] += red[1][tid + s]; }
+    __syncthreads();
+  }
+  if (tid == 0) { fold_post(part + 2 * blockIdx.x, red[0][0]); fold_post(part + 2 * blockIdx.x + 1, red[1][0]); }
+  if (!fold_last_block(counter, gridDim.x, &flag)) return;
+  a = b = 0.f;
+  for (int i = tid; i < (int)gridDim.x; i += 256) { a += fold_peek(part + 2 * i); b += fold_peek(part + 2 * i + 1); }
+  red[0][tid] = a;
+  red[1][tid] = b;
+  __syncthreads();
+  for (int s = 128; s > 0; s >>= 1) {
+    if (tid < s) { red[0][tid] += red[0][tid + s]; red[1][tid] += red[1][tid + s]; }
+    __syncthreads();
+  }
+  if (tid == 0) { atomicAdd(loss_acc + 0, red[0][0]); atomicAdd(loss_acc + 1, red[1][0]); }
+}
+
+constexpr int REG_SLAB = 16;
+struct RegTable { const float* X; float* gX; float* scratch; float* part; int R, D, mode, n_slabs, n_apply, pad; };
+struct RegTables { RegTable t[KL_REG_MAX_TABLES]; };
+
+__global__ __launch_bounds__(256) void reg_stats_fold_kernel(const RegTables tabs, unsigned* counters) {
+  __shared__ float nrs[REG_SLAB];
+  __shared__ int flag;
+  const RegTable __attribute__((address_space(4)))* tp = &KL_KERNARG(RegTables)->t[blockIdx.y];
+  const int n_slabs = tp->n_slabs;
+  if ((int)blockIdx.x >= n_slabs) return;
+  const float* __restrict__ X = tp->X;
+  const int R = tp->R, D = tp->D;
+  float* scratch = tp->scratch;
+  float* part = tp->part;
+  const int tid = threadIdx.x, lane = tid & 63, wave = tid >> 6;
+  const int r0 = blockIdx.x * REG_SLAB, r1 = min(R, r0 + REG_SLAB), rs = max(r0, 1);
+  float* nr = scratch + 3 * D;
+  for (int r = r0 + wave; r < r1; r += 4) {
+    float a = 0.f;
+    for (int d = lane; d < D; d += 64) { const float x = X[(long)r * D + d]; a += x * x; }
+#pragma unroll
+    for (int off = 32; off > 0; off >>= 1) a += __shfl_xor(a, off);
+    if (lane == 0) { nr[r] = a; nrs[r - r0] = a; }
+  }
+  float* P = part + (long)blockIdx.x * (D + 2);
+  for (int d = tid; d < D; d += 256) {
+    float a = 0.f;
+    for (int r = rs; r < r1; ++r) a += X[(long)r * D + d];
+    fold_post(P + d, a);
+  }
+  __syncthreads();
+  if (tid == 0) {
+    float n1 = 0.f, n2 = 0.f;
+    for (int r = rs; r < r1; ++r) { const float a = nrs[r - r0]; n1 += a; n2 += a * a; }
+    fold_post(P + D, n1);
+    fold_post(P + D + 1, n2);
+  }
+  if (!fold_last_block(counters + blockIdx.y, (unsigned)n_slabs, &flag)) return;
+  for (int d = tid; d < D; d += 256) {
+    float a = 0.f;
+    for (int b = 0; b < n_slabs; ++b) a += fold_peek(part + (long)b * (D + 2) + d);
+    scratch[d] = a / (float)(R - 1);
+    scratch[D + d] = a - X[(long)(R - 1) * D + d];
+    scratch[2 * D + d] = a - X[(long)1 * D + d];
+  }
+  if (tid == 0) {
+    float n1 = 0.f, n2 = 0.f;
+    for (int b = 0; b < n_slabs; ++b) { n1 += fold_peek(part + (long)b * (D + 2) + D); n2 += fold_peek(part + (long)b * (D + 2) + D + 1); }
+    scratch[3 * D + R] = n1;
+    scratch[3 * D + R + 1] = n2;
+  }
+}
+
+__global__ __launch_bounds__(256) void reg_apply_fold_kernel(const RegTables tabs, float* __restrict__ loss_acc, const unsigned* __restrict__ status) {
+  __shared__ float red[256];
+  if (status != nullptr && blockIdx.x == 0 && blockIdx.y == 0 && threadIdx.x == 0 && (status[0] | status[1]) != 0) loss_acc[3] += 1.f;
+  const RegTable __attribute__((address_space(4)))* tp = &KL_KERNARG(RegTables)->t[blockIdx.y];
+  const int n_apply = tp->n_apply;
+  if ((int)blockIdx.x >= n_apply) return;
+  reg_apply_body(tp->X, tp->R, tp->D, tp->gX, tp->mode, tp->scratch, loss_acc, blockIdx.x, n_apply, red);
+}
+
+inline size_t reg_table_floats(int R, int D) { return (size_t)3 * D + R + 8 + (size_t)((R + REG_SLAB - 1) / REG_SLAB) * (D + 2); }
+
+}
+
+int kl_launch_window_entry(const KlWindowEntry& e, hipStream_t stream) {
+  if (e.L < 0 || e.L > KL_ENTRY_MAX_LAYERS) return KL_ERR_SHAPE;
+  for (int j = 0; j < KL_ENTRY_MAX_ZERO; ++j)
+    if (e.zero[j] != nullptr && ((reinterpret_cast<uintptr_t>(e.zero[j]) & 3) || (e.zero_bytes[j] & 3))) return KL_ERR_ARG;
+  size_t most = (size_t)e.B * e.W * 4;
+  for (int j = 0; j < KL_ENTRY_MAX_ZERO; ++j)
+    if (e.zero[j] != nullptr && e.zero_bytes[j] > most) most = e.zero_bytes[j];
+  long g = (long)((most / 16 + 255) / 256);
+  if (g > 1024) g = 1024;
+  if (g < 1) g = 1;
+  hipLaunchKernelGGL(window_entry_kernel, dim3((unsigned)g, KL_ENTRY_MAX_ZERO + e.L), dim3(256), 0, stream, e);
+  return ok();
+}
+
+int kl_launch_copy_jobs(const KlCopyJob* jobs, int n, hipStream_t stream) {
+  if (n < 1 || n > KL_COPY_MAX_JOBS) return KL_ERR_SHAPE;
+  KlCopyJobs all;
+  memset(&all, 0, sizeof(all));
+  size_t most = 0;
+  for (int j = 0; j < n; ++j) {
+    if ((reinterpret_cast<uintptr_t>(jobs[j].src) | reinterpret_cast<uintptr_t>(jobs[j].dst)) & 3) return KL_ERR_ARG;
+    all.job[j] = jobs[j];
+    if (jobs[j].words > most) most = jobs[j].words;
+  }
+  if (most == 0) return 0;
+  long g = (long)((most / 4 + 255) / 256);
+  if (g > 512) g = 512;
+  if (g < 1) g = 1;
+  hipLaunchKernelGGL(copy_jobs_kernel, dim3((unsigned)g, n), dim3(256), 0, stream, all);
+  return ok();
+}
+
+int kl_rowstat_fold_blocks(int rows) {
+  int nb = (rows + 1023) / 1024;
+  return nb > KL_ROWSTAT_FOLD_MAX_BLOCKS ? KL_ROWSTAT_FOLD_MAX_BLOCKS : (nb < 1 ? 1 : nb);
+}
+
+int kl_launch_rowstat_reduce_fold(const float* rowstat, int rows, float* loss_acc, float* part, unsigned* counter, hipStream_t stream) {
+  hipLaunchKernelGGL(rowstat_reduce_fold_kernel, dim3(kl_rowstat_fold_blocks(rows)), dim3(256), 0, stream, rowstat, rows, part, counter,
+                     loss_acc);
+  return ok();
+}
+
+size_t kl_regulariser_fold_floats(int V, int W, int n_ctx, int ctx_vocab, int ctx_dim) {
+  return reg_table_floats(V, W) + (size_t)(n_ctx > 0 ? n_ctx : 0) * reg_table_floats(ctx_vocab, ctx_dim);
+}
+
+int kl_regulariser_fold_slabs(int R) { return (R + REG_SLAB - 1) / REG_SLAB; }
+
+int kl_launch_regulariser_grads_fold(const float* E, int V, int W, const float* const* ctx_tabs, int n_ctx, int ctx_vocab, int ctx_dim,
+                                     float* gE, float* const* gCtx, float* loss_acc, float* fold_scratch, unsigned* counters,
+                                     const unsigned* status, hipStream_t stream) {
+  if (n_ctx < 0 || n_ctx + 1 > KL_REG_MAX_TABLES) return KL_ERR_SHAPE;
+  RegTables tabs;
+  memset(&tabs, 0, sizeof(tabs));
+  int nt = 0, max_slabs = 1, max_apply = 1;
+  float* ws = fold_scratch;
+  auto add = [&](const float* X, float* gX, int R, int D, int mode) {
+    RegTable& t = tabs.t[nt++];
+    t.X = X; t.gX = gX; t.R = R; t.D = D; t.mode = mode;
+    t.scratch = ws;
+    t.part = ws + (size_t)3 * D + R + 8;
+    ws += reg_table_floats(R, D);
+    t.n_slabs = kl_regulariser_fold_slabs(R);
+    t.n_apply = grid_for((long)R * D, 256);
+    max_slabs = max(max_slabs, t.n_slabs);
+    max_apply = max(max_apply, t.n_apply);
+  };
+  if (V >= 2) add(E, gE, V, W, 0);
+  for (int n = 0; n < n_ctx; ++n) add(ctx_tabs[n], gCtx[n], ctx_vocab, ctx_dim, 1);
+  if (nt == 0) {
+    if (status) hipLaunchKernelGGL(reg_apply_fold_kernel, dim3(1, 1), dim3(256), 0, stream, tabs, loss_acc, status);
+    return ok();
+  }
+  hipLaunchKernelGGL(reg_stats_fold_kernel, dim3(max_slabs, nt), dim3(256), 0, stream, tabs, counters);
+  hipLaunchKernelGGL(reg_apply_fold_kernel, dim3(max_apply, nt), dim3(256), 0, stream, tabs, loss_acc, status);
+  return ok();
+}
diff --git a/ocrd_keraslm_amd/csrc/kl_kernels.h b/ocrd_keraslm_amd/csrc/kl_kernels.h
--- a/ocrd_keraslm_amd/csrc/kl_kernels.h
+++ b/ocrd_keraslm_amd/csrc/kl_kernels.h
@@ -244,6 +244,7 @@
 struct KlConvJob {
   const float* in; long ld_in; int rows, cols, rows_pad, transpose;
   bf16_t* out_hi; bf16_t* out_lo; long ld_out;
+  int gate_w;
 };
 struct KlConvJobs { KlConvJob job[KL_CONV_MAX_JOBS]; };
 int kl_launch_f32_to_bf16_jobs(const KlConvJob* jobs, int n, hipStream_t stream);
@@ -271,6 +272,28 @@
 int kl_fill_u32_async(void* p, size_t bytes, unsigned value, hipStream_t stream);
 int kl_zero_coherent_async(unsigned* p, size_t n_words, hipStream_t stream);
 
+#define KL_ENTRY_MAX_ZERO 6
+#define KL_ENTRY_MAX_LAYERS 16
+struct KlWindowEntry {
+  void* zero[KL_ENTRY_MAX_ZERO]; size_t zero_bytes[KL_ENTRY_MAX_ZERO];
+  const float* states; int B, W, L;
+  bf16_t* h_bf16[KL_ENTRY_MAX_LAYERS]; float* h_f32[KL_ENTRY_MAX_LAYERS]; float* c_f32[KL_ENTRY_MAX_LAYERS];
+};
+int kl_launch_window_entry(const KlWindowEntry& e, hipStream_t stream);
+#define KL_COPY_MAX_JOBS 4
+struct KlCopyJob { const void* src; void* dst; size_t words; };
+struct KlCopyJobs { KlCopyJob job[KL_COPY_MAX_JOBS]; };
+int kl_launch_copy_jobs(const KlCopyJob* jobs, int n, hipStream_t stream);
+#define KL_ROWSTAT_FOLD_MAX_BLOCKS 512
+int kl_rowstat_fold_blocks(int rows);
+int kl_launch_rowstat_reduce_fold(const float* rowstat, int rows, float* loss_acc, float* part, unsigned* counter, hipStream_t stream);
+#define KL_REG_MAX_TABLES 9
+size_t kl_regulariser_fold_floats(int V, int W, int n_ctx, int ctx_vocab, int ctx_dim);
+int kl_regulariser_fold_slabs(int R);
+int kl_launch_regulariser_grads_fold(const float* E, int V, int W, const float* const* ctx_tabs, int n_ctx, int ctx_vocab, int ctx_dim,
+                                     float* gE, float* const* gCtx, float* loss_acc, float* fold_scratch, unsigned* counters,
+                                     const unsigned* status, hipStream_t stream);
+
 int kl_launch_small_table(const float* A, int R, int D, const float* Kmat, long ldk, int N, float* C, long ldc,
                           hipStream_t stream);
 int kl_launch_p1_gather(const float* EK, const float* const* ctxk, int n_ctx, const float* bias, const int* idx,
@@ -280,6 +303,14 @@
                             float* states, hipStream_t stream);
 int kl_launch_ctx_grads(const float* Ctx, const float* K0rows, long ldk, int R, int D, const float* dT, long ldt, int N,
                         float* gK, long ldg, float* gCtx, hipStream_t stream, long ldr = 1);
+#define KL_TABLE_MAX_JOBS 24
+struct KlTableJob { int kind, R, D, W; const float* A; const float* B; long ldk; float* out; float* out_p; };
+struct KlTableJobs { KlTableJob job[KL_TABLE_MAX_JOBS]; };
+int kl_launch_table_jobs(const KlTableJob* jobs, int n, hipStream_t stream);
+int kl_launch_ctx_grads_fold(const float* Ctx, const float* K0rows, long ldk, int R, int D, const float* dT, long ldt, int N,
+                             float* gK, long ldg, float* gCtx, hipStream_t stream, long ldr = 1);
+int kl_launch_rows_to_state_all(const void* const* h_rows, int h_is_f32, const float* const* c_rows, int B, int W, int L, float* states,
+                                hipStream_t stream);
 int kl_launch_rows_tm_to_bm(const float* in, long ld_in, float* out, int B, int T, int V, hipStream_t stream);
 
 #define KL_SEGSUM_MAX_BUCKETS 65535
@@ -287,7 +318,8 @@
 int kl_segment_sums_share(long BT);
 size_t kl_segment_sums_ws_bytes(int B, int T, int n_ctx, int V, int R);
 int kl_launch_segment_sums(const bf16_t* dZ, long ld, int B, int T, int cols, const int* idx, const int* ctx, int n_ctx, int V, int R,
-                           float* dEK, float* dCtxK, void* ws, hipStream_t stream);
+                           float* dEK, float* dCtxK, void* ws, hipStream_t stream, bool zeroed = false);
+size_t kl_segment_sums_counter_bytes(int n_ctx, int V, int R);
 
 int kl_launch_rate_pick(const float* logits, long ld, int rows, int V, const int* tgt, int B, int T, float* tprob,
                         hipStream_t stream);
diff --git a/ocrd_keraslm_amd/csrc/segsum.hip b/ocrd_keraslm_amd/csrc/segsum.hip
--- a/ocrd_keraslm_amd/csrc/segsum.hip
+++ b/ocrd_keraslm_amd/csrc/segsum.hip
@@ -221,8 +221,10 @@
   return (size_t)(seg_pad(kl_segment_sums_buckets(n_ctx, V, R) + 1) + 2 * seg_pad(BT)) * sizeof(int);
 }
 
+size_t kl_segment_sums_counter_bytes(int n_ctx, int V, int R) { return (size_t)seg_pad((long)kl_segment_sums_buckets(n_ctx, V, R) + 1) * sizeof(int); }
+
 int kl_launch_segment_sums(const bf16_t* dZ, long ld, int B, int T, int cols, const int* idx, const int* ctx, int n_ctx, int V, int R,
-                           float* dEK, float* dCtxK, void* ws, hipStream_t stream) {
+                           float* dEK, float* dCtxK, void* ws, hipStream_t stream, bool zeroed) {
   const long BT = (long)B * T;
   if (B < 1 || T < 1 || BT > 0x7fffffffL || V < 1 || n_ctx < 0 || (n_ctx > 0 && R < 1)) return KL_ERR_SHAPE;
   if (n_ctx == 0) R = 0;
@@ -238,8 +240,9 @@
   const size_t n_a = (size_t)nbp / 4, n_b = (size_t)V * cols / 4, n_c = (size_t)R * cols / 4;
   size_t g = (n_a + n_b + n_c + 255) / 256;
   if (g > 1024) g = 1024;
-  hipLaunchKernelGGL(segsum_init_kernel, dim3((unsigned)g), dim3(256), 0, stream, reinterpret_cast<uint4*>(offs), n_a,
-                     reinterpret_cast<uint4*>(dEK), n_b, reinterpret_cast<uint4*>(dCtxK), n_c);
+  if (!zeroed)
+    hipLaunchKernelGGL(segsum_init_kernel, dim3((unsigned)g), dim3(256), 0, stream, reinterpret_cast<uint4*>(offs), n_a,
+                       reinterpret_cast<uint4*>(dEK), n_b, reinterpret_cast<uint4*>(dCtxK), n_c);
   const unsigned gr = (unsigned)((BT + 255) / 256);
   hipLaunchKernelGGL(segsum_hist_kernel, dim3(gr), dim3(256), 0, stream, idx, ctx, n_ctx, B, T, V, R, offs);
   const int n4 = (int)(nbp / 4), per4 = (n4 + SEG_SCAN_THREADS - 1) / SEG_SCAN_THREADS;
diff --git a/ocrd_keraslm_amd/csrc/tables.hip b/ocrd_keraslm_amd/csrc/tables.hip
--- a/ocrd_keraslm_amd/csrc/tables.hip
+++ b/ocrd_keraslm_amd/csrc/tables.hip
@@ -1,3 +1,5 @@
+#include <string.h>
+
 #include "kl_common.h"
 #include "kl_kernels.h"
 
@@ -84,6 +86,92 @@
   if (lane == 0) gCtx[(long)r * D + d] += a;
 }
 
+constexpr int CTXG_MAXD = 16, CTXG_WAVES = 8;
+__global__ __launch_bounds__(CTXG_WAVES * 64) void ctx_grads_fold_kernel(const float* __restrict__ Ctx, const float* __restrict__ Krows, long ldk,
+                                                                         int R, int D, const float* __restrict__ dT, long ldt, long ldr, int N,
+                                                                         float* __restrict__ gK, long ldg, float* __restrict__ gCtx, int nk) {
+  __shared__ float part[CTXG_WAVES][CTXG_MAXD][64];
+  const int wave = __builtin_amdgcn_readfirstlane(threadIdx.x >> 6), lane = threadIdx.x & 63;
+  if ((int)blockIdx.x < nk) {
+    const int col = blockIdx.x * 64 + lane;
+    float a[CTXG_MAXD];
+#pragma unroll
+    for (int d = 0; d < CTXG_MAXD; ++d) a[d] = 0.f;
+    const int per = (R + CTXG_WAVES - 1) / CTXG_WAVES, r0 = wave * per, r1 = min(R, r0 + per);
+    if (col < N) {
+      for (int r = r0; r < r1; ++r) {
+        const float t = dT[(long)col * ldt + r * ldr];
+#pragma unroll
+        for (int d = 0; d < CTXG_MAXD; ++d)
+          if (d < D) a[d] = fmaf(Ctx[(long)r * D + d], t, a[d]);
+      }
+    }
+#pragma unroll
+    for (int d = 0; d < CTXG_MAXD; ++d) part[wave][d][lane] = a[d];
+    __syncthreads();
+    for (int d = wave; d < D; d += CTXG_WAVES) {
+      float s = 0.f;
+#pragma unroll
+      for (int w = 0; w < CTXG_WAVES; ++w) s += part[w][d][lane];
+      if (col < N) gK[(long)d * ldg + col] += s;
+    }
+    return;
+  }
+  const long item = (long)(blockIdx.x - nk) * CTXG_WAVES + wave;
+  if (item >= (long)R * D) return;
+  const int r = (int)(item / D), d = (int)(item % D);
+  float a = 0.f;
+  for (int col = lane; col < N; col += 64) a = fmaf(dT[(long)col * ldt + r * ldr], Krows[(long)d * ldk + col], a);
+#pragma unroll
+  for (int off = 32; off > 0; off >>= 1) a += __shfl_xor(a, off);
+  if (lane == 0) gCtx[(long)r * D + d] += a;
+}
+
+__global__ void table_jobs_kernel(const KlTableJobs jobs) {
+  const KlTableJob __attribute__((address_space(4)))* jp =
+      &((const KlTableJobs __attribute__((address_space(4)))*)__builtin_amdgcn_kernarg_segment_ptr())->job[blockIdx.y];
+  const int kind = jp->kind, R = jp->R, D = jp->D, W = jp->W;
+  const float* __restrict__ A = jp->A;
+  const float* __restrict__ Bm = jp->B;
+  const long ldk = jp->ldk;
+  float* __restrict__ out = jp->out;
+  float* __restrict__ out_p = jp->out_p;
+  const long i0 = blockIdx.x * (long)blockDim.x + threadIdx.x, stride = (long)gridDim.x * blockDim.x;
+  if (kind == 0) {
+    for (long i = i0; i < (long)R * W; i += stride) {
+      const long r = i / W;
+      const int u = (int)(i % W);
+      const float* p = A + r * 4 * W + u;
+      float4 v = float4{p[0], p[W], p[2 * W], p[3 * W]};
+      if (Bm) { v.x += Bm[u]; v.y += Bm[W + u]; v.z += Bm[2 * W + u]; v.w += Bm[3 * W + u]; }
+      *reinterpret_cast<float4*>(out_p + i * 4) = v;
+    }
+    return;
+  }
+  const int N = 4 * W;
+  for (long e = i0; e < (long)R * N; e += stride) {
+    const int r = (int)(e / N), n = (int)(e % N);
+    float a = 0.f;
+    for (int k = 0; k < D; ++k) a = fmaf(A[(long)r * D + k], Bm[(long)k * ldk + n], a);
+    out[(long)r * N + n] = a;
+    if (out_p) out_p[(long)r * N + (n % W) * 4 + n / W] = a;
+  }
+}
+
+struct StateRows { const void* h[16]; const float* c[16]; };
+__global__ void rows_to_state_all_kernel(const StateRows rows, int h_is_f32, int B, int W, int L, float* __restrict__ states) {
+  const int layer = blockIdx.y;
+  const void* h_rows = ((const StateRows __attribute__((address_space(4)))*)__builtin_amdgcn_kernarg_segment_ptr())->h[layer];
+  const float* c_rows = ((const StateRows __attribute__((address_space(4)))*)__builtin_amdgcn_kernarg_segment_ptr())->c[layer];
+  const long total = (long)B * W;
+  for (long e = blockIdx.x * (long)blockDim.x + threadIdx.x; e < total; e += (long)gridDim.x * blockDim.x) {
+    const int b = (int)(e / W), u = (int)(e % W);
+    float* s = states + ((long)b * 2 * L + 2 * layer) * W;
+    s[u] = h_is_f32 ? reinterpret_cast<const float*>(h_rows)[e] : bf2f(reinterpret_cast<const bf16_t*>(h_rows)[e]);
+    s[W + u] = c_rows[e];
+  }
+}
+
 __global__ void rows_tm_to_bm_kernel(const float* __restrict__ in, long ld_in, float* __restrict__ out, int B, int T,
                                      int V) {
   const long total = (long)B * T * V;
@@ -147,6 +235,40 @@
   return ok();
 }
 
+int kl_launch_ctx_grads_fold(const float* Ctx, const float* K0rows, long ldk, int R, int D, const float* dT, long ldt, int N,
+                             float* gK, long ldg, float* gCtx, hipStream_t stream, long ldr) {
+  if (D < 1 || D > CTXG_MAXD || R < 1 || N < 1) return KL_ERR_SHAPE;
+  const int nk = (N + 63) / 64;
+  const long items = (long)R * D;
+  hipLaunchKernelGGL(ctx_grads_fold_kernel, dim3((unsigned)(nk + (items + CTXG_WAVES - 1) / CTXG_WAVES)), dim3(CTXG_WAVES * 64), 0, stream,
+                     Ctx, K0rows, ldk, R, D, dT, ldt, ldr, N, gK, ldg, gCtx, nk);
+  return ok();
+}
+
+int kl_launch_table_jobs(const KlTableJob* jobs, int n, hipStream_t stream) {
+  if (n < 1 || n > KL_TABLE_MAX_JOBS) return KL_ERR_SHAPE;
+  KlTableJobs all;
+  memset(&all, 0, sizeof(all));
+  long most = 1;
+  for (int j = 0; j < n; ++j) {
+    all.job[j] = jobs[j];
+    const long items = (long)jobs[j].R * jobs[j].W * (jobs[j].kind == 0 ? 1 : 4);
+    if (items > most) most = items;
+  }
+  hipLaunchKernelGGL(table_jobs_kernel, dim3(grid_for(most, 256), n), dim3(256), 0, stream, all);
+  return ok();
+}
+
+int kl_launch_rows_to_state_all(const void* const* h_rows, int h_is_f32, const float* const* c_rows, int B, int W, int L, float* states,
+                                hipStream_t stream) {
+  if (L < 1 || L > 16) return KL_ERR_SHAPE;
+  StateRows rows;
+  memset(&rows, 0, sizeof(rows));
+  for (int l = 0; l < L; ++l) { rows.h[l] = h_rows[l]; rows.c[l] = c_rows[l]; }
+  hipLaunchKernelGGL(rows_to_state_all_kernel, dim3(grid_for((long)B * W, 256), L), dim3(256), 0, stream, rows, h_is_f32, B, W, L, states);
+  return ok();
+}
+
 int kl_launch_rows_tm_to_bm(const float* in, long ld_in, float* out, int B, int T, int V, hipStream_t stream) {
   hipLaunchKernelGGL(rows_tm_to_bm_kernel, dim3(grid_for((long)B * T * V, 256)), dim3(256), 0, stream, in, ld_in, out,
                      B, T, V);
```

Result: no change. 36.50 million chars/s, median of 6 (+0.9%).
